# XiangLi2022/CM-TTS

Measured on AMD Instinct MI355X. Metric: mel-frames/s (text->mel hot path, consistency sampling T=4), higher is better.
Workload: dtype f32

## Files before the change

cm-tts_amd/csrc/cmtts_api.hip:

```cpp
#include <hip/hip_runtime.h>
#include <limits.h>
#include <math.h>
#include <stdio.h>
#include <stdlib.h>
#include <string.h>

#include <algorithm>
#include <map>
#include <string>
#include <vector>

#include "../../include/cmtts_hip.h"
#include "internal_hooks.h"
#include "conv_args.h"
#include "kernels.h"
#include "resblock_args.h"
#include "persist_args.h"
#include "cond_gemm.h"
#include "resblock_pair.h"
#include "inproj.h"
#include "attention.h"
#include "text_state.h"
#include "stream_windows.h"

namespace {

thread_local std::string g_err;
int fail(int code, const std::string& msg) {
    g_err = msg;
    return code;
}
#define HIPCHK(x)                                                                              \
    do {                                                                                       \
        hipError_t e_ = (x);                                                                   \
        if (e_ != hipSuccess) return fail(CMTTS_E_HIP, std::string(#x) + ": " + hipGetErrorString(e_)); \
    } while (0)
#define CHK(x)                 \
    do {                       \
        int r_ = (x);          \
        if (r_ != 0) return r_; \
    } while (0)

struct HostTensor {
    std::vector<int64_t> shape;
    std::vector<float> data;
    int64_t dim(int i) const { return i < (int)shape.size() ? shape[i] : 1; }
};

struct PackedConv {
    float* w = nullptr;
    float* bias = nullptr;
    int cout = 0, cin = 0, taps = 0, ld = 0;
    long tap_stride = 0, phase_stride = 0;
};

inline int round_up(int v, int m) { return (v + m - 1) / m * m; }

struct Allocs {
    std::vector<void*> ptrs;
    int upload(const std::vector<float>& h, float** out) {
        void* p = nullptr;
        HIPCHK(hipMalloc(&p, h.size() * sizeof(float) + 256));
        HIPCHK(hipMemcpy(p, h.data(), h.size() * sizeof(float), hipMemcpyHostToDevice));
        ptrs.push_back(p);
        *out = (float*)p;
        return 0;
    }
    int upload_bytes(const void* h, size_t nbytes, void** out) {
        void* p = nullptr;
        HIPCHK(hipMalloc(&p, nbytes + 256));
        HIPCHK(hipMemcpy(p, h, nbytes, hipMemcpyHostToDevice));
        ptrs.push_back(p);
        *out = p;
        return 0;
    }
    void release() {
        for (void* p : ptrs) (void)hipFree(p);
        ptrs.clear();
    }
};

int pack_conv(Allocs& al, const HostTensor& W, const HostTensor* bias, const std::vector<int>* perm, PackedConv* out,
              std::vector<float>* host_copy = nullptr) {
    const int Cout = (int)W.dim(0), Cin = (int)W.dim(1), K = (int)W.dim(2);
    const int ld = round_up(Cout, 4);
    std::vector<float> p((size_t)K * Cin * ld, 0.f);
    for (int k = 0; k < K; ++k)
        for (int ci = 0; ci < Cin; ++ci)
            for (int r = 0; r < Cout; ++r) {
                const int co = perm ? (*perm)[r] : r;
                p[((size_t)k * Cin + ci) * ld + r] = W.data[((size_t)co * Cin + ci) * K + k];
            }
    CHK(al.upload(p, &out->w));
    if (host_copy) *host_copy = p;
    out->bias = nullptr;
    if (bias) {
        std::vector<float> b(Cout);
        for (int r = 0; r < Cout; ++r) b[r] = bias->data[perm ? (*perm)[r] : r];
        CHK(al.upload(b, &out->bias));
    }
    out->cout = Cout; out->cin = Cin; out->taps = K; out->ld = ld;
    out->tap_stride = (long)Cin * ld;
    out->phase_stride = 0;
    return 0;
}

int pack_conv_transpose(Allocs& al, const HostTensor& W, const HostTensor& bias, int s, PackedConv* out,
                        std::vector<float>* two_tap = nullptr) {
    const int Cin = (int)W.dim(0), Cout = (int)W.dim(1), K = (int)W.dim(2);
    const int Q = K / s, ld = round_up(Cout, 4);
    if (two_tap && Q == 2) {
        two_tap->assign((size_t)2 * Cin * s * Cout, 0.f);
        for (int q = 0; q < 2; ++q)
            for (int ci = 0; ci < Cin; ++ci)
                for (int r = 0; r < s; ++r)
                    for (int co = 0; co < Cout; ++co)
                        (*two_tap)[((size_t)q * Cin + ci) * s * Cout + (size_t)r * Cout + co] = W.data[((size_t)ci * Cout + co) * K + (r + s * q)];
    }
    std::vector<float> p((size_t)s * Q * Cin * ld, 0.f);
    for (int r = 0; r < s; ++r)
        for (int q = 0; q < Q; ++q)
            for (int ci = 0; ci < Cin; ++ci)
                for (int co = 0; co < Cout; ++co)
                    p[(((size_t)r * Q + q) * Cin + ci) * ld + co] = W.data[((size_t)ci * Cout + co) * K + (r + s * q)];
    CHK(al.upload(p, &out->w));
    CHK(al.upload(bias.data, &out->bias));
    out->cout = Cout; out->cin = Cin; out->taps = Q; out->ld = ld;
    out->tap_stride = (long)Cin * ld;
    out->phase_stride = (long)Q * Cin * ld;
    return 0;
}

std::vector<float> to_fragment_order(const std::vector<float>& p, int taps, int K, int M) {
    std::vector<float> f((size_t)taps * K * M);
    const int G = K / 8, MTn = M / 32;
    for (int tap = 0; tap < taps; ++tap)
        for (int g = 0; g < G; ++g)
            for (int mt = 0; mt < MTn; ++mt)
                for (int lane = 0; lane < 64; ++lane)
                    for (int j = 0; j < 4; ++j)
                        f[((((size_t)tap * G + g) * MTn + mt) * 64 + lane) * 4 + j] =
                            p[((size_t)tap * K + 8 * g + 2 * j + (lane >> 5)) * M + 32 * mt + (lane & 31)];
    return f;
}

constexpr int WINO_PAD_HG = 4;
std::vector<float> to_wino_fragments(const std::vector<float>& p, int K, int M) {
    std::vector<float> f((size_t)4 * K * M + (size_t)WINO_PAD_HG * (M / 32) * 2 * 64 * 4, 0.0f);
    const int MTn = M / 32;
    for (int hg = 0; hg < K / 4; ++hg)
        for (int mt = 0; mt < MTn; ++mt)
            for (int ps = 0; ps < 2; ++ps)
                for (int lane = 0; lane < 64; ++lane)
                    for (int q = 0; q < 4; ++q) {
                        const int tr = 2 * ps + (q >> 1), k = 4 * hg + 2 * (q & 1) + (lane >> 5), mrow = 32 * mt + (lane & 31);
                        const double g0 = p[((size_t)0 * K + k) * M + mrow], g1 = p[((size_t)1 * K + k) * M + mrow], g2 = p[((size_t)2 * K + k) * M + mrow];
                        const double v = tr == 0 ? g0 : tr == 1 ? 0.5 * (g0 + g1 + g2) : tr == 2 ? 0.5 * (g0 - g1 + g2) : g2;
                        f[((((size_t)hg * MTn + mt) * 2 + ps) * 64 + lane) * 4 + q] = (float)v;
                    }
    return f;
}

constexpr int WINO43_PAD_KS = 4;
std::vector<float> to_wino43_fragments(const std::vector<float>& p, int K, int M) {
    const int NWV = M / 64;
    std::vector<float> f((size_t)(K / 4 + WINO43_PAD_KS) * NWV * 6 * 64 * 4, 0.0f);
    for (int ks = 0; ks < K / 4; ++ks)
        for (int w = 0; w < NWV; ++w)
            for (int tr = 0; tr < 6; ++tr)
                for (int lane = 0; lane < 64; ++lane)
                    for (int e = 0; e < 4; ++e) {
                        const int k = 4 * ks + (lane >> 4), mrow = 64 * w + 16 * e + (lane & 15);
// ... 816 lines not shown
            }
        if (H % 16 == 0 && (NL * C) % 32 == 0 && m->cond_all.ld == NL * C) {
            const std::vector<unsigned short> fs = to_fragment16_split(hp, 1, H, NL * C);
            CHK(al.upload_bytes(fs.data(), fs.size() * 2, &m->cond_all_f16[2]));
        }
    }
    CHK(al.upload(dproj, &m->dproj_wt));
    if (c.multi_speaker) CHK(al.upload(sproj, &m->sproj_wt));
    {
        GET(w, "net.skip_projection.conv.weight", C, C, 1); GET(b, "net.skip_projection.conv.bias", C);
        std::vector<float> hp;
        CHK(pack_conv(al, *w, b, nullptr, &m->skip_proj, &hp));
        if (C % 32 == 0 && m->skip_proj.ld == C) CHK(al.upload(to_fragment_order(hp, 1, C, C), &m->skip_f));
        GET(w2, "net.output_projection.conv.weight", c.n_mels, C, 1); GET(b2, "net.output_projection.conv.bias", c.n_mels);
        CHK(pack_conv(al, *w2, b2, nullptr, &m->out_proj, &hp));
        {
            const int ld = m->out_proj.ld, Mp = round_up(c.n_mels, 32);
            std::vector<float> padded((size_t)C * Mp, 0.f);
            for (int k = 0; k < C; ++k)
                for (int n = 0; n < c.n_mels; ++n) padded[(size_t)k * Mp + n] = hp[(size_t)k * ld + n];
            CHK(al.upload(to_fragment_order(padded, 1, C, Mp), &m->outp_f));
        }
    }
    if (m->cond_all_f && (NL * C) % 512 == 0) {
        GET(pe, va + "pitch_embed.weight", c.pitch_bins, H);
        float* peT = nullptr;
        void* p2 = nullptr;
        CHK(al.upload(transpose2d(pe->data.data(), c.pitch_bins, H), &peT));
        CHK(al.upload(std::vector<float>((size_t)NL * C, 0.f), &m->cond_zero_bias));
        HIPCHK(hipMalloc(&p2, (size_t)NL * C * c.pitch_bins * sizeof(float) + 256));
        al.ptrs.push_back(p2);
        CondGemmArgs ga;
        memset(&ga, 0, sizeof(ga));
        ga.X = peT; ga.Wf = m->cond_all_f; ga.bias = m->cond_all.bias; ga.Y = (float*)p2;
        ga.B = 1; ga.T = c.pitch_bins; ga.M = NL * C; ga.K = H; ga.force = 1; ga.row_split = NL * C / 512;
        if (cmtts_launch_cond_gemm(&ga, nullptr) == 0) {
            void* p2t = nullptr;
            HIPCHK(hipMalloc(&p2t, (size_t)NL * C * c.pitch_bins * sizeof(float) + 256));
            al.ptrs.push_back(p2t);
            k_transpose((const float*)p2, (float*)p2t, NL, C, c.pitch_bins, nullptr);
            HIPCHK(hipStreamSynchronize(nullptr));
            m->cond_p2 = (float*)p2;
            m->cond_p2t = (float*)p2t;
        }
    }
#undef GET
#undef UP
    m->host.clear();
    m->finalized = true;
    return 0;
}

constexpr int FFN2_SEG = 8;
struct TextWs {
    float *x, *h, *qk, *vt, *st, *o, *f, *part, *c1, *c2, *spk, *out1, *h128, *logd, *dround, *epred, *escaled, *pctl;
    int* cum;
    int64_t *eidx, *mlen;
    size_t bytes;
};
TextWs carve_text(const cmtts_config& c, int B, int L, void* base) {
    const int Lp = round_up(L, 4), H = c.hidden;
    Carver cv(base);
    TextWs w;
    const size_t n = (size_t)B * H * Lp;
    w.out1 = cv.take<float>(n);
    w.cum = cv.take<int>((size_t)B * L);
    w.spk = cv.take<float>((size_t)B * H);
    w.h128 = cv.take<float>((size_t)B * c.cwt_hidden * Lp);
    w.x = cv.take<float>(n);
    w.h = cv.take<float>(n);
    w.qk = cv.take<float>(3 * n);
    w.vt = w.qk + 2 * n;
    w.st = cv.take<float>((size_t)B * c.enc_heads * Lp * Lp);
    w.o = cv.take<float>(n);
    w.f = cv.take<float>(4 * n);
    w.part = cv.take<float>(FFN2_SEG * n);
    w.c1 = cv.take<float>(n);
    w.c2 = cv.take<float>(n);
    w.logd = cv.take<float>((size_t)B * L);
    w.dround = cv.take<float>((size_t)B * L);
    w.epred = cv.take<float>((size_t)B * L);
    w.eidx = cv.take<int64_t>((size_t)B * L);
    w.mlen = cv.take<int64_t>((size_t)B);
    w.escaled = cv.take<float>((size_t)B * L);
    w.pctl = cv.take<float>((size_t)B * L);
    w.bytes = cv.off + 256;
    return w;
}

struct FrameWs {
    float *xlr, *h128, *hp, *c1, *c2, *cwt, *r, *s1, *s2, *stats, *f0;
    int64_t* pidx;
    size_t bytes;
};
FrameWs carve_frame(const cmtts_config& c, int B, int T, void* base) {
    Carver cv(base);
    FrameWs w;
    const size_t n = (size_t)B * c.hidden * T;
    w.xlr = cv.take<float>(n);
    w.h128 = cv.take<float>((size_t)B * c.cwt_hidden * T);
    w.hp = cv.take<float>((size_t)B * c.cwt_hidden * T);
    w.c1 = cv.take<float>(n);
    w.c2 = cv.take<float>(n);
    w.cwt = cv.take<float>((size_t)B * T * 16);
    w.r = cv.take<float>((size_t)B * T);
    w.s1 = cv.take<float>((size_t)B * c.cwt_hidden);
    w.s2 = cv.take<float>((size_t)B * c.cwt_hidden);
    w.stats = cv.take<float>((size_t)B * 2);
    w.f0 = cv.take<float>((size_t)B * T);
    w.pidx = cv.take<int64_t>((size_t)B * T);
    w.bytes = cv.off + 256;
    return w;
}

struct DenWs {
    float *hin, *h, *u, *zb, *skip, *emb, *e1, *e2, *dproj, *sproj, *dp, *tbuf, *xcur, *cp;
    float* pst;
    unsigned long long* halo;
    size_t bytes;
};
DenWs carve_den(const cmtts_config& c, int B, int T, void* base) {
    Carver cv(base);
    DenWs w;
    const int C = c.res_channels, NL = c.res_layers;
    const size_t n = (size_t)B * C * T;
    w.hin = cv.take<float>((size_t)B * c.n_mels * T);
    w.h = cv.take<float>(n);
    w.u = cv.take<float>(n);
    w.zb = cv.take<float>(n);
    w.skip = cv.take<float>(n);
    w.emb = cv.take<float>((size_t)B * C);
    w.e1 = cv.take<float>((size_t)B * 4 * C);
    w.e2 = cv.take<float>((size_t)B * C);
    w.dproj = cv.take<float>((size_t)B * NL * C);
    w.sproj = cv.take<float>((size_t)B * NL * C);
    w.dp = cv.take<float>((size_t)B * NL * C);
    w.tbuf = cv.take<float>((size_t)B);
    w.xcur = cv.take<float>((size_t)B * T * c.n_mels);
    w.cp = cv.take<float>((size_t)NL * n);
    w.halo = cv.take<unsigned long long>(cmtts_persist_halo_bytes(B, T) / sizeof(unsigned long long));
    w.pst = cv.take<float>(cmtts_persist_state_floats(B, T));
    w.bytes = cv.off + 256;
    return w;
}

struct EnergyHead {
    const float* xin; const float* e_target; float e_control; const float* bins; int nbins; const float* E; float* out1; int64_t* e_idx; float* e_scaled;
    bool done;
    const float* e_table = nullptr;
};
int g_energy_head = 1;
int g_pred_wino = 1;
int g_pred_xres = 1;
int predictor(const Predictor& P, const float* in, int ld_in, int B, int T, int ld, const int64_t* ln_lens,
              const int64_t* out_lens, float* bufA, float* bufB, float* out, int O, hipStream_t s, int mode16 = 0, bool frame_level = false,
              EnergyHead* eh = nullptr) {
    const float* cur = in;
    int ldc = ld_in;
    auto other = [&](const float* p) { return p == bufA ? bufB : bufA; };
    int pend_ln = -1;
    for (size_t li = 0; li < P.convs.size(); ++li) {
        const PackedConv& w = P.convs[li];
        int rx = -2;
        float* dst = other(cur);
        if (frame_level && !mode16 && g_pred_wino && !ln_lens && li < P.convs_q.size() && P.convs_q[li] && w.taps == 5 && w.cout == 256 &&
            (pend_ln < 0 || w.cin == 256)) {
            ConvXlArgs xa;
            memset(&xa, 0, sizeof(xa));
            xa.x = cur; xa.y = dst; xa.wf = P.convs_q[li]; xa.bias = w.bias; xa.bstride = (long)w.cout * ld;
            xa.B = B; xa.C = 256; xa.T = T; xa.ld = ld; xa.k = w.taps; xa.dil = 1; xa.slope = 1.0f; xa.relu = 1;
            if (w.cin != 256) { xa.cin = w.cin; xa.xbstride = (long)w.cin * ldc; }
            if (pend_ln >= 0) { xa.ln_g = P.ln_g[pend_ln]; xa.ln_b = P.ln_b[pend_ln]; xa.ln_eps = 1e-12f; }
            if (ldc == ld || w.cin != 256) {
                rx = cmtts_launch_conv_k5q(&xa, (void*)s);
                if (rx == -3) return fail(CMTTS_E_HIP, "conv_k5q launch failed");
                if (rx == 0) pend_ln = -2;
            }
        }
        const bool small = (long)((T + 63) / 64) * B < 192;
        if (rx != 0 && !mode16 && g_pred_xres && small && P.convs_f[li] && w.cin == 256 && w.cout == 256 && ldc == ld) {
            ConvArgs a = conv_args(w, cur, T, ldc, (long)w.cin * ldc, dst, ld, (long)w.cout * ld, T);
            a.out[0].act = ACT_RELU;
            a.xres_nt = 1;
            if (pend_ln >= 0) { a.ln_g = P.ln_g[pend_ln]; a.ln_b = P.ln_b[pend_ln]; a.ln_eps = 1e-12f; a.ln_lens = ln_lens; a.ln_skip_tiles = 1; }
            rx = cmtts_launch_conv_xres(&a, P.convs_f[li], B, (void*)s);
            if (rx == -3) return fail(CMTTS_E_HIP, "conv_xres launch failed");
            if (rx == 0) pend_ln = -2;
        }
        if (pend_ln >= 0) {
            float* nd = other(cur);
            k_layernorm_ct(cur, nd, P.ln_g[pend_ln], P.ln_b[pend_ln], 1e-12f, ln_lens, B, T, ld, s);
            cur = nd;
            dst = other(cur);
        }
        pend_ln = -1;
        if (mode16 && li < P.convs_f16[mode16 - 1].size() && P.convs_f16[mode16 - 1][li]) {
            ConvArgs a = conv_args(w, cur, T, ldc, (long)w.cin * ldc, dst, ld, (long)w.cout * ld, T);
            a.out[0].act = ACT_RELU;
            a.text_epi = 1;
            rx = cmtts_launch_conv16(&a, P.convs_f16[mode16 - 1][li], mode16, B, (void*)s);
            if (rx == -3) return fail(CMTTS_E_HIP, "text16: predictor conv launch failed");
        }
        if (rx != 0 && g_pred_xl && P.convs_f[li] && ldc == ld && (long)((T + 63) / 64) * B >= 192) {
            ConvXlArgs xa;
            memset(&xa, 0, sizeof(xa));
            xa.x = cur; xa.y = dst; xa.wf = P.convs_f[li]; xa.bias = w.bias; xa.bstride = (long)w.cout * ld;
            xa.B = B; xa.C = 256; xa.T = T; xa.ld = ld; xa.k = w.taps; xa.dil = 1; xa.slope = 1.0f; xa.relu = 1;
            if (w.cin != 256) { xa.cin = w.cin; xa.xbstride = (long)w.cin * ldc; }
            rx = cmtts_launch_conv_xl(&xa, (void*)s);
            if (rx == -3) return fail(CMTTS_E_HIP, "conv_xl launch failed");
        }
        if (rx != 0) {
            ConvArgs a = conv_args(w, cur, T, ldc, (long)w.cin * ldc, dst, ld, (long)w.cout * ld, T);
            a.out[0].act = ACT_RELU;
            CHK(launch(a, EPI_PLAIN, B, s));
        }
        cur = dst;
        ldc = ld;
        if (g_pred_head && eh && g_energy_head && O == 1 && li + 1 == P.convs.size() && w.cout == 256) {
            k_ln_linear_energy(cur, P.ln_g[li], P.ln_b[li], 1e-12f, P.lin_w, P.lin_b, out, ln_lens, out_lens, B, T, ld, eh->xin, eh->e_target, eh->e_control,
                               eh->bins, eh->nbins, eh->E, eh->out1, eh->e_idx, eh->e_scaled, s, eh->e_table);
            eh->done = true;
            return 0;
        }
        if (g_pred_head && li + 1 == P.convs.size() && w.cout == 256 &&
            k_ln_linear(cur, P.ln_g[li], P.ln_b[li], 1e-12f, P.lin_w, P.lin_b, out, ln_lens, out_lens, B, T, ld, O, s))
            return 0;
        pend_ln = (int)li;
    }
    if (pend_ln >= 0) {
        float* nd = other(cur);
        k_layernorm_ct(cur, nd, P.ln_g[pend_ln], P.ln_b[pend_ln], 1e-12f, ln_lens, B, T, ld, s);
        cur = nd;
    }
    k_chan_linear(cur, P.lin_w, P.lin_b, out, out_lens, B, P.convs.back().cout, T, ld, O, s);
    return 0;
}

int cond_projections(cmtts_model* m, const DenWs& w, const float* cond_ct, int B, int T, hipStream_t s) {
    const cmtts_config& c = m->cfg;
    if (g_cond_gemm16 && m->precision >= 1 && m->precision <= 3 && m->cond_all_f16[m->precision - 1]) {
        CondGemmArgs g;
        g.X = cond_ct; g.Wf = nullptr; g.bias = m->cond_all.bias; g.Y = w.cp;
        g.row_split = 0;
        g.B = B; g.T = T; g.M = c.res_layers * c.res_channels; g.K = c.hidden; g.force = 1;
        const int r = cmtts_launch_cond_gemm16(&g, m->cond_all_f16[m->precision - 1], m->precision, (void*)s);
        if (r == 0) return 0;
        if (r != -2) return fail(CMTTS_E_HIP, "cond_gemm16 launch failed");
    }
    if (m->cond_all_f) {
        CondGemmArgs g;
        g.X = cond_ct; g.Wf = m->cond_all_f; g.bias = m->cond_all.bias; g.Y = w.cp;
        g.row_split = 0;
        g.B = B; g.T = T; g.M = c.res_layers * c.res_channels; g.K = c.hidden; g.force = g_cond_gemm == 2;
        const int r = g_cond_gemm ? cmtts_launch_cond_gemm(&g, (void*)s) : -2;
        if (r == 0) return 0;
        if (r != -2) return fail(CMTTS_E_HIP, "cond_gemm launch failed");
    }
    ConvArgs a = conv_args(m->cond_all, cond_ct, T, T, (long)c.hidden * T, w.cp, T, (long)c.res_layers * c.res_channels * T, T);
    return launch(a, EPI_PLAIN, B, s);
}

struct CondFactors {
    const float* p1 = nullptr;
    const float* p1t = nullptr;
    int ldp = 0, L = 0;
    const int64_t* mel2ph = nullptr;
    const int64_t* p_idx = nullptr;
    bool usable(const cmtts_model* m) const;
};
int g_cond_factored = 1;
int g_cond_inkernel = 1;
inline bool C_IS_256(const cmtts_config& c) { return c.res_channels == 256; }
bool CondFactors::usable(const cmtts_model* m) const {
    return g_cond_factored && p1 && mel2ph && p_idx && m->precision == 0 && m->cond_p2 && g_fused_resblock;
}
int cond_factored(cmtts_model* m, const DenWs& w, const CondFactors& f, int B, int T, hipStream_t s) {
    const cmtts_config& c = m->cfg;
    const int r = cmtts_launch_cond_expand(f.p1, f.ldp, f.L, m->cond_p2, c.pitch_bins, f.mel2ph, f.p_idx, w.cp, B, c.res_layers * c.res_channels, T, (void*)s);
    return r == 0 ? 0 : fail(CMTTS_E_HIP, "cond_expand launch failed");
}
int cond_phoneme_factor(cmtts_model* m, const float* out1, int B, int Lp, float* p1, hipStream_t s) {
    const cmtts_config& c = m->cfg;
    if (!m->cond_p2) return fail(CMTTS_E_UNSUPPORTED, "factored conditioner projections are not available for this model");
    CondGemmArgs g;
    memset(&g, 0, sizeof(g));
    g.X = out1; g.Wf = m->cond_all_f; g.bias = m->cond_zero_bias; g.Y = p1;
    g.B = B; g.T = Lp; g.M = c.res_layers * c.res_channels; g.K = c.hidden; g.force = 1;
    g.flat = 1;
    const long tiles = ((long)B * Lp + 63) / 64;
    const int npass = g.M / 512;
    int best = 1;
    double best_t = 1e30;
    for (int sp = 1; sp <= npass; ++sp) {
        const int ppg = (npass + sp - 1) / sp, groups = (npass + ppg - 1) / ppg;
        const long wg = tiles * groups, cap = persist_blocks();
        const double t = (double)((wg + cap - 1) / cap) * ppg;
        if (t < best_t - 1e-9) { best_t = t; best = sp; }
    }
    g.row_split = best;
    const int r = cmtts_launch_cond_gemm(&g, (void*)s);
    return r == 0 ? 0 : fail(r == -2 ? CMTTS_E_UNSUPPORTED : CMTTS_E_HIP, "cond_gemm (phoneme factor) launch failed");
}

int step_embedding(cmtts_model* m, const DenWs& w, const float* timesteps, const float* spk, int B, hipStream_t s,
                   float t_host = NAN) {
    const cmtts_config& c = m->cfg;
    const int C = c.res_channels, NL = c.res_layers;
    if (c.multi_speaker && !spk) return fail(CMTTS_E_INVALID, "speaker_emb is required for a multi-speaker model");
    const bool cacheable = g_step_cache && t_host == t_host;
    if (cacheable) {
        for (const cmtts_model::StepRow& e : m->step_rows)
            if (e.t == t_host && hipEventQuery(e.ready) == hipSuccess) {
                k_broadcast_row(e.row, w.dproj, B, NL * C, s);
                if (c.multi_speaker) {
                    k_dense_small(spk, c.hidden, 1, m->sproj_wt, nullptr, nullptr, w.sproj, B, c.hidden, NL * C, DENSE_NONE, s);
                    k_add_rows(w.dproj, w.sproj, w.dp, (long)B * NL * C, s);
                }
                return 0;
            }
    }
    k_diff_embed(timesteps, m->omega_res, w.emb, B, C, s);
    k_dense_small(w.emb, C, 1, m->mlp0_wt, nullptr, nullptr, w.e1, B, C, 4 * C, DENSE_MISH, s);
    k_dense_small(w.e1, 4 * C, 1, m->mlp2_wt, nullptr, nullptr, w.e2, B, 4 * C, C, DENSE_NONE, s);
    k_dense_small(w.e2, C, 1, m->dproj_wt, nullptr, nullptr, w.dproj, B, C, NL * C, DENSE_NONE, s);
    if (c.multi_speaker) {
        k_dense_small(spk, c.hidden, 1, m->sproj_wt, nullptr, nullptr, w.sproj, B, c.hidden, NL * C, DENSE_NONE, s);
        k_dense_small(w.e2, C, 1, m->dproj_wt, nullptr, w.sproj, w.dp, B, C, NL * C, DENSE_NONE, s);
    }
    if (cacheable && m->step_rows.size() < 16) {
        bool known = false;
        for (const cmtts_model::StepRow& e : m->step_rows) known = known || e.t == t_host;
        if (!known) {
            cmtts_model::StepRow e{t_host, nullptr, nullptr};
            void* p = nullptr;
            if (hipMalloc(&p, (size_t)NL * C * sizeof(float)) == hipSuccess && hipEventCreateWithFlags(&e.ready, hipEventDisableTiming) == hipSuccess) {
                e.row = (float*)p;
                m->al.ptrs.push_back(p);
                HIPCHK(hipMemcpyAsync(e.row, w.dproj, (size_t)NL * C * sizeof(float), hipMemcpyDeviceToDevice, s));
                HIPCHK(hipEventRecord(e.ready, s));
                m->step_rows.push_back(e);
            } else if (p) {
                (void)hipFree(p);
            }
        }
    }
    return 0;
}

struct MelPost {
    const float* xold;
    const float* noise;
    float c_out, c_skip, nstd;
    float* out;
};

int denoiser_prologue(cmtts_model* m, const DenWs& w, const float* x_src, float in_scale, const float* timesteps, const float* spk, int B,
                      int T, hipStream_t s, bool embed, float t_host, bool* halo_zeroed) {
    const cmtts_config& c = m->cfg;
    const int C = c.res_channels, NL = c.res_layers, M = c.n_mels;
    const long cs = (long)C * T;
    *halo_zeroed = false;
    int rin = -2;
    if (g_inproj_fused && m->in_proj_f) {
        InProjArgs ia;
        memset(&ia, 0, sizeof(ia));
        ia.x = x_src; ia.scale = in_scale; ia.wf = m->in_proj_f; ia.bias = m->in_proj.bias; ia.h = w.h;
        ia.B = B; ia.T = T; ia.M = M; ia.C = C;
        const bool persist_path = g_fused_resblock && g_persist && NL <= PERSIST_MAX_LAYERS;
        if (persist_path) { ia.zero = w.halo; ia.zero_f4 = (long)(cmtts_persist_halo_bytes(B, T) / 16); }
        rin = cmtts_launch_inproj(&ia, (void*)s);
        if (rin == -3) return fail(CMTTS_E_HIP, "inproj launch failed");
        *halo_zeroed = rin == 0 && persist_path && cmtts_persist_halo_bytes(B, T) % 16 == 0;
    }
    if (rin != 0) {
        k_mel_prep(x_src, nullptr, in_scale, w.hin, B, T, M, s);
        ConvArgs a = conv_args(m->in_proj, w.hin, T, T, (long)M * T, w.h, T, cs, T);
        a.out[0].act = ACT_RELU;
        CHK(launch(a, EPI_PLAIN, B, s));
    }
    if (embed) CHK(step_embedding(m, w, timesteps, spk, B, s, t_host));
    return 0;
}

int batch_invariant_form(const cmtts_model* m) {
    if (!m->batch_invariant || m->precision != 0 || !m->winograd || !g_persist_wino || !m->res[0].w3w) return 0;
    return m->winograd == 1 && g_persist_wino == 3 && m->res[0].w3w43 ? 1 : -1;
}
int check_batch_invariant(const cmtts_model* m) {
    if (batch_invariant_form(m) >= 0) return 0;
    return fail(CMTTS_E_UNSUPPORTED, "batch_invariant: the persistent denoiser stack runs the F(2,3) form (model option \"winograd\" = 2), "
                                     "which has no per-layer counterpart; set \"winograd\" to 1 or 0");
}

int denoiser_core(cmtts_model* m, const DenWs& w, const float* x_src, float in_scale, const float* timesteps,
                  const float* cond_ct, const float* spk, int B, int T, const MelPost& post, hipStream_t s, bool embed = true,
                  SideStream* pending = nullptr, float t_host = NAN,
                  const CondFactors* cfk = nullptr, bool* cp_ready = nullptr) {
    CHK(check_device_flag(true));
    const cmtts_config& c = m->cfg;
    const int C = c.res_channels, NL = c.res_layers, M = c.n_mels;
    const long cs = (long)C * T;
    bool halo_zeroed = false;
    CHK(denoiser_prologue(m, w, x_src, in_scale, timesteps, spk, B, T, s, embed, t_host, &halo_zeroed));
    if (pending) CHK(branch_join(pending));
    const float* dp = m->cfg.multi_speaker ? w.dp : w.dproj;
    const bool unfused = !g_fused_resblock;
    float* hcur = w.h;
    float* halt = w.u;
    bool layers_done = false;
    if (!unfused && g_persist && NL <= PERSIST_MAX_LAYERS) {
        PersistArgs pa;
        memset(&pa, 0, sizeof(pa));
        pa.x0 = w.h; pa.cp = w.cp; pa.cp_bstride = (long)NL * C * T;
        pa.dp = dp; pa.d = w.dproj; pa.vec_stride = (long)NL * C;
        pa.skip = w.skip; pa.halo = w.halo; pa.tmo = g_tmo_host;
        pa.B = B; pa.T = T; pa.NL = NL;
        pa.halo_zeroed = halo_zeroed;
        const int prec = m->precision;
        if (cfk && !(cp_ready && *cp_ready)) {
            pa.fact = 1; pa.p1 = cfk->p1; pa.p2 = m->cond_p2; pa.mel2ph = (const long long*)cfk->mel2ph; pa.pidx = (const long long*)cfk->p_idx;
            pa.ldp = cfk->ldp; pa.Lph = cfk->L; pa.ld2 = c.pitch_bins;
            pa.p1t = cfk->p1t; pa.p2t = m->cond_p2t;
        }
        if (g_persist_tail && m->skip_f && m->outp_f) {
            pa.tail = 1;
            pa.Wsf = m->skip_f; pa.bs = m->skip_proj.bias; pa.Wpf = m->outp_f; pa.bp = m->out_proj.bias;
            pa.skip_div = (float)sqrt((double)NL); pa.n_mels = M;
            pa.xold = post.xold; pa.noise = post.noise; pa.c_out = post.c_out; pa.c_skip = post.c_skip; pa.nstd = post.nstd;
            pa.out = post.out;
        }
        pa.wino = g_persist_wino && m->winograd && !prec && m->res[0].w3w && w.pst;
        if (pa.wino && g_persist_wino == 3 && m->winograd == 1 && m->res[0].w3w43) pa.wino = 3;
        pa.xst = w.pst;
        for (int l = 0; l < NL; ++l) {
            pa.W3f[l] = prec ? (const float*)m->res[l].w3f16[prec - 1] : (pa.wino == 3 ? m->res[l].w3w43 : pa.wino ? m->res[l].w3w : m->res[l].w3f);
            pa.Wof[l] = prec ? (const float*)m->res[l].wof16[prec - 1] : m->res[l].wof;
            pa.b3[l] = m->res[l].b3f; pa.bo[l] = m->res[l].outp.bias;
        }
        const bool prof = g_prof.on && g_prof.used + 2 <= g_prof.ev.size();
        const int need = cmtts_persist_plan(B, T, NL, persist_blocks(), g_persist == 2);
        if (need) CHK(persist_admit(s, need, persist_blocks()));
        if (prof) (void)hipEventRecord(g_prof.ev[g_prof.used], s);
        const int rc = prec ? cmtts_launch_denoiser_persist_lp(&pa, prec, persist_blocks(), g_persist == 2, (void*)s)
                            : cmtts_launch_denoiser_persist(&pa, persist_blocks(), g_persist == 2, (void*)s);
        if (rc == -3) return fail(CMTTS_E_HIP, "persistent denoiser launch failed");
        if (rc == 0) {
            CHK(persist_launched(s, need));
            if (prof) { (void)hipEventRecord(g_prof.ev[g_prof.used + 1], s); g_prof.used += 2; }
            layers_done = true;
            if (pa.tail) return 0;
        }
    }
    if (!layers_done && cfk && !(cp_ready && *cp_ready)) {
        CHK(cond_factored(m, w, *cfk, B, T, s));
        if (cp_ready) *cp_ready = true;
    }
    const bool w43 = batch_invariant_form(m) > 0;
    for (int l = 0; l < NL && !layers_done; ++l) {
        const ResLayer& R = m->res[l];
        const bool prof = g_prof.on && g_prof.used + 2 <= g_prof.ev.size() && (g_prof.seen++ % g_prof.stride) == 0;
        if (!unfused) {
            ResArgs ra;
            memset(&ra, 0, sizeof(ra));
            ra.x_in = hcur; ra.cp = w.cp + (long)l * C * T; ra.cp_bstride = (long)NL * C * T;
            ra.dp = dp + (long)l * C; ra.d = w.dproj + (long)l * C;
            ra.x_out = halt; ra.skip = w.skip;
            ra.W3f = R.w3f; ra.b3 = R.b3f; ra.Wof = R.wof; ra.bo = R.outp.bias;
            ra.vec_stride = (long)NL * C; ra.B = B; ra.T = T; ra.accum_skip = l > 0; ra.flag = g_tmo_host;
            if (prof) (void)hipEventRecord(g_prof.ev[g_prof.used], s);
            int lrc;
            if (m->precision == 0 || m->precision == 3) {
                const long tiles32 = (long)((T + 31) / 32) * B;
                ra.z = w.zb;
                if (w43) {
                    ra.W3f = R.w3w43;
                    lrc = cmtts_launch_resblock_w43(&ra, (void*)s);
                } else if (g_split_resblock == 2 || (g_split_resblock == 1 && tiles32 <= SPLIT_MAX_TILES)) lrc = cmtts_launch_resblock_split(&ra, (void*)s);
                else lrc = cmtts_launch_resblock(&ra, (void*)s);
            } else {
                ra.W3f = (const float*)R.w3f16[m->precision - 1];
                ra.Wof = (const float*)R.wof16[m->precision - 1];
                lrc = cmtts_launch_resblock_lp(&ra, m->precision, (void*)s);
            }
            if (lrc != 0) return fail(CMTTS_E_HIP, "fused residual block launch failed");
            if (prof) { (void)hipEventRecord(g_prof.ev[g_prof.used + 1], s); g_prof.used += 2; }
            float* t = hcur; hcur = halt; halt = t;
            continue;
        }
        {
            ConvArgs a = conv_args(R.cond, cond_ct, T, T, (long)c.hidden * T, halt, T, cs, T);
            a.out[0].bvec = dp + (long)l * C; a.out[0].bvec_zs = (long)NL * C;
            a.out[0].res = hcur; a.out[0].r_zs0 = cs; a.out[0].ldr = T;
            CHK(launch(a, EPI_PLAIN, B, s));
        }
        if (w43) {
            ResArgs ra;
            memset(&ra, 0, sizeof(ra));
            ra.u = halt; ra.x_in = hcur; ra.x_out = halt; ra.skip = w.skip; ra.z = w.zb;
            ra.d = w.dproj + (long)l * C; ra.dp = dp + (long)l * C; ra.cp = w.cp;
            ra.W3f = R.w3w43; ra.b3 = R.b3f; ra.Wof = R.wof; ra.bo = R.outp.bias;
            ra.vec_stride = (long)NL * C; ra.B = B; ra.T = T; ra.accum_skip = l > 0;
            if (cmtts_launch_resblock_w43(&ra, (void*)s) != 0) return fail(CMTTS_E_HIP, "F(4,3) residual block launch failed");
            float* t = hcur; hcur = halt; halt = t;
            continue;
        }
        {
            ConvArgs a = conv_args(R.conv3, halt, T, T, cs, w.zb, T, cs, T);
            if (prof) (void)hipEventRecord(g_prof.ev[g_prof.used], s);
            CHK(launch(a, EPI_GATED, B, s));
            if (prof) { (void)hipEventRecord(g_prof.ev[g_prof.used + 1], s); g_prof.used += 2; }
        }
        {
            ConvArgs a = conv_args(R.outp, w.zb, T, T, cs, hcur, T, cs, T);
            a.split = C;
            a.out[0].res = hcur; a.out[0].r_zs0 = cs; a.out[0].ldr = T;
            a.out[0].bvec = w.dproj + (long)l * C; a.out[0].bvec_zs = (long)NL * C;
            a.out[0].rmul = 0.70710678118654752440f;
            a.out[1].Y = w.skip; a.out[1].row_off = C; a.out[1].accum = l > 0;
            CHK(launch(a, EPI_PLAIN, B, s));
        }
    }
    {
        ConvArgs a = conv_args(m->skip_proj, w.skip, T, T, cs, halt, T, cs, T);
        a.pre_div = (float)sqrt((double)NL);
        a.out[0].act = ACT_RELU;
        CHK(launch(a, EPI_PLAIN, B, s));
        ConvArgs b = conv_args(m->out_proj, halt, T, T, cs, w.hin, T, (long)M * T, T);
        CHK(launch(b, EPI_PLAIN, B, s));
    }
    k_mel_post(w.hin, post.xold, post.noise, post.c_out, post.c_skip, post.nstd, post.out, B, T, M, g_tmo_host, s);
    return 0;
}

}

extern "C" {

const char* cmtts_last_error(void) { return g_err.c_str(); }
int cmtts_internal_fail(int code, const char* msg) { return fail(code, msg ? msg : "?"); }
const char* cmtts_version(void) { return "cmtts_hip 0.3 (gfx950)"; }
int cmtts_abi_version(void) { return CMTTS_ABI_VERSION; }

int cmtts_create(const cmtts_config* cfg, cmtts_model** out) {
    if (!cfg || !out) return fail(CMTTS_E_INVALID, "cmtts_create: null argument");
    cmtts_model* m = new cmtts_model();
    m->cfg = *cfg;
    *out = m;
    return 0;
}

int cmtts_set_tensor(cmtts_model* m, const char* name, const float* host_data, const int64_t* shape, int ndim) {
    if (!m || m->finalized) return fail(CMTTS_E_INVALID, "cmtts_set_tensor: model is null or already finalized");
    return set_tensor(m->host, name, host_data, shape, ndim);
}

int cmtts_finalize(cmtts_model* m) {
    if (!m || m->finalized) return fail(CMTTS_E_INVALID, "cmtts_finalize: model is null or already finalized");
    const int r = finalize_model(m);
    if (r != 0) m->al.release();
    if (r == 0 && !g_tmo_host) {
        if (hipHostMalloc((void**)&g_tmo_host, sizeof(unsigned), hipHostMallocMapped) != hipSuccess) g_tmo_host = nullptr;
        else *g_tmo_host = 0;
    }
    return r;
}

void cmtts_destroy(cmtts_model* m) {
    if (!m) return;
    for (cmtts_model::StepRow& e : m->step_rows) (void)hipEventDestroy(e.ready);
    m->al.release();
    delete m;
}

size_t cmtts_text_workspace_bytes(const cmtts_model* m, int B, int L) { return carve_text(m->cfg, B, L, nullptr).bytes; }
size_t cmtts_frame_workspace_bytes(const cmtts_model* m, int B, int T) { return carve_frame(m->cfg, B, T, nullptr).bytes; }
size_t cmtts_denoiser_workspace_bytes(const cmtts_model* m, int B, int T) { return carve_den(m->cfg, B, T, nullptr).bytes; }

int fft_stack(cmtts_model* m, const std::vector<EncLayer>& layers, const TextWs& w, const int64_t* src_lens, int B, int L,
              hipStream_t s, const int64_t* pad_lens = nullptr) {
    const cmtts_config& c = m->cfg;
    const int H = c.hidden, Lp = round_up(L, 4), NH = c.enc_heads, dh = H / NH;
    const long hs = (long)H * Lp;
    const int t96 = (L + 95) / 96, t64 = (L + 63) / 64;
    const bool cols96 = t96 * 96 <= t64 * 64;
    const bool xres_small = g_ffn_xres && g_xres_small && (long)t96 * B * 8 < 128;
    const bool xres_cols = g_ffn_xres && (cols96 || xres_small);
    for (size_t i = 0; i < layers.size(); ++i) {
        const EncLayer& E = layers[i];
        const bool fused_attn = g_attn_fused && dh == 128;
        const int pm = m->precision;
        const bool t16 = m->text16 && (pm == 1 || pm == 2) && E.ffn1_f16[pm - 1] && E.ffn2_f16[pm - 1] && E.qkv_f16[pm - 1] && E.wo_f16[pm - 1];
        const bool ln_qkv = !t16 && fused_attn && (g_text_xres & 1) && E.qkv_f && xres_cols && ((long)t96 * (3 * H / 128) * B >= 128 || xres_small);
        if (!ln_qkv) k_layernorm_ct(w.x, w.h, E.ln1_g, E.ln1_b, 1e-12f, nullptr, B, L, Lp, s);
        bool attn_done = false;
        if (fused_attn) {
            int rq = -2;
            if (ln_qkv) {
                ConvArgs a = conv_args(E.qkv, w.x, L, Lp, hs, w.qk, Lp, 3 * hs, L);
                a.ln_g = E.ln1_g; a.ln_b = E.ln1_b; a.ln_eps = 1e-12f;
                if (g_text_xres & 8) {
                    k_layernorm_ct(w.x, w.h, E.ln1_g, E.ln1_b, 1e-12f, nullptr, B, L, Lp, s);
                    a.X = w.h; a.ln_g = a.ln_b = nullptr;
                }
                a.xres_nt = g_qkv_nt ? g_qkv_nt : ((long)t96 * (3 * H / 128) * B > persist_blocks() ? 1 : 0);
                rq = cmtts_launch_conv_xres(&a, E.qkv_f, B, (void*)s);
// ... 62 lines not shown
            ConvOut& o = a.out[0];
            o.Y = w.o; o.y_zs0 = hs; o.y_zs1 = (long)dh * Lp; o.ldy = Lp; o.Tout = L; o.ostride = 1; o.alpha = 1.f; o.div = 1.f;
            CHK(launch(a, EPI_PLAIN, B * NH, s));
        }
        }
        {
            ConvArgs a = conv_args(E.wo, w.o, L, Lp, hs, w.x, Lp, hs, L);
            a.out[0].res = w.x; a.out[0].r_zs0 = hs; a.out[0].ldr = Lp; a.out[0].lens = src_lens;
            int rc = -2;
            if (t16) {
                a.text_epi = 1;
                rc = cmtts_launch_conv16(&a, E.wo_f16[pm - 1], pm, B, (void*)s);
                if (rc == -3) return fail(CMTTS_E_HIP, "text16: out-projection launch failed");
                a.text_epi = 0;
            } else if (E.wo_f && g_ffn_xres && (g_text_xres & 2)) {
                a.xres_nt = 1;
                rc = cmtts_launch_conv_xres(&a, E.wo_f, B, (void*)s);
                a.xres_nt = 0;
            }
            if (rc == -3) return fail(CMTTS_E_HIP, "conv_xres launch failed");
            if (rc != 0) CHK(launch(a, EPI_PLAIN, B, s));
        }
        if (t16) {
            k_layernorm_ct(w.x, w.h, E.ln2_g, E.ln2_b, 1e-12f, pad_lens, B, L, Lp, s);
            ConvArgs a = conv_args(E.ffn1, w.h, L, Lp, hs, w.f, Lp, 4 * hs, L);
            a.out[0].alpha = (float)pow((double)c.ffn_kernel, -0.5);
            a.out[0].act = ACT_GELU_ERF;
            a.text_epi = 1;
            int rc = cmtts_launch_conv16(&a, E.ffn1_f16[pm - 1], pm, B, (void*)s);
            if (rc == 0) {
                ConvArgs b = conv_args(E.ffn2, w.f, L, Lp, 4 * hs, w.x, Lp, hs, L);
                b.out[0].res = w.x; b.out[0].r_zs0 = hs; b.out[0].ldr = Lp; b.out[0].lens = src_lens;
                b.text_epi = 1;
                rc = cmtts_launch_conv16(&b, E.ffn2_f16[pm - 1], pm, B, (void*)s);
                if (rc != 0) return fail(CMTTS_E_HIP, "text16: FFN linear launch failed");
                continue;
            }
            if (rc != -2) return fail(CMTTS_E_HIP, "text16: FFN conv launch failed");
        }
        const bool ffn2_seg = m->ffn2_split && E.ffn2.cin % FFN2_SEG == 0 && E.ffn2.taps == 1;
        bool ffn_fused = false;
        {
            const float* wqf = g_ffn_wino == 2 ? E.ffn1_q : E.ffn1_p;
            const bool wq = g_ffn_wino && g_ffn_xres && g_ffn_fused && (g_text_xres & 4) && wqf && E.ffn2_f && m->ffn2_split && E.ffn2.cin % FFN2_SEG == 0 &&
                            E.ffn2.taps == 1 && E.ffn1.cout == FFN2_SEG * 128 && H == 256;
            const bool xr = wq || (xres_cols && E.ffn1_f && ((long)t96 * ((E.ffn1.cout + 127) / 128) * B >= 128 || xres_small));
            const bool ln_ffn = xr && (g_text_xres & 4);
            if (!ln_ffn) k_layernorm_ct(w.x, w.h, E.ln2_g, E.ln2_b, 1e-12f, pad_lens, B, L, Lp, s);
            ConvArgs a = conv_args(E.ffn1, ln_ffn ? w.x : w.h, L, Lp, hs, w.f, Lp, 4 * hs, L);
            a.out[0].alpha = (float)pow((double)c.ffn_kernel, -0.5);
            a.out[0].act = ACT_GELU_ERF;
            if (ln_ffn) { a.ln_g = E.ln2_g; a.ln_b = E.ln2_b; a.ln_eps = 1e-12f; a.ln_lens = pad_lens; a.ln_skip_tiles = pad_lens != nullptr; }
            int rc = -2;
            if (xr && g_ffn_fused && ffn2_seg && E.ffn2_f && E.ffn1.cout == FFN2_SEG * 128) {
                a.w2frag = E.ffn2_f; a.part = w.part; a.part_zs0 = (long)FFN2_SEG * hs; a.part_zs1 = hs; a.part_ld = Lp; a.M2 = H;
                rc = wq ? cmtts_launch_conv_xresq(&a, wqf, B, (void*)s, g_ffn_wino == 2 ? 1 : 2) : -2;
                if (rc == -2) rc = cmtts_launch_conv_xres(&a, E.ffn1_f, B, (void*)s);
                if (rc == 0) ffn_fused = true;
                else { a.w2frag = nullptr; a.part = nullptr; }
            }
            if (xr && !ffn_fused) rc = cmtts_launch_conv_xres(&a, E.ffn1_f, B, (void*)s);
            if (rc == -3) return fail(CMTTS_E_HIP, "conv_xres launch failed");
            if (rc != 0) {
                if (ln_ffn) {
                    k_layernorm_ct(w.x, w.h, E.ln2_g, E.ln2_b, 1e-12f, pad_lens, B, L, Lp, s);
                    a.X = w.h; a.ln_g = a.ln_b = nullptr; a.ln_lens = nullptr;
                }
                CHK(launch(a, EPI_PLAIN, B, s));
            }
        }
        if (ffn_fused) {
            k_reduce_partials(w.part, FFN2_SEG, E.ffn2.bias, w.x, src_lens, w.x, B, H, L, Lp, s);
        } else if (ffn2_seg) {
            const int kseg = E.ffn2.cin / FFN2_SEG;
            ConvArgs a = conv_args(E.ffn2, w.f, L, Lp, 4 * hs, w.part, Lp, (long)FFN2_SEG * hs, L);
            a.K = kseg;
            a.zdiv = FFN2_SEG; a.a_zs0 = 0; a.a_zs1 = (long)kseg * a.a_ld; a.x_zs1 = (long)kseg * Lp;
            a.out[0].y_zs1 = hs; a.out[0].bias = nullptr;
            CHK(launch(a, EPI_PLAIN, B * FFN2_SEG, s));
            k_reduce_partials(w.part, FFN2_SEG, E.ffn2.bias, w.x, src_lens, w.x, B, H, L, Lp, s);
        } else {
            ConvArgs a = conv_args(E.ffn2, w.f, L, Lp, 4 * hs, w.x, Lp, hs, L);
            a.out[0].res = w.x; a.out[0].r_zs0 = hs; a.out[0].ldr = Lp; a.out[0].lens = src_lens;
            CHK(launch(a, EPI_PLAIN, B, s));
        }
    }
    return 0;
}

int cmtts_text_forward(cmtts_model* m, const int64_t* texts, const int64_t* src_lens, const float* spker_embeds,
                       const int64_t* speakers, int B, int L, float d_control, float* log_d, float* d_rounded, int64_t* mel_len,
                       float* e_pred, int64_t* e_idx, float* enc_out_ct, float* speaker_emb,
                       void* text_ws, size_t text_ws_bytes, void* stream) {
    return cmtts_text_forward_ragged(m, texts, src_lens, nullptr, spker_embeds, speakers, B, L, d_control, log_d, d_rounded, mel_len, e_pred,
                                     e_idx, enc_out_ct, speaker_emb, text_ws, text_ws_bytes, stream);
}

int cmtts_text_forward_ragged(cmtts_model* m, const int64_t* texts, const int64_t* src_lens, const int64_t* pad_lens, const float* spker_embeds,
                              const int64_t* speakers, int B, int L, float d_control, float* log_d, float* d_rounded, int64_t* mel_len,
                              float* e_pred, int64_t* e_idx, float* enc_out_ct, float* speaker_emb,
                              void* text_ws, size_t text_ws_bytes, void* stream) {
    if (!m || !m->finalized) return fail(CMTTS_E_INVALID, "model not finalized");
    if (!texts || !src_lens || !text_ws || B <= 0 || L <= 0) return fail(CMTTS_E_INVALID, "cmtts_text_forward: bad argument");
    const cmtts_config& c = m->cfg;
    if (c.multi_speaker && c.n_speaker > 0 && !speakers) return fail(CMTTS_E_INVALID, "speakers (ids into the speaker_emb table) are required (model/cmtts.py:78)");
    if (c.multi_speaker && c.n_speaker <= 0 && !spker_embeds) return fail(CMTTS_E_INVALID, "Speaker embedding should not be None (model/cmtts.py:80)");
    const cmtts_control_tables& ct = m->ct;
    if ((ct.d || ct.e || ct.p) && ct.ld != L)
        return fail(CMTTS_E_INVALID, "cmtts_text_forward: the control tables' row pitch ld must equal L (cmtts_set_control_tables)");
    if (ct.d && d_control != 1.0f)
        return fail(CMTTS_E_INVALID, "cmtts_text_forward: a duration table replaces d_control, which must then be 1");
    if (ct.e && m->vc.e_control != 1.0f)
        return fail(CMTTS_E_INVALID, "cmtts_text_forward: an energy table replaces e_control, which must then be 1");
    TextWs w = carve_text(c, B, L, text_ws);
    if (text_ws_bytes < w.bytes) return fail(CMTTS_E_WORKSPACE, "text workspace too small");
    hipStream_t s = (hipStream_t)stream;
    const int H = c.hidden, Lp = round_up(L, 4);
    if (!log_d) log_d = w.logd;
    if (!d_rounded) d_rounded = w.dround;
    if (!mel_len) mel_len = w.mlen;
    if (!e_pred) e_pred = w.epred;
    if (!e_idx) e_idx = w.eidx;

    k_embed_tokens(texts, src_lens, m->embed, m->omega_h, m->pe_h, PE_ROWS, w.x, B, L, Lp, H, (float)sqrt((double)H), s);
    CHK(fft_stack(m, m->enc, w, src_lens, B, L, s, pad_lens));
    k_layernorm_ct(w.x, w.x, m->encln_g, m->encln_b, 1e-5f, src_lens, B, L, Lp, s);
    if (enc_out_ct && c.multi_speaker)
        k_copy_rows(enc_out_ct, L, w.x, Lp, L, (long)B * H, s);
    if (c.multi_speaker) {
        if (c.n_speaker > 0) k_gather_rows(m->spk_table, speakers, w.spk, B, H, c.n_speaker, s);
        else k_dense_small(spker_embeds, c.external_speaker_dim, 1, m->spk_wt, m->spk_b, nullptr, w.spk, B,
                      c.external_speaker_dim, H, DENSE_NONE, s);
        k_add_rowvec(w.x, w.spk, B, H, L, Lp, s, pad_lens);
        if (speaker_emb) HIPCHK(hipMemcpyAsync(speaker_emb, w.spk, (size_t)B * H * 4, hipMemcpyDeviceToDevice, s));
    }
    SideStream* ss = side_for(s);
    hipStream_t se = ss ? ss->side : s;
    float* ec1 = ss ? w.qk : w.c1;
    float* ec2 = ss ? w.qk + (size_t)B * H * Lp : w.c2;
    if (ss) CHK(branch_fork(ss));
    const int t16mode = (m->text16 && (m->precision == 1 || m->precision == 2)) ? m->precision : 0;
    CHK(predictor(m->dur, w.x, Lp, B, L, Lp, src_lens, src_lens, w.c1, w.c2, log_d, 1, s, t16mode));
    if (m->vc.d_target) {
        HIPCHK(hipMemcpyAsync(d_rounded, m->vc.d_target, (size_t)B * L * 4, hipMemcpyDeviceToDevice, s));
        k_cumsum_durations(m->vc.d_target, w.cum, mel_len, B, L, s);
    } else if (ct.d) {
        k_durations_table(log_d, ct.d, d_rounded, w.cum, mel_len, B, L, s);
    } else {
        k_durations(log_d, d_control, d_rounded, w.cum, mel_len, B, L, s);
    }
    if (ct.p) HIPCHK(hipMemcpyAsync(w.pctl, ct.p, (size_t)B * L * 4, hipMemcpyDeviceToDevice, s));
    if (enc_out_ct && !c.multi_speaker)
        k_copy_rows(enc_out_ct, L, w.x, Lp, L, (long)B * H, s);
    k_pos_embed_add(w.x, w.h, m->energy.alpha, m->omega_h, m->pe_h, PE_ROWS, B, H, L, Lp, se);
    EnergyHead eh{w.x, m->vc.e_target, m->vc.e_control, m->energy_bins, c.energy_bins - 1, m->energy_emb, w.out1, e_idx, w.escaled, false, ct.e};
    CHK(predictor(m->energy, w.h, Lp, B, L, Lp, pad_lens, pad_lens, ec1, ec2, e_pred, 1, se, t16mode, false, H == 256 ? &eh : nullptr));
    if (ss) CHK(branch_join(ss));
    if (!eh.done)
        k_energy_embed(w.x, e_pred, w.escaled, m->vc.e_target, m->vc.e_control, m->energy_bins, c.energy_bins - 1, m->energy_emb,
                       w.out1, e_idx, B, H, L, Lp, s, ct.e);
    {
        ConvArgs a = conv_args(m->cwt_in, w.out1, L, Lp, (long)H * Lp, w.h128, Lp, (long)c.cwt_hidden * Lp, L);
        int rc = -2;
        if (g_ffn_xres && g_pred_xres && m->cwt_in_f) {
            a.xres_nt = 1;
            rc = cmtts_launch_conv_xres(&a, m->cwt_in_f, B, (void*)s);
            if (rc == -3) return fail(CMTTS_E_HIP, "conv_xres launch failed");
            a.xres_nt = 0;
        }
        if (rc != 0) CHK(launch(a, EPI_PLAIN, B, s));
    }
    if (!m->vc.e_target && (ct.e || m->vc.e_control != 1.0f))
        HIPCHK(hipMemcpyAsync(e_pred, w.escaled, (size_t)B * L * 4, hipMemcpyDeviceToDevice, s));
    HIPCHK(hipGetLastError());
    return 0;
}

int cmtts_frame_forward(cmtts_model* m, const void* text_ws, int B, int L, int T, float* cond_ct, int64_t* mel2ph,
                        float* cwt_out, float* f0_denorm, int64_t* p_idx, float* f0_stats, void* frame_ws,
                        size_t frame_ws_bytes, void* stream) {
    return cmtts_frame_forward_sub(m, text_ws, B, L, 0, B, T, cond_ct, mel2ph, cwt_out, f0_denorm, p_idx, f0_stats, nullptr, frame_ws, frame_ws_bytes, stream);
}

int cmtts_frame_forward_sub(cmtts_model* m, const void* text_ws, int B_all, int L_all, int b0, int B, int T, float* cond_ct, int64_t* mel2ph,
                            float* cwt_out, float* f0_denorm, int64_t* p_idx, float* f0_stats, float* cond_p1, void* frame_ws,
                            size_t frame_ws_bytes, void* stream) {
    return cmtts_frame_forward_sub_t(m, text_ws, B_all, L_all, b0, B, T, cond_ct, mel2ph, cwt_out, f0_denorm, p_idx, f0_stats, cond_p1, nullptr, frame_ws,
                                     frame_ws_bytes, stream);
}

int cmtts_frame_forward_sub_t(cmtts_model* m, const void* text_ws, int B_all, int L_all, int b0, int B, int T, float* cond_ct, int64_t* mel2ph,
                              float* cwt_out, float* f0_denorm, int64_t* p_idx, float* f0_stats, float* cond_p1, float* cond_p1t, void* frame_ws,
                              size_t frame_ws_bytes, void* stream) {
    if (!m || !m->finalized) return fail(CMTTS_E_INVALID, "model not finalized");
    if (!text_ws || !frame_ws || !cond_ct || !mel2ph || B <= 0 || L_all <= 0 || T <= 0 || b0 < 0 || b0 + B > B_all)
        return fail(CMTTS_E_INVALID, "cmtts_frame_forward: bad argument");
    const cmtts_config& c = m->cfg;
    const int L = L_all;
    TextWs tw = carve_text(c, B_all, L_all, const_cast<void*>(text_ws));
    tw.out1 += (size_t)b0 * c.hidden * round_up(L_all, 4);
    tw.h128 += (size_t)b0 * c.cwt_hidden * round_up(L_all, 4);
    tw.cum += (size_t)b0 * L_all;
    tw.pctl += (size_t)b0 * L_all;
    if (m->ct.p && m->ct.ld != L_all)
        return fail(CMTTS_E_INVALID, "cmtts_frame_forward: the control tables' row pitch ld must equal L_all (cmtts_set_control_tables)");
    if (m->ct.p && m->vc.p_control != 1.0f)
        return fail(CMTTS_E_INVALID, "cmtts_frame_forward: a pitch table replaces p_control, which must then be 1");
    FrameWs w = carve_frame(c, B, T, frame_ws);
    if (frame_ws_bytes < w.bytes) return fail(CMTTS_E_WORKSPACE, "frame workspace too small");
    hipStream_t s = (hipStream_t)stream;
    const int H = c.hidden, Lp = round_up(L, 4), O = c.use_uv ? 11 : 10, CH = c.cwt_hidden;
    if (!cwt_out) cwt_out = w.cwt;
    if (!f0_denorm) f0_denorm = w.f0;
    if (!p_idx) p_idx = w.pidx;
    if (!f0_stats) f0_stats = w.stats;

    SideStream* ss = side_for(s);
    hipStream_t sst = ss ? ss->side : s;
    if (ss) CHK(branch_fork(ss));
    if (cond_p1t && !cond_p1) return fail(CMTTS_E_INVALID, "cmtts_frame_forward_sub_t: cond_p1t needs cond_p1");
    if (cond_p1 && m->cond_p2) {
        CHK(cond_phoneme_factor(m, tw.out1, B, Lp, cond_p1, sst));
        if (cond_p1t) k_transpose(cond_p1, cond_p1t, B * c.res_layers, c.res_channels, Lp, sst);
    }
    if (!(g_stats_mlp && k_stats_mlp(tw.out1, (long)H * Lp, Lp, m->st0_wt, m->st0_b, m->st2_wt, m->st2_b, m->st4_wt, m->st4_b, f0_stats, B, H, CH, CH, 2, sst))) {
        k_dense_small(tw.out1, (long)H * Lp, Lp, m->st0_wt, m->st0_b, nullptr, w.s1, B, H, CH, DENSE_RELU, sst);
        k_dense_small(w.s1, CH, 1, m->st2_wt, m->st2_b, nullptr, w.s2, B, CH, CH, DENSE_RELU, sst);
        k_dense_small(w.s2, CH, 1, m->st4_wt, m->st4_b, nullptr, f0_stats, B, CH, 2, DENSE_NONE, sst);
    }
    k_mel2ph(tw.cum, mel2ph, B, L, T, s);
    if (!g_cwt_in_phoneme) k_length_regulate(tw.out1, mel2ph, w.xlr, B, H, Lp, T, s);
    bool hp_done = false;
    if (g_cwt_in_phoneme) {
        k_pos_embed_add_lr(tw.h128, Lp, mel2ph, m->cwt_in.bias, w.hp, m->cwt.alpha, m->omega_cwt, m->pe_cwt, PE_ROWS, B, CH, T, s);
        hp_done = true;
    } else {
        ConvArgs a = conv_args(m->cwt_in, w.xlr, T, T, (long)H * T, w.h128, T, (long)CH * T, T);
        CHK(launch(a, EPI_PLAIN, B, s));
    }
    if (!hp_done) k_pos_embed_add(w.h128, w.hp, m->cwt.alpha, m->omega_cwt, m->pe_cwt, PE_ROWS, B, CH, T, T, s);
    CHK(predictor(m->cwt, w.hp, T, B, T, T, nullptr, nullptr, w.c1, w.c2, cwt_out, O, s, (m->text16 && (m->precision == 1 || m->precision == 2)) ? m->precision : 0, true));
    if (ss) CHK(branch_join(ss));
    if (m->ct.p) k_pitch_table_scale(cwt_out, mel2ph, tw.cum, tw.pctl, B, O, L, T, s);
    else if (m->vc.p_control != 1.0f) k_scale(cwt_out, cwt_out, (long)B * T * O, m->vc.p_control, s);
    if (m->vc.cwt_spec) {
        k_pitch_index(m->vc.cwt_spec, 10, m->vc.f0_mean, m->vc.f0_std, 1, 1.0f, nullptr, 0, c.use_uv ? m->vc.uv : nullptr,
                      c.pitch_norm_eps, w.r, p_idx, f0_denorm, B, T, s);
    } else {
        k_pitch_index(cwt_out, O, f0_stats, f0_stats + 1, 2, c.cwt_std_scale, c.use_uv ? cwt_out + (O - 1) : nullptr, O, nullptr,
                      c.pitch_norm_eps, w.r, p_idx, f0_denorm, B, T, s);
    }
    if (g_cwt_in_phoneme) k_lr_gather_add(tw.out1, mel2ph, Lp, p_idx, m->pitch_emb, cond_ct, B, H, T, s);
    else k_gather_add(w.xlr, p_idx, m->pitch_emb, cond_ct, B, H, T, s);
    HIPCHK(hipGetLastError());
    return 0;
}

namespace {
struct TextStateLayout {
    long off[TEXT_STATE_MAX_REGIONS], bytes[TEXT_STATE_MAX_REGIONS], stride[TEXT_STATE_MAX_REGIONS];
    long rec_bytes;
    int n_regions;
};
TextStateLayout text_state_layout(const cmtts_config& c, int L, bool with_p) {
    const int Lp = round_up(L, 4);
    TextStateLayout t;
    t.bytes[0] = (long)c.hidden * Lp * 4;
    t.bytes[1] = (long)c.cwt_hidden * Lp * 4;
    t.bytes[2] = (long)c.hidden * 4;
    t.bytes[3] = (long)L * 4;
    t.bytes[4] = (long)L * 4;
    t.n_regions = with_p ? 5 : 4;
    long off = TEXT_STATE_HEADER_BYTES;
    for (int g = 0; g < t.n_regions; ++g) {
        t.stride[g] = t.bytes[g];
        t.off[g] = off;
        off += (t.bytes[g] + 15) / 16 * 16;
    }
    t.rec_bytes = off;
    return t;
}
TextStateCopy text_state_args(const cmtts_config& c, void* ws, int B_all, int L, void* records, int n, int unpack, bool with_p) {
    const TextStateLayout t = text_state_layout(c, L, with_p);
    TextWs tw = carve_text(c, B_all, L, ws);
    char* base[TEXT_STATE_MAX_REGIONS] = {(char*)tw.out1, (char*)tw.h128, (char*)tw.spk, (char*)tw.cum, (char*)tw.pctl};
    TextStateCopy a;
    memset(&a, 0, sizeof(a));
    int chunks = 0;
    for (int g = 0; g < t.n_regions; ++g) {
        TextStateRegion& R = a.reg[g];
        R.ws = base[g]; R.ws_stride = t.stride[g]; R.rec_off = t.off[g]; R.bytes = t.bytes[g];
        R.vec16 = ((uintptr_t)R.ws % 16 == 0 && R.ws_stride % 16 == 0 && R.bytes % 16 == 0 && (uintptr_t)records % 16 == 0) ? 1 : 0;
        R.chunk0 = chunks;
        chunks += (int)((R.bytes + TEXT_STATE_CHUNK - 1) / TEXT_STATE_CHUNK);
    }
    a.n_regions = t.n_regions; a.n_chunks = chunks; a.unpack = unpack;
    a.layout = with_p ? TEXT_STATE_LAYOUT_P : TEXT_STATE_LAYOUT;
    a.n = n; a.B_all = B_all; a.L_all = L; a.hidden = c.hidden; a.cwt_hidden = c.cwt_hidden;
    a.rec = (char*)records; a.rec_bytes = t.rec_bytes;
    a.cum = tw.cum;
    return a;
}
}

size_t cmtts_text_state_record_bytes(const cmtts_model* m, int L_all) {
    if (!m || L_all <= 0) return 0;
    return (size_t)text_state_layout(m->cfg, L_all, m->ct.p != nullptr).rec_bytes;
}

int cmtts_text_state_pack(cmtts_model* m, const void* text_ws, int B_all, int L_all, const int32_t* rows, int n, const int64_t* global_idx,
                          const int64_t* src_lens, void* records, void* stream) {
    if (!m || !m->finalized) return fail(CMTTS_E_INVALID, "model not finalized");
    if (!text_ws || !records || (n > 0 && !rows) || B_all <= 0 || L_all <= 0 || n < 0)
        return fail(CMTTS_E_INVALID, "cmtts_text_state_pack: bad argument");
    if ((uintptr_t)records % 16) return fail(CMTTS_E_INVALID, "cmtts_text_state_pack: records must be 16-byte aligned");
    if (m->ct.p && m->ct.ld != L_all)
        return fail(CMTTS_E_INVALID, "cmtts_text_state_pack: the control tables' row pitch ld must equal L_all (cmtts_set_control_tables)");
    TextStateCopy a = text_state_args(m->cfg, const_cast<void*>(text_ws), B_all, L_all, records, n, 0, m->ct.p != nullptr);
    a.rows = rows; a.index = global_idx; a.src_lens = src_lens;
    if (cmtts_launch_text_state_copy(&a, stream) != 0) return fail(CMTTS_E_HIP, "text-state pack launch failed");
    return 0;
}

int cmtts_text_state_unpack(cmtts_model* m, const void* records, int n, int L_all, void* text_ws, size_t text_ws_bytes, void* stream) {
    if (!m || !m->finalized) return fail(CMTTS_E_INVALID, "model not finalized");
    if (!text_ws || !records || n <= 0 || L_all <= 0) return fail(CMTTS_E_INVALID, "cmtts_text_state_unpack: bad argument");
    if ((uintptr_t)records % 16) return fail(CMTTS_E_INVALID, "cmtts_text_state_unpack: records must be 16-byte aligned");
    if (text_ws_bytes < carve_text(m->cfg, n, L_all, nullptr).bytes) return fail(CMTTS_E_WORKSPACE, "text workspace too small");
    if (m->ct.p && m->ct.ld != L_all)
        return fail(CMTTS_E_INVALID, "cmtts_text_state_unpack: the control tables' row pitch ld must equal L_all (cmtts_set_control_tables)");
    TextStateCopy a = text_state_args(m->cfg, text_ws, n, L_all, const_cast<void*>(records), n, 1, m->ct.p != nullptr);
    if (cmtts_launch_text_state_copy(&a, stream) != 0) return fail(CMTTS_E_HIP, "text-state unpack launch failed");
    return 0;
}

int cmtts_length_regulate(const float* x_ct, const float* durations, int B, int C, int L, int T, float* out_ct,
                          int64_t* mel2ph, int64_t* mel_len, int32_t* scratch_cum, void* stream) {
    if (!x_ct || !durations || !out_ct || !mel2ph || !mel_len || !scratch_cum || B <= 0 || L <= 0 || T <= 0)
        return fail(CMTTS_E_INVALID, "cmtts_length_regulate: bad argument");
    hipStream_t s = (hipStream_t)stream;
    k_cumsum_durations(durations, scratch_cum, mel_len, B, L, s);
    k_mel2ph(scratch_cum, mel2ph, B, L, T, s);
    k_length_regulate(x_ct, mel2ph, out_ct, B, C, L, T, s);
    HIPCHK(hipGetLastError());
    return 0;
}

int cmtts_denoiser_forward(cmtts_model* m, const float* x, const float* timesteps, const float* cond_ct,
                           const float* speaker_emb, int B, int T, float* out, void* ws, size_t ws_bytes, void* stream) {
    if (!m || !m->finalized) return fail(CMTTS_E_INVALID, "model not finalized");
    if (!x || !timesteps || !cond_ct || !out || !ws || B <= 0 || T <= 0)
        return fail(CMTTS_E_INVALID, "cmtts_denoiser_forward: bad argument");
    CHK(check_batch_invariant(m));
    DenWs w = carve_den(m->cfg, B, T, ws);
    if (ws_bytes < w.bytes) return fail(CMTTS_E_WORKSPACE, "denoiser workspace too small");
    hipStream_t s = (hipStream_t)stream;
    SideStream* ss = g_fused_resblock ? side_for(s) : nullptr;
    if (ss) CHK(branch_fork(ss));
    if (g_fused_resblock) CHK(cond_projections(m, w, cond_ct, B, T, ss ? ss->side : s));
    const MelPost post = {nullptr, nullptr, 1.0f, 0.0f, 0.0f, out};
    CHK(denoiser_core(m, w, x, 1.0f, timesteps, cond_ct, speaker_emb, B, T, post, s, true, ss));
    HIPCHK(hipGetLastError());
    return 0;
}

int cmtts_schedule(const cmtts_model* m, int n_steps, float* sigmas, float* renoise_std) {
    if (!m || !sigmas || !renoise_std || n_steps < 1) return fail(CMTTS_E_INVALID, "cmtts_schedule: bad argument");
    const cmtts_config& c = m->cfg;
    if (n_steps == 1) {
        sigmas[0] = c.sigma_max;
        renoise_std[0] = -1.0f;
        return 0;
    }
    const double rho = c.rho, tmax = pow((double)c.sigma_max, 1.0 / rho), tmin = pow((double)c.sigma_min, 1.0 / rho);
    for (int i = 0; i < n_steps; ++i) {
        const double tsi = 0.0, tsn = (i + 1 == n_steps) ? 1.0 : 0.0;
        const double t = pow(tmax + tsi / 1.0 * (tmin - tmax), rho);
        double nt = pow(tmax + tsn / 1.0 * (tmin - tmax), rho);
        nt = nt < c.sigma_min ? (double)c.sigma_min : (nt > c.sigma_max ? (double)c.sigma_max : nt);
        sigmas[i] = (float)t;
        renoise_std[i] = (float)sqrt(nt * nt - (double)c.sigma_min * (double)c.sigma_min);
    }
    return 0;
}

}
namespace {
int sample_core(cmtts_model* m, const DenWs& w, const float* noise, long noise_stride, const float* cond_ct, const float* speaker_emb, int B,
                int T, int n_steps, const float* sigmas, const float* renoise_std, float* mel, hipStream_t s, const CondFactors* cf = nullptr) {
    const cmtts_config& c = m->cfg;
    const long nel = (long)B * T * c.n_mels;
    SideStream* ss = g_fused_resblock ? side_for(s) : nullptr;
    if (ss) CHK(branch_fork(ss));
    const CondFactors* cfk = nullptr;
    CondFactors cf_local;
    bool cp_ready = false;
    if (g_fused_resblock) {
        if (cf && cf->usable(m)) {
            const bool inkernel = g_cond_inkernel && g_persist && g_persist_tail && m->skip_f && m->outp_f && c.res_layers <= PERSIST_MAX_LAYERS &&
                                  cmtts_persist_plan(B, T, c.res_layers, persist_blocks(), g_persist == 2) > 0;
            if (inkernel && cf->ldp <= T && m->cond_p2t && C_IS_256(c)) {
                cf_local = *cf;
                if (!cf_local.p1t) {
                    k_transpose(cf->p1, w.cp, B * c.res_layers, c.res_channels, cf->ldp, ss ? ss->side : s);
                    cf_local.p1t = w.cp;
                }
                cfk = &cf_local;
            } else CHK(cond_factored(m, w, *cf, B, T, ss ? ss->side : s));
        } else CHK(cond_projections(m, w, cond_ct, B, T, ss ? ss->side : s));
    }
    k_scale(noise, w.xcur, nel, c.sigma_max, s);
    const float smin = c.sigma_min, sd2 = c.sigma_data * c.sigma_data;
    for (int i = 0; i < n_steps; ++i) {
        const float sg = sigmas[i];
        const float dm = sg - smin;
        const float c_skip = sd2 / (dm * dm + sd2);
        const float rt = sqrtf(sg * sg + sd2);
        const float c_out = dm * c.sigma_data / rt;
        const float c_in = 1.0f / rt;
        const float t_resc = 250.0f * logf(sg + 1e-44f);
        const bool new_sigma = i == 0 || sigmas[i] != sigmas[i - 1];
        const bool embed_side = i == 0 && ss != nullptr;
        if (new_sigma) k_fill_float(w.tbuf, t_resc, B, embed_side ? ss->side : s);
        if (embed_side) CHK(step_embedding(m, w, w.tbuf, speaker_emb, B, ss->side, t_resc));
        const bool last = i + 1 == n_steps;
        const bool renoise = renoise_std[i] >= 0.0f;
        const MelPost post = {w.xcur, renoise ? noise + (long)(1 + i) * noise_stride : nullptr, c_out, c_skip,
                              renoise ? renoise_std[i] : 0.0f, last ? mel : w.xcur};
        CHK(denoiser_core(m, w, w.xcur, c_in, w.tbuf, cond_ct, speaker_emb, B, T, post, s, new_sigma && !embed_side, i == 0 ? ss : nullptr, t_resc, cfk, &cp_ready));
    }
    HIPCHK(hipGetLastError());
    return 0;
}

DenWs den_slice(const cmtts_config& c, const DenWs& w, int b0, int T) {
    const long C = c.res_channels, NL = c.res_layers, M = c.n_mels;
    DenWs v = w;
    v.hin += (long)b0 * M * T; v.h += b0 * C * T; v.u += b0 * C * T; v.zb += b0 * C * T; v.skip += b0 * C * T;
    v.emb += b0 * C; v.e1 += b0 * 4 * C; v.e2 += b0 * C; v.dproj += b0 * NL * C; v.sproj += b0 * NL * C; v.dp += b0 * NL * C;
    v.tbuf += b0; v.xcur += (long)b0 * T * M; v.cp += (long)b0 * NL * C * T;
    return v;
}
}
extern "C" {

int cmtts_sample(cmtts_model* m, const float* noise, const float* cond_ct, const float* speaker_emb, int B, int T,
                 int n_steps, const float* sigmas, const float* renoise_std, float* mel, void* ws, size_t ws_bytes,
                 void* stream) {
    if (!m || !m->finalized) return fail(CMTTS_E_INVALID, "model not finalized");
    if (!noise || !cond_ct || !mel || !ws || !sigmas || !renoise_std || B <= 0 || T <= 0 || n_steps < 1)
        return fail(CMTTS_E_INVALID, "cmtts_sample: bad argument");
    CHK(check_batch_invariant(m));
    const cmtts_config& c = m->cfg;
    DenWs w = carve_den(c, B, T, ws);
    if (ws_bytes < w.bytes) return fail(CMTTS_E_WORKSPACE, "denoiser workspace too small");
    return sample_core(m, w, noise, (long)B * T * c.n_mels, cond_ct, speaker_emb, B, T, n_steps, sigmas, renoise_std, mel, (hipStream_t)stream);
}

int cmtts_sample_factored(cmtts_model* m, const float* noise, const float* cond_ct, const float* speaker_emb, int B, int T,
                          int n_steps, const float* sigmas, const float* renoise_std, float* mel, void* ws, size_t ws_bytes,
                          void* stream, const float* cond_p1, int p1_ld, int L, const int64_t* mel2ph, const int64_t* p_idx) {
    return cmtts_sample_factored_t(m, noise, cond_ct, speaker_emb, B, T, n_steps, sigmas, renoise_std, mel, ws, ws_bytes, stream, cond_p1, nullptr, p1_ld, L,
                                   mel2ph, p_idx);
}

int cmtts_sample_factored_t(cmtts_model* m, const float* noise, const float* cond_ct, const float* speaker_emb, int B, int T,
                            int n_steps, const float* sigmas, const float* renoise_std, float* mel, void* ws, size_t ws_bytes,
                            void* stream, const float* cond_p1, const float* cond_p1t, int p1_ld, int L, const int64_t* mel2ph, const int64_t* p_idx) {
    if (!m || !m->finalized) return fail(CMTTS_E_INVALID, "model not finalized");
    if (!noise || !cond_ct || !mel || !ws || !sigmas || !renoise_std || B <= 0 || T <= 0 || n_steps < 1)
        return fail(CMTTS_E_INVALID, "cmtts_sample_factored: bad argument");
    if (cond_p1 && (!mel2ph || !p_idx || L <= 0 || p1_ld < L)) return fail(CMTTS_E_INVALID, "cmtts_sample_factored: incomplete factors");
    CHK(check_batch_invariant(m));
    const cmtts_config& c = m->cfg;
    DenWs w = carve_den(c, B, T, ws);
    if (ws_bytes < w.bytes) return fail(CMTTS_E_WORKSPACE, "denoiser workspace too small");
    CondFactors cf;
    cf.p1 = cond_p1; cf.ldp = p1_ld; cf.L = L; cf.mel2ph = mel2ph; cf.p_idx = p_idx;
    cf.p1t = cond_p1 ? cond_p1t : nullptr;
    return sample_core(m, w, noise, (long)B * T * c.n_mels, cond_ct, speaker_emb, B, T, n_steps, sigmas, renoise_std, mel, (hipStream_t)stream,
                       cond_p1 ? &cf : nullptr);
}

int cmtts_sample_ragged(cmtts_model* m, const cmtts_sample_group* groups, int n_groups, int n_steps, const float* sigmas,
                        const float* renoise_std, int tail_frames, void* stream) {
    if (!m || !m->finalized) return fail(CMTTS_E_INVALID, "model not finalized");
    if (!groups || n_groups < 1 || n_steps < 1 || !sigmas || !renoise_std || tail_frames < 0)
        return fail(CMTTS_E_INVALID, "cmtts_sample_ragged: bad argument");
    CHK(check_batch_invariant(m));
    const cmtts_config& c = m->cfg;
    const int C = c.res_channels, NL = c.res_layers, M = c.n_mels;
    hipStream_t s = (hipStream_t)stream;
    long padded_tiles = 0;
    for (int g = 0; g < n_groups; ++g) {
        const cmtts_sample_group& G = groups[g];
        if (!G.noise || !G.cond_ct || !G.mel || !G.ws || G.B <= 0 || G.T <= 0) return fail(CMTTS_E_INVALID, "cmtts_sample_ragged: bad group");
        if (c.multi_speaker && !G.speaker_emb) return fail(CMTTS_E_INVALID, "speaker_emb is required for a multi-speaker model");
        if (G.ws_bytes < carve_den(c, G.B, G.T, nullptr).bytes) return fail(CMTTS_E_WORKSPACE, "denoiser workspace too small");
        padded_tiles += (long)G.B * ((G.T + 63) / 64);
    }
    bool one_launch = m->precision == 0 && g_fused_resblock && g_persist && g_persist_tail && g_inproj_fused && m->skip_f && m->outp_f &&
                      m->in_proj_f && NL <= PERSIST_MAX_LAYERS && n_groups <= PERSIST_MAX_GROUPS && padded_tiles * 2 > persist_blocks();
    for (int g = 0; g < n_groups && one_launch; ++g)
        if ((groups[g].T + 63) / 64 > 127 || (groups[g].T + 63) / 64 > std::min(persist_blocks(), PERSIST_MAX_WG) || groups[g].B > 1023 || (long)C * groups[g].T >= (1L << 30) ||
            cmtts_persist_halo_bytes(groups[g].B, groups[g].T) % 16 != 0)
            one_launch = false;
    if (!one_launch) {
        for (int g = 0; g < n_groups; ++g) {
            const cmtts_sample_group& G = groups[g];
            const int rc = cmtts_sample_factored(m, G.noise, G.cond_ct, G.speaker_emb, G.B, G.T, n_steps, sigmas, renoise_std, G.mel, G.ws, G.ws_bytes,
                                                 stream, G.cond_p1, G.p1_ld, G.L, G.mel2ph, G.p_idx);
            if (rc != 0) return rc;
        }
        return 0;
    }
    CHK(check_device_flag(true));
    const int cap_all = std::min(persist_blocks(), PERSIST_MAX_WG);
    auto utt_tiles = [&](const cmtts_sample_group& G, int b, int eval) {
        const int tiles = (G.T + 63) / 64;
        if (!G.active_frames) return (long)tiles;
        const long need = (long)G.active_frames[b] + tail_frames + (long)NL * (n_steps - eval);
        return std::min<long>(tiles, std::max<long>(1, (need + 63) / 64));
    };
    std::vector<int> keep(n_groups);
    {
        long total = 0;
        for (int g = 0; g < n_groups; ++g) {
            keep[g] = groups[g].B;
            for (int b = 0; b < groups[g].B; ++b) total += utt_tiles(groups[g], b, 0);
        }
        if (total > cap_all) {
            std::vector<int> order(n_groups), k2 = keep;
            for (int g = 0; g < n_groups; ++g) order[g] = g;
            std::sort(order.begin(), order.end(), [&](int x, int y) { return groups[x].T < groups[y].T; });
            long out = 0, rest = total;
            for (int g : order) {
                while (rest > cap_all && k2[g] > 0) {
                    const long t = utt_tiles(groups[g], k2[g] - 1, 0);
                    out += t; rest -= t; --k2[g];
                }
                if (rest <= cap_all) break;
            }
            if (rest <= cap_all && rest > 0 && out <= 64) keep = k2;
        }
    }
    bool fact_all = g_cond_inkernel != 0;
    for (int g = 0; g < n_groups && fact_all; ++g) {
        if (keep[g] == 0) continue;
        CondFactors cf;
        cf.p1 = groups[g].cond_p1; cf.ldp = groups[g].p1_ld; cf.L = groups[g].L; cf.mel2ph = groups[g].mel2ph; cf.p_idx = groups[g].p_idx;
        if (!cf.usable(m) || groups[g].p1_ld > groups[g].T || !m->cond_p2t) fact_all = false;
    }
    std::vector<DenWs> ws(n_groups);
    SideStream* ss = side_for(s);
    struct JoinGuard {
        SideStream* ss; bool armed;
        ~JoinGuard() { if (armed && ss) (void)branch_join(ss); }
    } guard{ss, false};
    if (ss) { CHK(branch_fork(ss)); guard.armed = true; }
    bool any_aside = false;
    for (int g = 0; g < n_groups; ++g) {
        const cmtts_sample_group& G = groups[g];
        ws[g] = carve_den(c, G.B, G.T, G.ws);
        if (keep[g] < G.B) any_aside = true;
        if (keep[g] == 0) continue;
        CondFactors cf;
        cf.p1 = G.cond_p1; cf.ldp = G.p1_ld; cf.L = G.L; cf.mel2ph = G.mel2ph; cf.p_idx = G.p_idx;
        if (fact_all) {
            k_transpose(G.cond_p1, ws[g].cp, keep[g] * NL, C, G.p1_ld, s);
        }
        else if (cf.usable(m)) CHK(cond_factored(m, ws[g], cf, keep[g], G.T, ss ? ss->side : s));
        else CHK(cond_projections(m, ws[g], G.cond_ct, keep[g], G.T, ss ? ss->side : s));
        k_scale(G.noise, ws[g].xcur, (long)keep[g] * G.T * M, c.sigma_max, s);
        if (G.active_frames) HIPCHK(hipMemsetAsync(G.mel, 0, (size_t)keep[g] * G.T * M * sizeof(float), s));
    }
    if (ss) { guard.armed = false; CHK(branch_join(ss)); }
    if (any_aside) {
        hipStream_t q = ss ? ss->side : s;
        if (ss) { CHK(branch_fork(ss)); guard.armed = true; }
        const int prev_persist = g_persist;
        g_persist = 0;
        int rc = 0;
// ... 472 lines not shown
    if (!(max_wav_value > 0.f && max_wav_value <= 32768.f)) return fail(CMTTS_E_INVALID, "cmtts_vocoder_forward_windows: max_wav_value outside (0, 32768]");
    if (ws_bytes < cmtts_vocoder_windows_workspace_bytes(v, N, Tw)) return fail(CMTTS_E_WORKSPACE, "cmtts_vocoder_forward_windows: workspace too small");
    hipStream_t s = (hipStream_t)stream;
    std::vector<StreamWindow> tab(N);
    hipPointerAttribute_t at{};
    const bool known = hipPointerGetAttributes(&at, windows) == hipSuccess;
    if (!known) (void)hipGetLastError();
    const bool on_host = known && at.type == hipMemoryTypeHost;
    const bool on_dev = known && (at.type == hipMemoryTypeDevice || at.type == hipMemoryTypeManaged || at.type == hipMemoryTypeUnified);
    if (!on_host && !on_dev) return fail(CMTTS_E_INVALID, "cmtts_vocoder_forward_windows: the window table must be device or page-locked host memory");
    if (on_host) {
        memcpy(tab.data(), windows, (size_t)N * sizeof(StreamWindow));
    } else {
        HIPCHK(hipMemcpyAsync(tab.data(), windows, (size_t)N * sizeof(StreamWindow), hipMemcpyDeviceToHost, s));
        HIPCHK(hipStreamSynchronize(s));
    }
    for (int n = 0; n < N; ++n) {
        const StreamWindow& w = tab[n];
        char msg[200];
        const char* bad = w.b < 0 || w.b >= B                                   ? "utterance outside [0, B)"
                          : w.start < 0 || (long)w.start + Tw > T              ? "window outside [0, T)"
                          : w.core_len <= 0 || w.core_len > core               ? "core_len outside [1, core]"
                          : w.core_off < 0 || (long)w.core_off + w.core_len > Tw ? "core_off + core_len > Tw"
                                                                                  : nullptr;
        if (bad) {
            snprintf(msg, sizeof msg, "cmtts_vocoder_forward_windows: window %d (%d, %d, %d, %d): %s", n, w.b, w.start, w.core_off, w.core_len, bad);
            return fail(CMTTS_E_INVALID, msg);
        }
    }
    Carver cv(ws);
    float* mel_w = cv.take<float>((size_t)N * 80 * Tw);
    StreamWindow* win = cv.take<StreamWindow>(N);
    void* gws = cv.base + ((cv.off + 255) & ~(size_t)255);
    if (on_host) HIPCHK(hipMemcpyAsync(win, windows, (size_t)N * sizeof(StreamWindow), hipMemcpyHostToDevice, s));
    else HIPCHK(hipMemcpyAsync(win, windows, (size_t)N * sizeof(StreamWindow), hipMemcpyDeviceToDevice, s));
    if (cmtts_launch_mel_window_gather(mel_ct, 80, T, win, N, Tw, mel_w, (void*)s) != 0) return fail(CMTTS_E_HIP, "mel window gather launch failed");
    const float* x = nullptr;
    int ch = 0, Ti = 0, ld = 0;
    if (const int rc = vocoder_generator(v, mel_w, N, Tw, gws, s, &x, &ch, &Ti, &ld)) return rc;
    long hop = 1;
    for (int i = 0; i < 4; ++i) hop *= v->up_rate[i];
    const int rc = cmtts_launch_conv_post_windows(x, v->post_w, v->post_b, 3.0f, 0.01f, win, N, ch, Ti, ld, v->post_k, (int)hop, core,
                                                  max_wav_value, pcm, (void*)s);
    if (rc == -2) return fail(CMTTS_E_UNSUPPORTED, "cmtts_vocoder_forward_windows: conv_post kernel wider than 7");
    if (rc != 0) return fail(CMTTS_E_HIP, "conv_post windows launch failed");
    return 0;
}
int cmtts_internal_mel_window_gather(const float* mel_ct, int B, int T, const int32_t* windows, int N, int Tw, float* out, void* stream) {
    (void)B;
    if (!mel_ct || !windows || !out || N <= 0 || Tw <= 0 || Tw > T) return fail(CMTTS_E_INVALID, "cmtts_internal_mel_window_gather: bad argument");
    return cmtts_launch_mel_window_gather(mel_ct, 80, T, (const StreamWindow*)windows, N, Tw, out, stream) == 0 ? 0
                                                                                                              : fail(CMTTS_E_HIP, "gather launch failed");
}

struct Knob { const char* name; int* var; int lo, hi; };
static int knob_set(const Knob* tab, size_t n, const char* name, int value, bool* found) {
    for (size_t i = 0; i < n; ++i)
        if (!strcmp(name, tab[i].name)) {
            *found = true;
            const int prev = *tab[i].var;
            if (value >= tab[i].lo && value <= tab[i].hi) *tab[i].var = value;
            return prev;
        }
    *found = false;
    return 0;
}

int cmtts_set_option(const char* name, int value) {
    if (!name) return fail(CMTTS_E_INVALID, "cmtts_set_option: null name");
    if (!strcmp(name, "cooperative_launch")) {
        const int prev = cmtts_persist_set_cooperative(value == 2 ? -1 : (value == 0 || value == 1) ? value : -2);
        return prev < 0 ? 2 : prev;
    }
    if (!strcmp(name, "process_group")) {
        return cmtts_persist_note_process_group(value);
    }
    static const Knob tab[] = {
        {"branch_streams", &g_branch_streams, 0, 1},
        {"resblock_split", &g_split_resblock, 0, 2},
        {"step_cache", &g_step_cache, 0, 1},
    };
    bool found;
    const int prev = knob_set(tab, sizeof(tab) / sizeof(tab[0]), name, value, &found);
    if (found) return prev;
    return fail(CMTTS_E_INVALID, "cmtts_set_option: unknown option");
}

int cmtts_model_set_option(cmtts_model* m, const char* name, int value) {
    if (!m || !name) return fail(CMTTS_E_INVALID, "cmtts_model_set_option: null argument");
    const Knob tab[] = {
        {"ffn2_split", &m->ffn2_split, 0, 1},
        {"text16", &m->text16, 0, 1},
        {"winograd", &m->winograd, 0, 2},
        {"batch_invariant", &m->batch_invariant, 0, 1},
    };
    bool found;
    const int prev = knob_set(tab, sizeof(tab) / sizeof(tab[0]), name, value, &found);
    if (found) return prev;
    return fail(CMTTS_E_INVALID, "cmtts_model_set_option: unknown option");
}

int cmtts_vocoder_set_option(cmtts_vocoder* v, const char* name, int value) {
    if (!v || !name) return fail(CMTTS_E_INVALID, "cmtts_vocoder_set_option: null argument");
    const Knob tab[] = {
        {"ups16", &v->ups16, 0, 1},
        {"winograd", &v->winograd, 0, 1},
        {"batch_invariant", &v->batch_invariant, 0, 1},
    };
    bool found;
    const int prev = knob_set(tab, sizeof(tab) / sizeof(tab[0]), name, value, &found);
    if (found) return prev;
    return fail(CMTTS_E_INVALID, "cmtts_vocoder_set_option: unknown option");
}

int cmtts_internal_set(const char* name, int value) {
    if (!name) return fail(CMTTS_E_INVALID, "cmtts_internal_set: null name");
    static const Knob tab[] = {
        {"qkv_nt", &g_qkv_nt, 0, 3},
        {"cwt_in_phoneme", &g_cwt_in_phoneme, 0, 1},
        {"pred_xres", &g_pred_xres, 0, 1},
        {"xres_small", &g_xres_small, 0, 1},
        {"cond_inkernel", &g_cond_inkernel, 0, 1},
        {"cond_factored", &g_cond_factored, 0, 1},
        {"cond_gemm16", &g_cond_gemm16, 0, 1},
        {"cond_gemm", &g_cond_gemm, 0, 2},
        {"persist_tail", &g_persist_tail, 0, 1},
        {"persist_wino", &g_persist_wino, 0, 3},
        {"inproj_fused", &g_inproj_fused, 0, 1},
        {"ffn_xres", &g_ffn_xres, 0, 1},
        {"ffn_wino", &g_ffn_wino, 0, 2},
        {"ffn_fused", &g_ffn_fused, 0, 1},
        {"text_xres", &g_text_xres, 0, 15},
        {"attn_fused", &g_attn_fused, 0, 1},
        {"pred_xl", &g_pred_xl, 0, 1},
        {"pred_head", &g_pred_head, 0, 1},
        {"voc_pair", &g_voc_pair, 0, 2},
        {"voc_pair3", &g_voc_pair3, 0, 1},
        {"voc_pairw", &g_voc_pairw, 0, 1},
        {"voc_pair128", &g_voc_pair128, 0, 1},
        {"voc_rb16", &g_voc_rb16, 0, 2},
        {"voc_xl", &g_voc_xl, 0, 1},
        {"voc_wino64_k", &g_voc_wino64_k, 3, 99},
        {"voc_wino43", &g_voc_wino43, 0, 3},
        {"voc_qpair", &g_voc_qpair, 0, 2},
        {"voc_wino64", &g_voc_wino64, 0, 1},
        {"voc_wino", &g_voc_wino, 0, 2},
        {"voc_xl16", &g_voc_xl16, 0, 1},
        {"voc_upsT", &g_voc_upsT, 0, 1},
        {"post_v4", &g_post_v4, 0, 1},
        {"pred_wino", &g_pred_wino, 0, 1},
        {"energy_head", &g_energy_head, 0, 1},
        {"stats_mlp", &g_stats_mlp, 0, 1},
        {"text_xt16", &g_conv_xt16, 0, 1},
    };
    if (!strcmp(name, "voc_xl_split")) return cmtts_xl_set_split(value);
    if (!strcmp(name, "attn_qb")) return cmtts_attention_set_qb(value);
    if (!strcmp(name, "xres_nt")) return cmtts_xres_set_nt(value);
    bool found;
    const int prev = knob_set(tab, sizeof(tab) / sizeof(tab[0]), name, value, &found);
    if (found) return prev;
    return fail(CMTTS_E_INVALID, "cmtts_internal_set: unknown switch");
}

int cmtts_internal_cond_projections(cmtts_model* m, const float* cond_ct, int B, int T, float* cp, void* stream) {
    if (!m || !cond_ct || !cp || B <= 0 || T <= 0) return fail(CMTTS_E_INVALID, "cmtts_internal_cond_projections: bad argument");
    DenWs w;
    memset(&w, 0, sizeof(w));
    w.cp = cp;
    return cond_projections(m, w, cond_ct, B, T, (hipStream_t)stream);
}

int cmtts_internal_cond_factored(cmtts_model* m, const float* p1, int p1_ld, int L, const int64_t* mel2ph, const int64_t* p_idx, int B, int T,
                                 float* cp, void* stream) {
    if (!m || !m->finalized || !p1 || !mel2ph || !p_idx || !cp) return fail(CMTTS_E_INVALID, "cmtts_internal_cond_factored: bad argument");
    if (!m->cond_p2) return fail(CMTTS_E_UNSUPPORTED, "no pitch-table factor for this model");
    DenWs w;
    memset(&w, 0, sizeof(w));
    w.cp = cp;
    CondFactors cf;
    cf.p1 = p1; cf.ldp = p1_ld; cf.L = L; cf.mel2ph = mel2ph; cf.p_idx = p_idx;
    return cond_factored(m, w, cf, B, T, (hipStream_t)stream);
}

int cmtts_poll_error(void) { return check_device_flag(); }

int cmtts_set_persistent_denoiser(int mode) {
    const int prev = g_persist;
    if (mode >= 0 && mode <= 2) g_persist = mode;
    return prev;
}

int cmtts_set_fused_resblock(int on) {
    const int prev = g_fused_resblock ? 1 : 0;
    g_fused_resblock = on != 0;
    return prev;
}

int cmtts_set_precision(cmtts_model* m, int mode) {
    if (!m || mode < 0 || mode > 3) return fail(CMTTS_E_INVALID, "cmtts_set_precision: mode 0 (fp32), 1 (bf16), 2 (fp16) or 3 (fp16x3)");
    m->precision = mode;
    return 0;
}

int cmtts_set_variance_controls(cmtts_model* m, const cmtts_variance_controls* vc) {
    if (!m) return fail(CMTTS_E_INVALID, "cmtts_set_variance_controls: null model");
    const cmtts_variance_controls off = {1.f, 1.f, nullptr, nullptr, nullptr, nullptr, nullptr, nullptr};
    if (!vc) { m->vc = off; return 0; }
    if (!(vc->p_control > 0.f) || !(vc->e_control == vc->e_control))
        return fail(CMTTS_E_INVALID, "cmtts_set_variance_controls: p_control must be > 0 (it also scales the uv logit)");
    if (vc->cwt_spec && (!vc->f0_mean || !vc->f0_std || (m->cfg.use_uv && !vc->uv)))
        return fail(CMTTS_E_INVALID, "cmtts_set_variance_controls: a pitch target needs cwt_spec, f0_mean, f0_std (and uv)");
    m->vc = *vc;
    return 0;
}

int cmtts_set_control_tables(cmtts_model* m, const cmtts_control_tables* t) {
    if (!m) return fail(CMTTS_E_INVALID, "cmtts_set_control_tables: null model");
    const cmtts_control_tables off = {nullptr, nullptr, nullptr, 0};
    if (!t) t = &off;
    if ((t->d || t->e || t->p) && t->ld <= 0)
        return fail(CMTTS_E_INVALID, "cmtts_set_control_tables: ld (the row pitch = L of the next text-side call) must be > 0");
    m->ct = *t;
    return 0;
}

int cmtts_vocoder_set_precision(cmtts_vocoder* v, int mode) {
    if (!v || mode < 0 || mode > 3) return fail(CMTTS_E_INVALID, "cmtts_vocoder_set_precision: mode 0 (fp32), 1 (bf16), 2 (fp16) or 3 (fp16x3)");
    v->precision = mode;
    return 0;
}

int cmtts_set_resblock_tile(int frames) {
    if (frames != 0 && frames != 32 && frames != 64) return fail(CMTTS_E_INVALID, "cmtts_set_resblock_tile: 0, 32 or 64");
    cmtts_resblock_set_tile(frames);
    return 0;
}

int cmtts_set_debug_stamps(void* dev_buf) {
    cmtts_resblock_set_debug((long long*)dev_buf);
    cmtts_persist_set_debug((long long*)dev_buf);
    cmtts_pair_set_debug((long long*)dev_buf);
    cmtts_xres_set_debug((long long*)dev_buf);
    {
        int M = 0, K = 0;
        const char* mk = getenv("CMTTS_CONV_DBG_MK");
        if (mk && sscanf(mk, "%d,%d", &M, &K) == 2) cmtts_conv_set_debug(dev_buf ? (long long*)dev_buf : nullptr, M, K);
        else cmtts_conv_set_debug(nullptr, 0, 0);
    }
    return 0;
}

int cmtts_profile_begin(int max_launches, int stride) {
    if (max_launches <= 0 || stride <= 0) return fail(CMTTS_E_INVALID, "cmtts_profile_begin: bad argument");
    g_prof.stride = stride;
    g_prof.seen = 0;
    for (hipEvent_t e : g_prof.ev) (void)hipEventDestroy(e);
    g_prof.ev.assign((size_t)max_launches * 2, nullptr);
    for (auto& e : g_prof.ev) HIPCHK(hipEventCreate(&e));
    g_prof.used = 0;
    g_prof.on = true;
    return 0;
}
int cmtts_profile_end(double* total_ms, int* n_launches) {
    if (!total_ms || !n_launches) return fail(CMTTS_E_INVALID, "cmtts_profile_end: bad argument");
    g_prof.on = false;
    double tot = 0.0;
    for (size_t i = 0; i + 1 < g_prof.used; i += 2) {
        HIPCHK(hipEventSynchronize(g_prof.ev[i + 1]));
        float ms = 0.f;
        HIPCHK(hipEventElapsedTime(&ms, g_prof.ev[i], g_prof.ev[i + 1]));
        tot += ms;
    }
    *total_ms = tot;
    *n_launches = (int)(g_prof.used / 2);
    for (hipEvent_t e : g_prof.ev) (void)hipEventDestroy(e);
    g_prof.ev.clear();
    g_prof.used = 0;
    return 0;
}

int cmtts_wav_to_int16(const float* wav, int16_t* pcm, int64_t n, float max_wav_value, void* stream) {
    if (!wav || !pcm || n < 0) return fail(CMTTS_E_INVALID, "cmtts_wav_to_int16: bad argument");
    if (n) k_wav_to_int16(wav, pcm, (long)n, max_wav_value, (hipStream_t)stream);
    HIPCHK(hipGetLastError());
    return 0;
}

size_t cmtts_decoder_workspace_bytes(const cmtts_model* m, int B, int T) { return carve_text(m->cfg, B, T, nullptr).bytes; }

int cmtts_decoder_forward(cmtts_model* m, const float* x_ct, const int64_t* lens, int B, int T, float* out_ct, void* ws,
                          size_t ws_bytes, void* stream) {
    if (!m || !m->finalized) return fail(CMTTS_E_INVALID, "model not finalized");
    if (m->dec.empty()) return fail(CMTTS_E_INVALID, "cmtts_decoder_forward: the state dict held no decoder.* tensors");
    if (!x_ct || !lens || !out_ct || !ws || B <= 0 || T <= 0) return fail(CMTTS_E_INVALID, "cmtts_decoder_forward: bad argument");
    if (T + 1 >= PE_ROWS) return fail(CMTTS_E_UNSUPPORTED, "cmtts_decoder_forward: T exceeds the position table");
    const cmtts_config& c = m->cfg;
    TextWs w = carve_text(c, B, T, ws);
    if (ws_bytes < w.bytes) return fail(CMTTS_E_WORKSPACE, "decoder workspace too small");
    hipStream_t s = (hipStream_t)stream;
    const int H = c.hidden, Tp = round_up(T, 4);
    k_copy_rows(w.f, Tp, x_ct, T, T, (long)B * H, s);
    k_pos_embed_add(w.f, w.x, m->dec_alpha, m->omega_h, m->pe_h, PE_ROWS, B, H, T, Tp, s, lens);
    CHK(fft_stack(m, m->dec, w, lens, B, T, s));
    k_layernorm_ct(w.x, w.x, m->decln_g, m->decln_b, 1e-5f, lens, B, T, Tp, s);
    k_copy_rows(out_ct, T, w.x, Tp, T, (long)B * H, s);
    HIPCHK(hipGetLastError());
    return 0;
}

int cmtts_length_mask(const int64_t* lens, uint8_t* mask, int B, int W, void* stream) {
    if (!lens || !mask || B <= 0 || W < 0) return fail(CMTTS_E_INVALID, "cmtts_length_mask: bad argument");
    if (W == 0) return 0;
    k_length_mask(lens, mask, B, W, (hipStream_t)stream);
    HIPCHK(hipGetLastError());
    return 0;
}

int cmtts_transpose(const float* in, float* out, int B, int R, int C, void* stream) {
    if (!in || !out || B <= 0 || R <= 0 || C <= 0) return fail(CMTTS_E_INVALID, "cmtts_transpose: bad argument");
    k_transpose(in, out, B, R, C, (hipStream_t)stream);
    HIPCHK(hipGetLastError());
    return 0;
}

int cmtts_pack_conv_weight(const float* host_w, int Cout, int Cin, int K, float** dev_packed, int* ld) {
    if (!host_w || !dev_packed || !ld || Cout <= 0 || Cin <= 0 || K <= 0) return fail(CMTTS_E_INVALID, "cmtts_pack_conv_weight: bad argument");
    HostTensor W;
    W.shape = {Cout, Cin, K};
    W.data.assign(host_w, host_w + (size_t)Cout * Cin * K);
    Allocs al;
    PackedConv p;
    CHK(pack_conv(al, W, nullptr, nullptr, &p));
    *dev_packed = p.w;
    *ld = p.ld;
// ... 23 lines not shown
```

cm-tts_amd/csrc/cond_gemm.h:

```cpp
#pragma once

struct CondGemmArgs {
    const float* X;
    const float* Wf;
    const float* bias;
    float* Y;
    int B, T, M, K;
    int force;
    int flat;
    int row_split;
};

#ifdef __cplusplus
extern "C" {
#endif
int cmtts_launch_cond_gemm(const CondGemmArgs* a, void* stream);
int cmtts_launch_cond_expand(const float* p1, int ldp, int L, const float* p2, int ld2, const int64_t* mel2ph, const int64_t* pidx,
                             float* cp, int B, int M, int T, void* stream);
int cmtts_launch_cond_gemm16(const CondGemmArgs* a, const void* wf16, int mode, void* stream);
#ifdef __cplusplus
}
#endif
```

cm-tts_amd/csrc/cond_gemm.hip:

```cpp
#include <hip/hip_runtime.h>
#include "cond_gemm.h"

typedef float f32x16 __attribute__((ext_vector_type(16)));
typedef float f32x4 __attribute__((ext_vector_type(4)));

namespace {

constexpr int K = 256;
constexpr int NW = 8;
constexpr int MT = 2;
constexpr int FN = 64;
constexpr int NT = FN / 32;
constexpr int X_LD = FN + 4;
constexpr int RING = 4;
constexpr int NG = K / 8;

__device__ __forceinline__ float ldg(const float* base, unsigned idx) {
    return *reinterpret_cast<const float*>(reinterpret_cast<const char*>(base) + (size_t)(idx * 4u));
}
__device__ __forceinline__ int acc_row(int r, int lane) { return (r & 3) + 8 * (r >> 2) + 4 * (lane >> 5); }

__global__ __launch_bounds__(64 * NW, 2) void cond_gemm_kernel(const CondGemmArgs a) {
    extern __shared__ __attribute__((aligned(16))) float xs[];
    const int tid = threadIdx.x, lane = tid & 63, w = tid >> 6;
    const int t0 = blockIdx.x * FN;
    const int l31 = lane & 31, khalf = lane >> 5;
    const int T = a.T;
    const long ncol = a.flat ? (long)a.B * T : T;
    auto col_x = [&](long c) -> long { return a.flat ? (c / T) * (long)K * T + (c % T) : (long)blockIdx.y * K * T + c; };
    auto col_y = [&](long c) -> long { return a.flat ? (c / T) * (long)a.M * T + (c % T) : (long)blockIdx.y * a.M * T + c; };
    const float* xin = a.X;
    float* yb = a.Y;

    {
        const long t = t0 + lane;
        const long xo = col_x(t < ncol ? t : ncol - 1);
#pragma unroll 1
        for (int i = 0; i < K / NW; i += 8) {
            float xv[8];
#pragma unroll
            for (int q = 0; q < 8; ++q) xv[q] = xin[xo + (long)(w * (K / NW) + i + q) * T];
#pragma unroll
            for (int q = 0; q < 8; ++q) xs[(w * (K / NW) + i + q) * X_LD + lane] = t < ncol ? xv[q] : 0.f;
        }
    }
    const int MTn = a.M / 32;
    auto load_a = [&](f32x4 (&dst)[MT], int mt0, int g) {
#pragma unroll
        for (int i = 0; i < MT; ++i)
            dst[i] = *reinterpret_cast<const f32x4*>(a.Wf + (((long)g * MTn + mt0 + i) * 64 + lane) * 4);
    };
    auto load_b = [&](float (&dst)[4][NT], int g) {
        const float* bs = xs + (g * 8 + khalf) * X_LD + l31;
#pragma unroll
        for (int kk = 0; kk < 4; ++kk)
#pragma unroll
            for (int j = 0; j < NT; ++j) dst[kk][j] = bs[2 * kk * X_LD + j * 32];
    };
    const int npass_all = a.M / (32 * MT * NW);
    const int ppg = (npass_all + (int)gridDim.z - 1) / (int)gridDim.z;
    const int p_first = (int)blockIdx.z * ppg;
    const int npass = min(npass_all, p_first + ppg);
    if (p_first >= npass) return;
    f32x4 A[RING][MT];
#pragma unroll
    for (int s = 0; s < RING - 1; ++s) load_a(A[s], (p_first * NW + w) * MT, s);
    __syncthreads();

    for (int p = p_first; p < npass; ++p) {
        const int mt0 = (p * NW + w) * MT;
        f32x16 acc[MT][NT];
#pragma unroll
        for (int i = 0; i < MT; ++i)
#pragma unroll
            for (int j = 0; j < NT; ++j)
#pragma unroll
                for (int r = 0; r < 16; ++r) acc[i][j][r] = 0.f;
        float Bv[2][4][NT];
        load_b(Bv[0], 0);
        const int mt_next = (min(p + 1, npass - 1) * NW + w) * MT;
#pragma unroll 1
        for (int it = 0; it < NG; it += RING) {
#pragma unroll
            for (int s = 0; s < RING; ++s) {
                const int nx = it + s + RING - 1;
                if (nx < NG) load_a(A[(s + RING - 1) % RING], mt0, nx);
                else load_a(A[(s + RING - 1) % RING], mt_next, nx - NG);
                load_b(Bv[(s + 1) & 1], min(it + s + 1, NG - 1));
                __builtin_amdgcn_sched_barrier(0);
#pragma unroll
                for (int kk = 0; kk < 4; ++kk)
#pragma unroll
                    for (int i = 0; i < MT; ++i)
#pragma unroll
                        for (int j = 0; j < NT; ++j)
                            acc[i][j] = __builtin_amdgcn_mfma_f32_32x32x2f32(A[s][i][kk], Bv[s & 1][kk][j], acc[i][j], 0, 0, 0);
                __builtin_amdgcn_sched_barrier(0);
            }
        }
#pragma unroll
        for (int i = 0; i < MT; ++i) {
            const int m0 = (mt0 + i) * 32;
            float bi[16];
#pragma unroll
            for (int r = 0; r < 16; ++r) bi[r] = ldg(a.bias, (unsigned)(m0 + acc_row(r, lane)));
#pragma unroll
            for (int j = 0; j < NT; ++j) {
                const long t = t0 + j * 32 + l31;
                const long yo = col_y(t < ncol ? t : ncol - 1);
#pragma unroll
                for (int r = 0; r < 16; ++r)
                    if (t < ncol) yb[yo + (long)(m0 + acc_row(r, lane)) * T] = acc[i][j][r] + bi[r];
            }
        }
    }
}

}

extern "C" int cmtts_launch_cond_gemm(const CondGemmArgs* ap, void* stream_) {
    const CondGemmArgs& a = *ap;
    if (a.K != K || a.M % (32 * MT * NW) != 0 || (long)a.M * a.T >= (1L << 30) || a.B <= 0 || a.T <= 0) return -2;
    if (a.flat && (long)a.B * a.T >= (1L << 30)) return -2;
    if (!a.force && (long)((a.T + FN - 1) / FN) * a.B < 128) return -2;
    static bool attr_set = false;
    const size_t lds = (size_t)K * X_LD * sizeof(float);
    if (!attr_set) {
        if (hipFuncSetAttribute(reinterpret_cast<const void*>(cond_gemm_kernel), hipFuncAttributeMaxDynamicSharedMemorySize,
                                (int)lds) != hipSuccess)
            return -3;
        attr_set = true;
    }
    const int zsplit = a.row_split > 1 ? a.row_split : 1;
    const dim3 grid = a.flat ? dim3((unsigned)(((long)a.B * a.T + FN - 1) / FN), 1, zsplit) : dim3((a.T + FN - 1) / FN, a.B, zsplit);
    hipLaunchKernelGGL(cond_gemm_kernel, grid, dim3(64 * NW), lds, (hipStream_t)stream_, a);
    return hipGetLastError() == hipSuccess ? 0 : -3;
}

namespace {
constexpr int CEX_ROWS = 64;
template <int V>
__global__ __launch_bounds__(256) void cond_expand_kernel(const float* __restrict__ p1, int ldp, int L, const float* __restrict__ p2, int ld2,
                                                          const int64_t* __restrict__ mel2ph, const int64_t* __restrict__ pidx,
                                                          float* __restrict__ cp, int M, int T) {
    const int t = (blockIdx.x * 64 + (threadIdx.x & 63)) * V;
    const int r0 = blockIdx.y * CEX_ROWS + (threadIdx.x >> 6) * (CEX_ROWS / 4), b = blockIdx.z;
    if (t >= T) return;
    int ph[V], ix[V];
#pragma unroll
    for (int e = 0; e < V; ++e) {
        const int64_t p64 = mel2ph[(long)b * T + t + e];
        ph[e] = (int)(p64 > L ? L : p64);
        const int i = (int)pidx[(long)b * T + t + e];
        ix[e] = i < 0 ? 0 : (i >= ld2 ? ld2 - 1 : i);
    }
    const float* a = p1 + ((long)b * M + r0) * ldp;
    const float* q = p2 + (long)r0 * ld2;
    float* o = cp + ((long)b * M + r0) * T + t;
#pragma unroll 1
    for (int r = 0; r < CEX_ROWS / 4; r += 4) {
        float av[4][V], qv[4][V];
#pragma unroll
        for (int j = 0; j < 4; ++j)
#pragma unroll
            for (int e = 0; e < V; ++e) {
                av[j][e] = a[(long)(r + j) * ldp + (ph[e] > 0 ? ph[e] - 1 : 0)];
                qv[j][e] = q[(long)(r + j) * ld2 + ix[e]];
            }
#pragma unroll
        for (int j = 0; j < 4; ++j) {
            if (V == 4) {
                f32x4 v;
#pragma unroll
                for (int e = 0; e < 4; ++e) v[e] = (ph[e] > 0 ? av[j][e] : 0.f) + qv[j][e];
                *reinterpret_cast<f32x4*>(o + (long)(r + j) * T) = v;
            } else {
                o[(long)(r + j) * T] = (ph[0] > 0 ? av[j][0] : 0.f) + qv[j][0];
            }
        }
    }
}
}

extern "C" int cmtts_launch_cond_expand(const float* p1, int ldp, int L, const float* p2, int ld2, const int64_t* mel2ph, const int64_t* pidx,
                                        float* cp, int B, int M, int T, void* stream_) {
    if (M % CEX_ROWS != 0 || B <= 0 || T <= 0 || L <= 0) return -2;
    if ((T & 3) == 0 && ((uintptr_t)cp & 15) == 0)
        hipLaunchKernelGGL(cond_expand_kernel<4>, dim3((T / 4 + 63) / 64, M / CEX_ROWS, B), dim3(256), 0, (hipStream_t)stream_, p1, ldp, L, p2, ld2,
                           mel2ph, pidx, cp, M, T);
    else
        hipLaunchKernelGGL(cond_expand_kernel<1>, dim3((T + 63) / 64, M / CEX_ROWS, B), dim3(256), 0, (hipStream_t)stream_, p1, ldp, L, p2, ld2,
                           mel2ph, pidx, cp, M, T);
    return hipGetLastError() == hipSuccess ? 0 : -3;
}
```

cm-tts_amd/csrc/conv_k5q.hip:

```cpp
#include <hip/hip_runtime.h>
#include <stdint.h>
#include "resblock_pair.h"
#include "xcd_map.h"
#ifndef XCD_MAP
#define XCD_MAP 1
#endif

namespace {

typedef float f32x4 __attribute__((ext_vector_type(4)));
typedef float f32x2 __attribute__((ext_vector_type(2)));

constexpr int CO = 256;
constexpr int KT = 5, PAD = 2;
constexpr int BN = 64;
constexpr int XIN = BN + KT;
constexpr int XW = 72;
constexpr int NPT = 12;
constexpr int NV = XW / 4;
constexpr int R = 4;
constexpr int U = 2;

template <int CIN, bool LN>
__global__ __launch_bounds__(256, 2) void conv_k5q_kernel(const ConvXlArgs a) {
    constexpr int NKS = CIN / 4;
    static_assert(NKS % U == 0, "k-steps per round");
    extern __shared__ __attribute__((aligned(16))) float Xs[];
    const int tid = threadIdx.x, lane = tid & 63, nthr = blockDim.x;
    const int wl = __builtin_amdgcn_readfirstlane(tid >> 6), nwv = nthr >> 6;
    const int w = blockIdx.z * nwv + wl;
    int bx_ = blockIdx.x, by_ = blockIdx.y;
    if (XCD_MAP) xcd_tile(bx_, by_);
    const int b = by_;
    const int t0 = bx_ * BN;
    const int T = a.T;
    const float* xb = a.x + (long)b * (a.cin ? a.xbstride : a.bstride);
    float* gs = Xs + CIN * XW;
    if (LN) {
        for (int i = tid; i < 256; i += nthr) { gs[i] = a.ln_g[i]; gs[256 + i] = a.ln_b[i]; }
    }
    {
        const int tbase = t0 - PAD;
        constexpr int total = CIN * NV;
#pragma unroll 1
        for (int base = tid; base < total; base += nthr * NV) {
            f32x4 v[NV];
#pragma unroll
            for (int u = 0; u < NV; ++u) {
                const int idx = min(base + u * nthr, total - 1), r = idx / NV, q = idx - r * NV;
                const int t = tbase + 4 * q;
                const float* src = xb + (long)r * a.ld;
                if (t >= 0 && t + 3 < T) v[u] = *reinterpret_cast<const f32x4*>(src + t);
                else {
#pragma unroll
                    for (int c = 0; c < 4; ++c) v[u][c] = src[min(max(t + c, 0), T - 1)];
                }
            }
#pragma unroll
            for (int u = 0; u < NV; ++u) {
                const int idx = base + u * nthr;
                if (idx < total) {
                    const int r = idx / NV, q = idx - r * NV;
                    const int t = tbase + 4 * q;
                    f32x4 o;
#pragma unroll
                    for (int c = 0; c < 4; ++c) o[c] = (4 * q + c < XIN && t + c >= 0 && t + c < T) ? v[u][c] : 0.f;
                    *reinterpret_cast<f32x4*>(Xs + r * XW + 4 * q) = o;
                }
            }
        }
    }
    __syncthreads();
    if constexpr (LN) {
        static_assert(!LN || CIN == 256, "LayerNorm prologue: 256 channels");
        const int l31 = lane & 31, khalf = lane >> 5;
        for (int cb = 32 * wl; cb < XW; cb += 32 * nwv) {
            const int c = cb + l31;
            const int t = t0 - PAD + c;
            const bool live = c < XIN && t >= 0 && t < T;
            const float* cr = Xs + min(c, XW - 1) + 4 * khalf * XW;
            float p[4] = {0.f, 0.f, 0.f, 0.f}, q[4];
#pragma unroll 8
            for (int i2 = 0; i2 < 32; ++i2)
#pragma unroll
                for (int y = 0; y < 4; ++y) p[y] += cr[(y + 8 * i2) * XW];
#pragma unroll
            for (int y = 0; y < 4; ++y) q[y] = __shfl_xor(p[y], 32);
            float tot = 0.f;
#pragma unroll
            for (int y = 0; y < 4; ++y) tot += khalf ? q[y] : p[y];
#pragma unroll
            for (int y = 0; y < 4; ++y) tot += khalf ? p[y] : q[y];
            const float mean = tot / 256.0f;
#pragma unroll
            for (int y = 0; y < 4; ++y) p[y] = 0.f;
#pragma unroll 8
            for (int i2 = 0; i2 < 32; ++i2)
#pragma unroll
                for (int y = 0; y < 4; ++y) { const float d = cr[(y + 8 * i2) * XW] - mean; p[y] = __fmaf_rn(d, d, p[y]); }
#pragma unroll
            for (int y = 0; y < 4; ++y) q[y] = __shfl_xor(p[y], 32);
            float var = 0.f;
#pragma unroll
            for (int y = 0; y < 4; ++y) var += khalf ? q[y] : p[y];
#pragma unroll
            for (int y = 0; y < 4; ++y) var += khalf ? p[y] : q[y];
            var = var / 256.0f;
            const float rstd = 1.0f / sqrtf(var + a.ln_eps);
            if (live) {
                float* wc = Xs + c + 4 * khalf * XW;
                const float* g = gs + 4 * khalf;
                const float* be = gs + 256 + 4 * khalf;
#pragma unroll 1
                for (int i0 = 0; i0 < 32; i0 += 4) {
                    float xv[16], gv[16], bv[16];
#pragma unroll
                    for (int e = 0; e < 16; ++e) {
                        const int k = (e & 3) + 8 * (i0 + (e >> 2));
                        xv[e] = wc[k * XW]; gv[e] = g[k]; bv[e] = be[k];
                    }
#pragma unroll
                    for (int e = 0; e < 16; ++e) {
                        const int k = (e & 3) + 8 * (i0 + (e >> 2));
                        wc[k * XW] = __fmaf_rn((xv[e] - mean) * rstd, gv[e], bv[e]);
                    }
                }
            }
        }
        __syncthreads();
    }

    f32x4 M[4][6];
#pragma unroll
    for (int i = 0; i < 4; ++i)
#pragma unroll
        for (int p = 0; p < 6; ++p) M[i][p] = f32x4{0.f, 0.f, 0.f, 0.f};
    {
        constexpr int NWVT = CO / 64;
        const __amdgpu_buffer_rsrc_t rs = __builtin_amdgcn_make_buffer_rsrc(const_cast<float*>(a.wf), 0, NKS * NWVT * NPT * 1024, 0x00020000);
        const int voff = lane * 16;
        f32x4 A[R][6];
        auto load_a = [&](f32x4 (&dst)[6], int ks0, int n) {
            const int soff = ((min(ks0 + n / 2, NKS - 1) * NWVT + w) * NPT + 6 * (n % 2)) * 1024;
#pragma unroll
            for (int p = 0; p < 6; ++p) dst[p] = __builtin_bit_cast(f32x4, __builtin_amdgcn_raw_buffer_load_b128(rs, voff + p * 1024, soff, 0));
        };
        const float* xl = Xs + (lane >> 4) * XW + 4 * (lane & 15);
        float D[2][6];
        auto load_d = [&](float (&d)[6], int ks0, int n) {
            const float* r = xl + min(ks0 + n / 2, NKS - 1) * (4 * XW);
            if (n % 2 == 0) {
                const f32x4 p = *reinterpret_cast<const f32x4*>(r);
                const f32x2 q = *reinterpret_cast<const f32x2*>(r + 4);
                d[0] = p[0]; d[1] = p[1]; d[2] = p[2]; d[3] = p[3]; d[4] = q.x; d[5] = q.y;
            } else {
                const f32x4 p = *reinterpret_cast<const f32x4*>(r + 4);
                d[0] = r[3]; d[1] = p[0]; d[2] = p[1]; d[3] = p[2]; d[4] = p[3]; d[5] = r[8];
            }
        };
#pragma unroll
        for (int s = 0; s < R - 1; ++s) load_a(A[s], 0, s);
        load_d(D[0], 0, 0);
#pragma unroll 1
        for (int ks0 = 0; ks0 < NKS; ks0 += U) {
#pragma unroll
            for (int n = 0; n < U * 2; ++n) {
                const int slot = n % R;
                float V[6];
                {
                    const float (&d)[6] = D[n & 1];
                    const f32x2 P01 = {d[0], d[1]}, P23 = {d[2], d[3]}, P45 = {d[4], d[5]};
                    const f32x2 c4 = {4.f, 4.f}, cm5 = {-5.f, -5.f}, c2 = {2.f, -2.f};
                    const f32x2 V05 = __builtin_elementwise_fma(c4, P01, __builtin_elementwise_fma(cm5, P23, P45));
                    const float u0 = __builtin_fmaf(-4.f, d[2], d[4]), u1 = __builtin_fmaf(-4.f, d[1], d[3]);
                    const float u2 = d[4] - d[2], u3 = d[3] - d[1];
                    const f32x2 a0 = {u0, u0}, a1 = {u1, -u1}, b0 = {u2, u2}, b1 = {u3, u3};
                    const f32x2 V12 = a0 + a1;
                    const f32x2 V34 = __builtin_elementwise_fma(c2, b1, b0);
                    V[0] = V05.x; V[1] = V12.x; V[2] = V12.y; V[3] = V34.x; V[4] = V34.y; V[5] = V05.y;
                }
                __builtin_amdgcn_sched_barrier(0);
                load_a(A[(slot + R - 1) % R], ks0, n + R - 1);
                load_d(D[(n + 1) & 1], ks0, n + 1);
#pragma unroll
                for (int p = 0; p < 6; ++p)
#pragma unroll
                    for (int i = 0; i < 4; ++i) M[i][p] = __builtin_amdgcn_mfma_f32_16x16x4f32(A[slot][p][i], V[p], M[i][p], 0, 0, 0);
                __builtin_amdgcn_sched_barrier(0);
            }
        }
    }

    float* yb = a.y + (long)b * a.bstride;
    const int q4 = lane & 15, rq = lane >> 4;
    const int tq = t0 + 4 * q4;
    const bool vec = ((a.ld & 3) == 0) && ((reinterpret_cast<size_t>(yb) & 15) == 0) && tq + 3 < T;
#pragma unroll
    for (int i = 0; i < 4; ++i) {
        float bi[4];
#pragma unroll
        for (int r = 0; r < 4; ++r) bi[r] = a.bias[w * 64 + 16 * i + 4 * rq + r];
#pragma unroll
        for (int r = 0; r < 4; ++r) {
            const int row = w * 64 + 16 * i + 4 * rq + r;
            const float m0 = M[i][0][r], m1 = M[i][1][r], m2 = M[i][2][r], m3 = M[i][3][r], m4 = M[i][4][r], m5 = M[i][5][r];
            const float s12 = m1 + m2, d12 = m1 - m2, s34 = m3 + m4, d34 = m3 - m4;
            f32x4 y;
            y[0] = ((m0 + s12) + s34) + bi[r];
            y[1] = __builtin_fmaf(2.f, d34, d12) + bi[r];
            y[2] = __builtin_fmaf(4.f, s34, s12) + bi[r];
            y[3] = (__builtin_fmaf(8.f, d34, d12) + m5) + bi[r];
            if (a.relu) {
#pragma unroll
                for (int c = 0; c < 4; ++c) y[c] = y[c] > 0.f ? y[c] : 0.f;
            }
            const long o = (long)row * a.ld + tq;
            if (vec) *reinterpret_cast<f32x4*>(yb + o) = y;
            else {
#pragma unroll
                for (int c = 0; c < 4; ++c)
                    if (tq + c < T) yb[o + c] = y[c];
            }
        }
    }
}

template <int CIN, bool LN>
int launch_k5q(const ConvXlArgs& a, hipStream_t stream) {
    const size_t lds = ((size_t)CIN * XW + (LN ? 512 : 0)) * sizeof(float);
    static bool attr_set = false;
    if (!attr_set) {
        if (hipFuncSetAttribute(reinterpret_cast<const void*>(conv_k5q_kernel<CIN, LN>), hipFuncAttributeMaxDynamicSharedMemorySize, (int)lds) != hipSuccess) return -3;
        attr_set = true;
    }
    const long tiles = (long)((a.T + BN - 1) / BN) * a.B;
    const int split = a.row_split == 1 || a.row_split == 2 || a.row_split == 4 ? a.row_split : (tiles >= 128 ? 1 : tiles >= 64 ? 2 : 4);
    dim3 grid((a.T + BN - 1) / BN, a.B, split);
    hipLaunchKernelGGL((conv_k5q_kernel<CIN, LN>), grid, dim3(256 / split), lds, stream, a);
    return hipGetLastError() == hipSuccess ? 0 : -3;
}

}

extern "C" int cmtts_launch_conv_k5q(const ConvXlArgs* a, void* stream_) {
    hipStream_t s = (hipStream_t)stream_;
    if (a->C != CO || a->k != KT || a->dil != 1 || a->T < 1 || a->B < 1 || a->res || a->accum || a->slope != 1.0f || !a->wf || !a->bias) return -2;
    const int cin = a->cin ? a->cin : a->C;
    if (a->ln_g && (!a->ln_b || cin != 256)) return -2;
    if (cin == 256) return a->ln_g ? launch_k5q<256, true>(*a, s) : launch_k5q<256, false>(*a, s);
    if (cin == 128 && !a->ln_g) return launch_k5q<128, false>(*a, s);
    return -2;
}
```

cm-tts_amd/csrc/conv_xres.hip:

```cpp
#include <hip/hip_runtime.h>
#include <stdlib.h>
#include "conv_args.h"
#include "conv_epilogue.h"

typedef float f32x4 __attribute__((ext_vector_type(4)));
typedef float f32x2 __attribute__((ext_vector_type(2)));

namespace {

#ifndef XRES_OCC1
#define XRES_OCC1 2
#endif
constexpr int KMAX = 256;
constexpr int HALO = 8;
constexpr int RING = 4;

template <bool LN, int NT, int WQ = 0>
__global__ __launch_bounds__(256, NT == 1 ? XRES_OCC1 : 1) void conv_xres_kernel(const ConvArgs a, const float* __restrict__ wfrag, long long* dbg) {
    constexpr int BN = 32 * NT;
    constexpr int X_LD = BN + HALO;
    extern __shared__ __attribute__((aligned(16))) float xs[];
    const int tid = threadIdx.x, lane = tid & 63, w = tid >> 6;
    auto stamp = [&](int slot) {
        if (dbg && lane == 0)
            dbg[((((long)blockIdx.z * gridDim.y + blockIdx.y) * gridDim.x + blockIdx.x) * 4 + w) * 8 + slot] =
                (long long)__builtin_readcyclecounter();
    };
    stamp(0);
    int by = blockIdx.y, bz = blockIdx.z;
    if (gridDim.x == 1 && (gridDim.z & 7) == 0) {
        const int lin = blockIdx.y + gridDim.y * blockIdx.z;
        const int slot = lin >> 3;
        by = slot % gridDim.y;
        bz = (lin & 7) + 8 * (slot / gridDim.y);
    }
    const int n0 = blockIdx.x * BN;
    const int mt = by * 4 + w;
    const int z = bz;
    if (LN && a.ln_skip_tiles && a.ln_lens && n0 > 0 && (int64_t)n0 >= a.ln_lens[z]) return;
    const int l31 = lane & 31, khalf = lane >> 5;
    const float* Xb = a.X + z * a.x_zs0;
    const int MTn = (a.M + 31) / 32;
    const int total = (a.K / 16) * a.taps * 2;

    const int mtc = min(mt, MTn - 1);
    const float* wl = wfrag + ((long)mtc * 64 + lane) * 4;
    auto load_a = [&](f32x4& dst, int it) {
        dst = *reinterpret_cast<const f32x4*>(wl + (long)min(it, total - 1) * MTn * 256);
    };
    f32x4 A[RING];
    if constexpr (WQ == 0) {
#pragma unroll
        for (int s = 0; s < RING - 1; ++s) load_a(A[s], s);
    }

    const int xw = BN + (a.taps - 1) * a.dil;
    float* gs = xs + a.K * X_LD;
    if (LN) { gs[tid] = a.ln_g[tid]; gs[256 + tid] = a.ln_b[tid]; }
    if (((n0 - a.pad) & 3) == 0 && (a.ldx & 3) == 0 && ((uintptr_t)Xb & 15) == 0) {
        constexpr int V = X_LD / 4, U = NT == 3 ? 26 : 10;
        const int nvec = a.K * V;
        const int t00 = n0 - a.pad;
#pragma unroll 1
        for (int base = tid; base < nvec; base += 256 * U) {
            f32x4 v[U];
#pragma unroll
            for (int u = 0; u < U; ++u) {
                const int idx = min(base + 256 * u, nvec - 1);
                const int row = idx / V, c4 = idx - row * V;
                const int t4 = min(max(t00 + 4 * c4, 0), a.ldx - 4);
                v[u] = *reinterpret_cast<const f32x4*>(Xb + (long)row * a.ldx + t4);
            }
#pragma unroll
            for (int u = 0; u < U; ++u) {
                const int idx = base + 256 * u;
                if (idx < nvec) {
                    const int row = idx / V, c4 = idx - row * V;
                    const int c = 4 * c4, t = t00 + c;
                    f32x4 o;
#pragma unroll
                    for (int e = 0; e < 4; ++e) o[e] = (c + e < xw && t + e >= 0 && t + e < a.Tin) ? v[u][e] : 0.f;
                    *reinterpret_cast<f32x4*>(xs + row * X_LD + c) = o;
                }
            }
        }
    } else {
        const int rows = a.K / 4;
#pragma unroll
        for (int cp = 0; cp < 2; ++cp) {
            const int c = lane + 64 * cp;
            const int t = n0 - a.pad + c;
            const bool ok = c < xw && t >= 0 && t < a.Tin;
            const int tc = min(max(t, 0), a.Tin - 1);
            if (c < X_LD) {
#pragma unroll 1
                for (int k0 = w * rows; k0 < (w + 1) * rows; k0 += 32) {
                    float v[32];
#pragma unroll
                    for (int q = 0; q < 32; ++q) v[q] = Xb[(long)min(k0 + q, a.K - 1) * a.ldx + tc];
#pragma unroll
                    for (int q = 0; q < 32; ++q)
                        if (k0 + q < (w + 1) * rows) xs[(k0 + q) * X_LD + c] = ok ? v[q] : 0.f;
                }
            }
        }
    }
    stamp(1);
    __syncthreads();
    if (LN) {
        const int c = 32 * w + l31;
        const int t = n0 - a.pad + c;
        const bool live = c < xw && t >= 0 && t < a.Tin;
        const bool on = live && !(a.ln_lens && (int64_t)t >= a.ln_lens[z]);
        const float* col = xs + min(c, X_LD - 1);
        float p[4] = {0.f, 0.f, 0.f, 0.f}, q[4];
        const float* cr = col + 4 * khalf * X_LD;
#pragma unroll 8
        for (int i2 = 0; i2 < 32; ++i2)
#pragma unroll
            for (int y = 0; y < 4; ++y) p[y] += cr[(y + 8 * i2) * X_LD];
#pragma unroll
        for (int y = 0; y < 4; ++y) q[y] = __shfl_xor(p[y], 32);
        float tot = 0.f;
#pragma unroll
        for (int y = 0; y < 4; ++y) tot += khalf ? q[y] : p[y];
#pragma unroll
        for (int y = 0; y < 4; ++y) tot += khalf ? p[y] : q[y];
        const float mean = tot / 256.0f;
#pragma unroll
        for (int y = 0; y < 4; ++y) p[y] = 0.f;
#pragma unroll 8
        for (int i2 = 0; i2 < 32; ++i2)
#pragma unroll
            for (int y = 0; y < 4; ++y) { const float d = cr[(y + 8 * i2) * X_LD] - mean; p[y] = __fmaf_rn(d, d, p[y]); }
#pragma unroll
        for (int y = 0; y < 4; ++y) q[y] = __shfl_xor(p[y], 32);
        float var = 0.f;
#pragma unroll
        for (int y = 0; y < 4; ++y) var += khalf ? q[y] : p[y];
#pragma unroll
        for (int y = 0; y < 4; ++y) var += khalf ? p[y] : q[y];
        var = var / 256.0f;
        const float rstd = 1.0f / sqrtf(var + a.ln_eps);
        if (on) {
            float* wc = xs + c + 4 * khalf * X_LD;
            const float* g = gs + 4 * khalf;
            const float* be = gs + 256 + 4 * khalf;
#pragma unroll 1
            for (int i0 = 0; i0 < 32; i0 += 4) {
                float xv[16], gv[16], bv[16];
#pragma unroll
                for (int e = 0; e < 16; ++e) {
                    const int k = (e & 3) + 8 * (i0 + (e >> 2));
                    xv[e] = wc[k * X_LD]; gv[e] = g[k]; bv[e] = be[k];
                }
#pragma unroll
                for (int e = 0; e < 16; ++e) {
                    const int k = (e & 3) + 8 * (i0 + (e >> 2));
                    wc[k * X_LD] = __fmaf_rn((xv[e] - mean) * rstd, gv[e], bv[e]);
                }
            }
        } else if (live) {
            float* wc = xs + c + 4 * khalf * X_LD;
#pragma unroll 8
            for (int i2 = 0; i2 < 32; ++i2)
#pragma unroll
                for (int y = 0; y < 4; ++y) wc[(y + 8 * i2) * X_LD] = 0.f;
        }
        __syncthreads();
    }
    stamp(2);

    constexpr int NTQ = NT == 3 ? 2 : 1;
    f32x4 Mq[WQ == 1 ? 2 : 1][WQ == 1 ? NTQ : 1][6];
    f32x4 Mp[WQ == 2 ? 2 : 1][WQ == 2 ? NT : 1][4];
    f32x16 acc[NT];
#pragma unroll
    for (int j = 0; j < NT; ++j)
#pragma unroll
        for (int r = 0; r < 16; ++r) acc[j][r] = 0.f;
    const float* bl = xs + khalf * X_LD + l31;
    if constexpr (WQ == 2) {
#pragma unroll
        for (int i = 0; i < 2; ++i)
#pragma unroll
            for (int nt = 0; nt < NT; ++nt)
#pragma unroll
                for (int p = 0; p < 4; ++p) Mp[i][nt][p] = f32x4{0.f, 0.f, 0.f, 0.f};
        constexpr int R = 3, U = 2;
        const int NKS = a.K / 4;
        const __amdgpu_buffer_rsrc_t rs = __builtin_amdgcn_make_buffer_rsrc(const_cast<float*>(wfrag), 0, NKS * MTn * 6 * 1024, 0x00020000);
        const int voff = lane * 16;
        const int mtu = __builtin_amdgcn_readfirstlane(mtc);
        f32x4 Ap[R][2];
        auto load_ap = [&](f32x4 (&dst)[2], int ks0, int n) {
            const int soff = ((min(ks0 + n / 3, NKS - 1) * MTn + mtu) * 3 + (n % 3)) * 2048;
#pragma unroll
            for (int j = 0; j < 2; ++j) dst[j] = __builtin_bit_cast(f32x4, __builtin_amdgcn_raw_buffer_load_b128(rs, voff + j * 1024, soff, 0));
        };
        const float* xl = xs + (lane >> 4) * X_LD + 2 * (lane & 15);
        float D[2][NT][4];
        auto load_dp = [&](float (&d)[NT][4], int ks0, int n) {
            const int g = n % 3;
#pragma unroll
            for (int nt = 0; nt < NT; ++nt) {
                const float* r = xl + min(ks0 + n / 3, NKS - 1) * (4 * X_LD) + nt * 32;
                if (g == 1) {
                    const f32x2 q = *reinterpret_cast<const f32x2*>(r + 4);
                    d[nt][0] = r[3]; d[nt][1] = q.x; d[nt][2] = q.y; d[nt][3] = r[6];
                } else {
                    const f32x2 p = *reinterpret_cast<const f32x2*>(r + 3 * g), q = *reinterpret_cast<const f32x2*>(r + 3 * g + 2);
// ... 167 lines not shown
#pragma unroll
                    for (int nt = 0; nt < NT; ++nt) {
                        const float m0 = Mp[i][nt][0][r], m1 = Mp[i][nt][1][r], m2 = Mp[i][nt][2][r], m3 = Mp[i][nt][3][r];
                        f32x2 y;
                        y.x = (m0 + m1) + m2;
                        y.y = (m1 - m2) - m3;
#pragma unroll
                        for (int c = 0; c < 2; ++c) {
                            float v = y[c];
                            if (o.bias) v += bq;
                            v *= o.alpha;
                            y[c] = act_apply(v, ACT_GELU_ERF);
                        }
                        *reinterpret_cast<f32x2*>(xs + rowl * X_LD + 2 * (p16 + 16 * nt)) = y;
                    }
                }
        } else if constexpr (WQ == 1) {
            const int q4 = lane & 15, rq = lane >> 4;
#pragma unroll
            for (int i = 0; i < 2; ++i)
#pragma unroll
                for (int r = 0; r < 4; ++r) {
                    const int rowl = w * 32 + 16 * i + 4 * rq + r;
                    const float bq = o.bias ? o.bias[(unsigned)(mt * 32 + 16 * i + 4 * rq + r)] : 0.f;
#pragma unroll
                    for (int nt = 0; nt < NTQ; ++nt) {
                        const float m0 = Mq[i][nt][0][r], m1 = Mq[i][nt][1][r], m2 = Mq[i][nt][2][r], m3 = Mq[i][nt][3][r], m4 = Mq[i][nt][4][r], m5 = Mq[i][nt][5][r];
                        const float s12 = m1 + m2, d12 = m1 - m2, s34 = m3 + m4, d34 = m3 - m4;
                        f32x4 y;
                        y[0] = (m0 + s12) + s34;
                        y[1] = __builtin_fmaf(2.f, d34, d12);
                        y[2] = __builtin_fmaf(4.f, s34, s12);
                        y[3] = __builtin_fmaf(8.f, d34, d12) + m5;
#pragma unroll
                        for (int c = 0; c < 4; ++c) {
                            float v = y[c];
                            if (o.bias) v += bq;
                            v *= o.alpha;
                            y[c] = act_apply(v, ACT_GELU_ERF);
                        }
                        const int col = 4 * (q4 + 16 * nt);
                        if (col < BN) *reinterpret_cast<f32x4*>(xs + rowl * X_LD + col) = y;
                    }
                }
        } else {
#pragma unroll
        for (int j = 0; j < NT; ++j)
#pragma unroll
            for (int r = 0; r < 16; ++r) {
                float v = acc[j][r];
                if (o.bias) v += bi[r];
                v *= o.alpha;
                v = act_apply(v, ACT_GELU_ERF);
                xs[(w * 32 + (r & 3) + 8 * (r >> 2) + 4 * khalf) * X_LD + j * 32 + l31] = v;
            }
        }
        __syncthreads();
        f32x16 acc2[2][NT];
#pragma unroll
        for (int i = 0; i < 2; ++i)
#pragma unroll
            for (int j = 0; j < NT; ++j)
#pragma unroll
                for (int r = 0; r < 16; ++r) acc2[i][j][r] = 0.f;
#pragma unroll
        for (int it = 0; it < 16; ++it)
#pragma unroll
            for (int kk = 0; kk < 4; ++kk) {
                float b2[NT];
#pragma unroll
                for (int j = 0; j < NT; ++j) b2[j] = bl[(it * 8 + 2 * kk) * X_LD + j * 32];
#pragma unroll
                for (int i = 0; i < 2; ++i)
#pragma unroll
                    for (int j = 0; j < NT; ++j)
                        acc2[i][j] = __builtin_amdgcn_mfma_f32_32x32x2f32(A2[it][i][kk], b2[j], acc2[i][j], 0, 0, 0);
            }
        float* pb = a.part + z * a.part_zs0 + by * a.part_zs1;
#pragma unroll
        for (int i = 0; i < 2; ++i)
#pragma unroll
            for (int j = 0; j < NT; ++j) {
                const int n = n0 + j * 32 + l31;
                if (n < a.N && n < o.Tout) {
#pragma unroll
                    for (int r = 0; r < 16; ++r)
                        pb[(unsigned)((2 * w + i) * 32 + (r & 3) + 8 * (r >> 2) + 4 * khalf) * (unsigned)a.part_ld + (unsigned)n] = acc2[i][j][r] * 1.0f;
                }
            }
        stamp(4);
        return;
    }
    if (mt >= MTn) return;
    if (epi_simple(o) && o.act == ACT_GELU_ERF) {
#pragma unroll
        for (int j = 0; j < NT; ++j) epi_tile_simple<ACT_GELU_ERF>(o, acc[j], mt * 32, 4 * khalf, n0 + j * 32 + l31, a.M, a.N, z);
    } else if (epi_simple(o) && o.act == ACT_RELU) {
#pragma unroll
        for (int j = 0; j < NT; ++j) epi_tile_simple<ACT_RELU>(o, acc[j], mt * 32, 4 * khalf, n0 + j * 32 + l31, a.M, a.N, z);
    } else if (epi_simple(o) && o.act == ACT_NONE) {
#pragma unroll
        for (int j = 0; j < NT; ++j) epi_tile_simple<ACT_NONE>(o, acc[j], mt * 32, 4 * khalf, n0 + j * 32 + l31, a.M, a.N, z);
    } else {
#pragma unroll
        for (int j = 0; j < NT; ++j) epi_tile(o, acc[j], mt * 32, 4 * khalf, n0 + j * 32 + l31, a.M, a.N, z, 0);
    }
    stamp(4);
}

long long* g_xres_dbg = nullptr;
int g_xres_nt = 0;

}

extern "C" void cmtts_xres_set_debug(long long* dbg) { g_xres_dbg = dbg; }
extern "C" int cmtts_xres_set_nt(int nt) { const int p = g_xres_nt; if (nt == 0 || nt == 1 || nt == 3) g_xres_nt = nt; return p; }

extern "C" int cmtts_launch_conv_xres(const ConvArgs* ap, const float* wfrag, int nbatch, void* stream_) {
    const ConvArgs& a = *ap;
    if (a.M <= 0 || a.N <= 0 || nbatch <= 0) return 0;
    if (!wfrag || a.zdiv != 1 || a.split != INT_MAX || a.dil <= 0 || a.K % 32 != 0 || a.K > KMAX || (a.taps - 1) * a.dil > HALO ||
        a.pre_div != 1.0f || a.pre_slope != 1.0f)
        return -2;
    if (a.ln_g && (!a.ln_b || a.K != 256)) return -2;
    if (a.w2frag) {
        const ConvOut& o = a.out[0];
        if (!a.part || a.M2 != 256 || a.M % 128 != 0 || a.K < 128 || o.ostride != 1 || o.ooff_base || o.ooff_mul || o.row_off || o.div != 1.0f || o.accum || o.bvec || o.act != ACT_GELU_ERF || o.res || o.lens) return -2;
    }
    const int mblocks = ((a.M + 31) / 32 + 3) / 4;
    const long wg96 = (long)((a.N + 95) / 96) * mblocks * nbatch;
    const int nt = a.xres_nt == 1 || a.xres_nt == 3 ? a.xres_nt : (g_xres_nt == 1 || g_xres_nt == 3 ? g_xres_nt : (wg96 >= 128 ? 3 : 1));
    const int bn = 32 * nt, x_ld = bn + HALO;
    static bool attr_set = false;
    const size_t lds = (size_t)a.K * x_ld * sizeof(float) + (a.ln_g ? 2 * 256 * sizeof(float) : 0);
    if (!attr_set) {
        const int mx = (int)((size_t)KMAX * (96 + HALO) * sizeof(float) + 2 * 256 * sizeof(float));
        if (hipFuncSetAttribute(reinterpret_cast<const void*>(conv_xres_kernel<false, 3>), hipFuncAttributeMaxDynamicSharedMemorySize, mx) != hipSuccess ||
            hipFuncSetAttribute(reinterpret_cast<const void*>(conv_xres_kernel<true, 3>), hipFuncAttributeMaxDynamicSharedMemorySize, mx) != hipSuccess ||
            hipFuncSetAttribute(reinterpret_cast<const void*>(conv_xres_kernel<false, 1>), hipFuncAttributeMaxDynamicSharedMemorySize, mx) != hipSuccess ||
            hipFuncSetAttribute(reinterpret_cast<const void*>(conv_xres_kernel<true, 1>), hipFuncAttributeMaxDynamicSharedMemorySize, mx) != hipSuccess)
            return -3;
        attr_set = true;
    }
    dim3 grid((a.N + bn - 1) / bn, mblocks, nbatch);
    long long* dbg = g_xres_dbg;
    if (dbg) {
        static const char* want = getenv("CMTTS_XRES_DBG_M");
        if (want && atoi(want) != a.M) dbg = nullptr;
    }
    hipStream_t st = (hipStream_t)stream_;
    if (dbg) {
        static const char* twice = getenv("CMTTS_XRES_DBG_TWICE");
        if (twice && atoi(twice) == 1 && a.out[0].res != a.out[0].Y && !a.w2frag) {
            if (nt == 3) { if (a.ln_g) hipLaunchKernelGGL((conv_xres_kernel<true, 3>), grid, dim3(256), lds, st, a, wfrag, nullptr); else hipLaunchKernelGGL((conv_xres_kernel<false, 3>), grid, dim3(256), lds, st, a, wfrag, nullptr); }
            else { if (a.ln_g) hipLaunchKernelGGL((conv_xres_kernel<true, 1>), grid, dim3(256), lds, st, a, wfrag, nullptr); else hipLaunchKernelGGL((conv_xres_kernel<false, 1>), grid, dim3(256), lds, st, a, wfrag, nullptr); }
        }
    }
    if (nt == 3) {
        if (a.ln_g) hipLaunchKernelGGL((conv_xres_kernel<true, 3>), grid, dim3(256), lds, st, a, wfrag, dbg);
        else hipLaunchKernelGGL((conv_xres_kernel<false, 3>), grid, dim3(256), lds, st, a, wfrag, dbg);
    } else {
        if (a.ln_g) hipLaunchKernelGGL((conv_xres_kernel<true, 1>), grid, dim3(256), lds, st, a, wfrag, dbg);
        else hipLaunchKernelGGL((conv_xres_kernel<false, 1>), grid, dim3(256), lds, st, a, wfrag, dbg);
    }
    return hipGetLastError() == hipSuccess ? 0 : -3;
}

extern "C" int cmtts_launch_conv_xresq(const ConvArgs* ap, const float* wfrag, int nbatch, void* stream_, int form) {
    const ConvArgs& a = *ap;
    if (a.M <= 0 || a.N <= 0 || nbatch <= 0) return 0;
    if (!wfrag || a.zdiv != 1 || a.split != INT_MAX || a.dil <= 0 || a.K % 32 != 0 || a.K > KMAX || (a.taps - 1) * a.dil > HALO ||
        a.pre_div != 1.0f || a.pre_slope != 1.0f)
        return -2;
    if (a.ln_g && (!a.ln_b || a.K != 256)) return -2;
    if (!a.w2frag || a.taps != 9 || a.dil != 1 || a.pad != 4 || a.K != 256) return -2;
    if (a.w2frag) {
        const ConvOut& o = a.out[0];
        if (!a.part || a.M2 != 256 || a.M % 128 != 0 || a.K < 128 || o.ostride != 1 || o.ooff_base || o.ooff_mul || o.row_off || o.div != 1.0f || o.accum || o.bvec || o.act != ACT_GELU_ERF || o.res || o.lens) return -2;
    }
    const int mblocks = ((a.M + 31) / 32 + 3) / 4;
    const long wg96 = (long)((a.N + 95) / 96) * mblocks * nbatch;
    const int nt = a.xres_nt == 1 || a.xres_nt == 3 ? a.xres_nt : (g_xres_nt == 1 || g_xres_nt == 3 ? g_xres_nt : (wg96 >= 128 ? 3 : 1));
    const int bn = 32 * nt, x_ld = bn + HALO;
    static bool attr_set = false;
    const size_t lds = (size_t)a.K * x_ld * sizeof(float) + (a.ln_g ? 2 * 256 * sizeof(float) : 0);
    if (!attr_set) {
        const int mx = (int)((size_t)KMAX * (96 + HALO) * sizeof(float) + 2 * 256 * sizeof(float));
        if (hipFuncSetAttribute(reinterpret_cast<const void*>(conv_xres_kernel<false, 3, 1>), hipFuncAttributeMaxDynamicSharedMemorySize, mx) != hipSuccess ||
            hipFuncSetAttribute(reinterpret_cast<const void*>(conv_xres_kernel<true, 3, 1>), hipFuncAttributeMaxDynamicSharedMemorySize, mx) != hipSuccess ||
            hipFuncSetAttribute(reinterpret_cast<const void*>(conv_xres_kernel<false, 1, 1>), hipFuncAttributeMaxDynamicSharedMemorySize, mx) != hipSuccess ||
            hipFuncSetAttribute(reinterpret_cast<const void*>(conv_xres_kernel<true, 1, 1>), hipFuncAttributeMaxDynamicSharedMemorySize, mx) != hipSuccess ||
            hipFuncSetAttribute(reinterpret_cast<const void*>(conv_xres_kernel<false, 3, 2>), hipFuncAttributeMaxDynamicSharedMemorySize, mx) != hipSuccess ||
            hipFuncSetAttribute(reinterpret_cast<const void*>(conv_xres_kernel<true, 3, 2>), hipFuncAttributeMaxDynamicSharedMemorySize, mx) != hipSuccess ||
            hipFuncSetAttribute(reinterpret_cast<const void*>(conv_xres_kernel<false, 1, 2>), hipFuncAttributeMaxDynamicSharedMemorySize, mx) != hipSuccess ||
            hipFuncSetAttribute(reinterpret_cast<const void*>(conv_xres_kernel<true, 1, 2>), hipFuncAttributeMaxDynamicSharedMemorySize, mx) != hipSuccess)
            return -3;
        attr_set = true;
    }
    dim3 grid((a.N + bn - 1) / bn, mblocks, nbatch);
    long long* dbg = g_xres_dbg;
    if (dbg) {
        static const char* want = getenv("CMTTS_XRES_DBG_M");
        if (want && atoi(want) != a.M) dbg = nullptr;
    }
    hipStream_t st = (hipStream_t)stream_;
    if (form == 2) {
        if (nt == 3) {
            if (a.ln_g) hipLaunchKernelGGL((conv_xres_kernel<true, 3, 2>), grid, dim3(256), lds, st, a, wfrag, dbg);
            else hipLaunchKernelGGL((conv_xres_kernel<false, 3, 2>), grid, dim3(256), lds, st, a, wfrag, dbg);
        } else {
            if (a.ln_g) hipLaunchKernelGGL((conv_xres_kernel<true, 1, 2>), grid, dim3(256), lds, st, a, wfrag, dbg);
            else hipLaunchKernelGGL((conv_xres_kernel<false, 1, 2>), grid, dim3(256), lds, st, a, wfrag, dbg);
        }
    } else if (nt == 3) {
        if (a.ln_g) hipLaunchKernelGGL((conv_xres_kernel<true, 3, 1>), grid, dim3(256), lds, st, a, wfrag, dbg);
        else hipLaunchKernelGGL((conv_xres_kernel<false, 3, 1>), grid, dim3(256), lds, st, a, wfrag, dbg);
    } else {
        if (a.ln_g) hipLaunchKernelGGL((conv_xres_kernel<true, 1, 1>), grid, dim3(256), lds, st, a, wfrag, dbg);
        else hipLaunchKernelGGL((conv_xres_kernel<false, 1, 1>), grid, dim3(256), lds, st, a, wfrag, dbg);
    }
    return hipGetLastError() == hipSuccess ? 0 : -3;
}
```

cm-tts_amd/csrc/internal_hooks.h:

```cpp
#pragma once
#ifdef __cplusplus
extern "C" {
#endif
int cmtts_internal_set(const char* name, int value);
struct cmtts_model;
int cmtts_internal_cond_projections(struct cmtts_model* m, const float* cond_ct, int B, int T, float* cp, void* stream);
int cmtts_internal_cond_factored(struct cmtts_model* m, const float* p1, int p1_ld, int L, const int64_t* mel2ph, const int64_t* p_idx, int B, int T,
                                 float* cp, void* stream);
int cmtts_internal_mel_window_gather(const float* mel_ct, int B, int T, const int32_t* windows, int N, int Tw, float* out, void* stream);
#ifdef __cplusplus
}
#endif
```

cm-tts_amd/csrc/kernels.hip:

```cpp
#include <hip/hip_runtime.h>
#include <math.h>
#include <stdint.h>
#include "kernels.h"

namespace {

__device__ __forceinline__ float sin_exact(float a) { return (float)sin((double)a); }
__device__ __forceinline__ float cos_exact(float a) { return (float)cos((double)a); }

__device__ __forceinline__ float pos_embed(int p, int c, int C, const float* omega, const float* tab, int tab_rows) {
    if (p == 0) return 0.f;
    if (p < tab_rows) return tab[(long)p * C + c];
    const int half = C >> 1;
    const int j = c < half ? c : c - half;
    const float arg = (float)p * omega[j];
    return c < half ? sin_exact(arg) : cos_exact(arg);
}

template <typename FlagFn>
__device__ void block_positions(FlagFn flag, int T, int* pos, int* counts) {
    const int tid = threadIdx.x;
    const int seg = (T + 255) / 256;
    const int start = tid * seg;
    const int end = min(T, start + seg);
    int cnt = 0;
    for (int t = start; t < end; ++t) cnt += flag(t) ? 1 : 0;
    counts[tid] = cnt;
    __syncthreads();
    if (tid == 0) {
        int run = 0;
        for (int i = 0; i < 256; ++i) { const int c = counts[i]; counts[i] = run; run += c; }
    }
    __syncthreads();
    int run = counts[tid];
    for (int t = start; t < end; ++t) {
        const bool f = flag(t);
        run += f ? 1 : 0;
        pos[t] = f ? run : 0;
    }
    __syncthreads();
}

constexpr int EMB_CG = 32;
__global__ __launch_bounds__(256) void embed_tokens_kernel(const int64_t* texts, const int64_t* lens,
                                                           const float* E, const float* omega, const float* tab,
                                                           int tab_rows, float* x, int L, int ld, int C, float scale) {
    extern __shared__ int sh[];
    int* counts = sh;
    int* pos = sh + 256;
    const int b = blockIdx.x;
    const int64_t* tok = texts + (long)b * L;
    block_positions([&](int t) { return tok[t] != 0; }, L, pos, counts);
    const int len = (int)lens[b];
    const int c0 = blockIdx.y * EMB_CG;
    for (int idx = threadIdx.x; idx < EMB_CG * L; idx += 256) {
        const int cl = idx / L, l = idx - cl * L, c = c0 + cl;
        if (c >= C) break;
        float v = 0.f;
        if (l < len) v = scale * E[tok[l] * C + c] + pos_embed(pos[l], c, C, omega, tab, tab_rows);
        x[((long)b * C + c) * ld + l] = v;
    }
}

__global__ __launch_bounds__(256) void layernorm_ct_kernel(const float* in, float* out, const float* gamma,
                                                           const float* beta, float eps, const int64_t* lens,
                                                           int T, int ld) {
    constexpr int C = 256;
    const int lane = threadIdx.x & 63, w = threadIdx.x >> 6;
    const int tx = lane & 7, ty = lane >> 3;
    const int t = blockIdx.x * 32 + w * 8 + tx;
    const int b = blockIdx.y;
    const bool ok = t < T;
    float v[32];
    float sum = 0.f;
#pragma unroll
    for (int i = 0; i < 32; ++i) {
        const int c = ty + 8 * i;
        v[i] = ok ? in[((long)b * C + c) * ld + t] : 0.f;
        sum += v[i];
    }
    float tot = 0.f;
#pragma unroll
    for (int y = 0; y < 8; ++y) tot += __shfl(sum, y * 8 + tx);
    const float mean = tot / (float)C;
    float sq = 0.f;
#pragma unroll
    for (int i = 0; i < 32; ++i) { const float d = v[i] - mean; sq = __fmaf_rn(d, d, sq); }
    float var = 0.f;
#pragma unroll
    for (int y = 0; y < 8; ++y) var += __shfl(sq, y * 8 + tx);
    var = var / (float)C;
    const float rstd = 1.0f / sqrtf(var + eps);
    const bool keep = !(lens && (int64_t)t >= lens[b]);
    if (ok) {
#pragma unroll
        for (int i = 0; i < 32; ++i) {
            const int c = ty + 8 * i;
            const float y = __fmaf_rn((v[i] - mean) * rstd, gamma[c], beta[c]);
            out[((long)b * C + c) * ld + t] = keep ? y : 0.f;
        }
    }
}

__global__ __launch_bounds__(256) void softmax_cols_kernel(float* st, const int64_t* lens, int H, int L, int ld, long zs) {
    __shared__ float red[4][64];
    const int il = threadIdx.x & 63, sl = threadIdx.x >> 6;
    const int i = blockIdx.x * 64 + il;
    const int z = blockIdx.y;
    const int len = min((int)lens[z / H], L);
    float* col = st + (long)z * zs + min(i, L - 1);
    float mx = -INFINITY;
    for (int j = sl; j < len; j += 4) mx = fmaxf(mx, col[(long)j * ld]);
    red[sl][il] = mx;
    __syncthreads();
    mx = fmaxf(fmaxf(red[0][il], red[1][il]), fmaxf(red[2][il], red[3][il]));
    __syncthreads();
    float sum = 0.f;
    for (int j = sl; j < len; j += 4) sum += expf(col[(long)j * ld] - mx);
    red[sl][il] = sum;
    __syncthreads();
    sum = (red[0][il] + red[1][il]) + (red[2][il] + red[3][il]);
    if (i >= L) return;
    for (int j = sl; j < len; j += 4) col[(long)j * ld] = expf(col[(long)j * ld] - mx) / sum;
    for (int j = len + sl; j < L; j += 4) col[(long)j * ld] = 0.f;
}

__global__ void add_rowvec_kernel(float* x, const float* vec, int C, int L, int ld, const int64_t* lens) {
    const int l = blockIdx.x * blockDim.x + threadIdx.x;
    const int c = blockIdx.y, b = blockIdx.z;
    if (l < L && !(lens && (int64_t)l >= lens[b])) x[((long)b * C + c) * ld + l] += vec[(long)b * C + c];
}

constexpr int POS_CG = 8;
__global__ __launch_bounds__(256) void pos_embed_add_kernel(const float* x, float* out, const float* alpha,
                                                            const float* omega, const float* tab, int tab_rows,
                                                            int C, int T, int ld, const int64_t* lens) {
    extern __shared__ int sh[];
    int* counts = sh;
    int* pos = sh + 256;
    const int b = blockIdx.x;
    const float* x0 = x + (long)b * C * ld;
    block_positions([&](int t) { return x0[t] != 0.f; }, T, pos, counts);
    const float al = alpha[0];
    const int c0 = blockIdx.y * POS_CG;
    const int valid = lens ? (int)min((int64_t)T, lens[b]) : T;
    for (int cl = 0; cl < POS_CG && c0 + cl < C; ++cl) {
        const int c = c0 + cl;
        for (int t = threadIdx.x; t < T; t += 256) {
            const long off = ((long)b * C + c) * ld + t;
            const float v = x[off] + al * pos_embed(pos[t], c, C, omega, tab, tab_rows);
            out[off] = t < valid ? v : 0.f;
        }
    }
}

__global__ __launch_bounds__(256) void pos_embed_add_lr_kernel(const float* src, int ldl, const int64_t* mel2ph, const float* padv, float* out,
                                                               const float* alpha, const float* omega, const float* tab, int tab_rows,
                                                               int C, int T) {
    extern __shared__ int sh[];
    int* counts = sh;
    int* pos = sh + 256;
    const int b = blockIdx.x;
    const int64_t* mp = mel2ph + (long)b * T;
    const float* s0 = src + (long)b * C * ldl;
    const float pad0 = padv[0];
    block_positions([&](int t) { const int64_t ph = mp[t]; return (ph > 0 ? s0[ph - 1] : pad0) != 0.f; }, T, pos, counts);
    const float al = alpha[0];
    const int c0 = blockIdx.y * POS_CG;
    for (int cl = 0; cl < POS_CG && c0 + cl < C; ++cl) {
        const int c = c0 + cl;
        const float* sc = s0 + (long)c * ldl;
        const float pc = padv[c];
        for (int t = threadIdx.x; t < T; t += 256) {
            const int64_t ph = mp[t];
            const float xv = ph > 0 ? sc[ph - 1] : pc;
            out[((long)b * C + c) * T + t] = xv + al * pos_embed(pos[t], c, C, omega, tab, tab_rows);
        }
    }
}

__global__ __launch_bounds__(256) void chan_linear_kernel(const float* x, const float* W, const float* bias,
                                                          float* out, const int64_t* lens, int C, int T, int ld, int O) {
    extern __shared__ float wsh[];
    float* part = wsh + O * C;
    for (int i = threadIdx.x; i < O * C; i += 256) wsh[i] = W[i];
    __syncthreads();
    const int tl = threadIdx.x & 63, cs = threadIdx.x >> 6;
    const int t = blockIdx.x * 64 + tl;
    const int b = blockIdx.y;
    const int tc = min(t, T - 1);
    const int cq = C / 4, c0 = cs * cq;
    float acc[16];
#pragma unroll
    for (int o = 0; o < 16; ++o) acc[o] = 0.f;
    const float* xb = x + (long)b * C * ld + tc;
#pragma unroll 8
    for (int c = c0; c < c0 + cq; ++c) {
        const float xv = xb[(long)c * ld];
#pragma unroll
        for (int o = 0; o < 16; ++o)
            if (o < O) acc[o] = fmaf(xv, wsh[o * C + c], acc[o]);
    }
    if (cs > 0) {
#pragma unroll
        for (int o = 0; o < 16; ++o)
            if (o < O) part[((cs - 1) * 16 + o) * 64 + tl] = acc[o];
    }
    __syncthreads();
    if (cs == 0 && t < T) {
        const bool keep = !(lens && (int64_t)t >= lens[b]);
#pragma unroll
        for (int o = 0; o < 16; ++o)
            if (o < O) {
                const float v = ((acc[o] + part[(0 * 16 + o) * 64 + tl]) + part[(1 * 16 + o) * 64 + tl]) + part[(2 * 16 + o) * 64 + tl];
                out[((long)b * T + t) * O + o] = keep ? v + bias[o] : 0.f;
            }
    }
}

constexpr int LNL_PAD = 65;
struct EnergyEpi {
    const float* xin;
    const float* e_target;
    float e_control;
    const float* bins;
    int nbins;
    const float* E;
    float* out1;
    int64_t* e_idx;
    float* e_scaled;
    const float* e_table;
};
template <int O, int EE = 0>
__global__ __launch_bounds__(256) void ln_linear_kernel(const float* __restrict__ x, const float* __restrict__ gamma,
                                                        const float* __restrict__ beta, float eps, const float* __restrict__ W,
                                                        const float* __restrict__ bias, float* __restrict__ out,
                                                        const int64_t* ln_lens, const int64_t* out_lens, int T, int ld, const EnergyEpi ee = EnergyEpi{}) {
    constexpr int C = 256, CQ = 64;
    constexpr int NV = (O + 2) * C / 4;
    constexpr int PER = (NV + 255) / 256;
    __shared__ float lsm[(O + 2) * 4 * LNL_PAD];
    {
        float4 wv[PER];
#pragma unroll
        for (int u = 0; u < PER; ++u) {
            const int i4 = min((int)threadIdx.x + 256 * u, NV - 1);
            const int r = i4 >> 6, c4 = i4 & 63;
            const float* src = r < O ? W + (long)r * C : (r == O ? gamma : beta);
            wv[u] = *reinterpret_cast<const float4*>(src + 4 * c4);
        }
#pragma unroll
        for (int u = 0; u < PER; ++u) {
            const int i4 = threadIdx.x + 256 * u;
            if (i4 < NV) {
                const int r = i4 >> 6, c = 4 * (i4 & 63);
                float* d = lsm + (r * 4 + (c >> 6)) * LNL_PAD + (c & 63);
                d[0] = wv[u].x; d[1] = wv[u].y; d[2] = wv[u].z; d[3] = wv[u].w;
            }
        }
    }
    const int lane = threadIdx.x & 63, w = threadIdx.x >> 6;
    const int col = lane & 15, q = lane >> 4;
    const int t = blockIdx.x * 64 + w * 16 + col;
    const int b = blockIdx.y;
    const int tc = min(t, T - 1);
    const float* xb = x + ((long)b * C + q * CQ) * ld + tc;
    float v[CQ];
#pragma unroll
    for (int i = 0; i < CQ; ++i) v[i] = xb[(long)i * ld];
    __syncthreads();
    float s = 0.f;
#pragma unroll
    for (int i = 0; i < CQ; ++i) s += v[i];
    s += __shfl_xor(s, 16);
    s += __shfl_xor(s, 32);
    const float mean = s / (float)C;
    float sq = 0.f;
#pragma unroll
    for (int i = 0; i < CQ; ++i) { const float d = v[i] - mean; sq = __fmaf_rn(d, d, sq); }
    sq += __shfl_xor(sq, 16);
    sq += __shfl_xor(sq, 32);
    const float rstd = 1.0f / sqrtf(sq / (float)C + eps);
    const bool ln_keep = !(ln_lens && (int64_t)t >= ln_lens[b]);
    float acc[O];
#pragma unroll
    for (int o = 0; o < O; ++o) acc[o] = 0.f;
    const float* wq = lsm + q * LNL_PAD;
#pragma unroll
    for (int i = 0; i < CQ; ++i) {
        float y = __fmaf_rn((v[i] - mean) * rstd, wq[(O * 4) * LNL_PAD + i], wq[((O + 1) * 4) * LNL_PAD + i]);
        if (!ln_keep) y = 0.f;
#pragma unroll
        for (int o = 0; o < O; ++o) acc[o] = __fmaf_rn(y, wq[(o * 4) * LNL_PAD + i], acc[o]);
    }
#pragma unroll
    for (int o = 0; o < O; ++o) {
        acc[o] += __shfl_xor(acc[o], 16);
        acc[o] += __shfl_xor(acc[o], 32);
    }
    const bool keep = !(out_lens && (int64_t)t >= out_lens[b]);
    if (q == 0 && t < T) {
#pragma unroll
        for (int o = 0; o < O; ++o) out[((long)b * T + t) * O + o] = keep ? acc[o] + bias[o] : 0.f;
    }
    if constexpr (EE) {
        static_assert(EE == 0 || O == 1, "energy head");
        if (t < T) {
            const float pred = keep ? acc[0] + bias[0] : 0.f;
            float v;
            if (ee.e_target) v = ee.e_target[(long)b * T + t];
            else if constexpr (EE == 2) { v = pred * ee.e_table[(long)b * T + t]; if (q == 0) ee.e_scaled[(long)b * T + t] = v; }
            else { v = pred * ee.e_control; if (q == 0 && ee.e_control != 1.0f) ee.e_scaled[(long)b * T + t] = v; }
            int lo = 0, hi = ee.nbins;
            while (lo < hi) { const int mid = (lo + hi) >> 1; if (ee.bins[mid] >= v) hi = mid; else lo = mid + 1; }
            if (v != v) lo = ee.nbins;
            if (q == 0) ee.e_idx[(long)b * T + t] = lo;
            const float* e = ee.E + (long)lo * C + q * CQ;
            const float* xi = ee.xin + ((long)b * C + q * CQ) * ld + t;
            float* o1 = ee.out1 + ((long)b * C + q * CQ) * ld + t;
            float xv[CQ], ev[CQ];
#pragma unroll
            for (int i = 0; i < CQ; ++i) { xv[i] = xi[(long)i * ld]; ev[i] = e[i]; }
#pragma unroll
            for (int i = 0; i < CQ; ++i) o1[(long)i * ld] = xv[i] + ev[i];
        }
        else if (t < ld) {
            float* o1 = ee.out1 + ((long)b * C + q * CQ) * ld + t;
#pragma unroll
            for (int i = 0; i < CQ; ++i) o1[(long)i * ld] = 0.f;
// ... 687 lines not shown
```

Measured before the change: 1.963 million.

## Fuse positional embedding into predictor first convs and skip redundant step embeddings

Folds the length-regulated gather plus positional-embedding add into the first pitch-predictor conv (k5q gather variant), and folds the energy-predictor positional embedding into the xres conv. Has the conditioner GEMM write the transposed phoneme factor directly instead of running a separate transpose. Reuses cached per-sigma step-embedding rows, which skips the step-embedding computation and the side-stream fork when a row is ready. Each piece removes a kernel launch or an intermediate round trip through memory, at the cost of more kernel variants and more complex dispatch conditions.

New measurement: 1.963 million. No clear change (-0.0%).

```diff
diff --git a/cm-tts_amd/csrc/cmtts_api.hip b/cm-tts_amd/csrc/cmtts_api.hip
--- a/cm-tts_amd/csrc/cmtts_api.hip
+++ b/cm-tts_amd/csrc/cmtts_api.hip
@@ -18,6 +18,8 @@
 #include "persist_args.h"
 #include "cond_gemm.h"
 #include "resblock_pair.h"
+#include "conv_k5q.h"
+#include "conv_xres_pe.h"
 #include "inproj.h"
 #include "attention.h"
 #include "text_state.h"
@@ -1140,9 +1142,16 @@
 int g_energy_head = 1;
 int g_pred_wino = 1;
 int g_pred_xres = 1;
+struct LrInput {
+    const float* src; int ldl; const int64_t* mel2ph; const float* pad; float* hp; const float* alpha; const float* omega; const float* tab; int C;
+    int kind = 1;
+};
+int g_xres_pe = 1;
+int g_k5q_gather = 1;
 int predictor(const Predictor& P, const float* in, int ld_in, int B, int T, int ld, const int64_t* ln_lens,
               const int64_t* out_lens, float* bufA, float* bufB, float* out, int O, hipStream_t s, int mode16 = 0, bool frame_level = false,
-              EnergyHead* eh = nullptr) {
+              EnergyHead* eh = nullptr,
+              const LrInput* lri = nullptr) {
     const float* cur = in;
     int ldc = ld_in;
     auto other = [&](const float* p) { return p == bufA ? bufB : bufA; };
@@ -1159,21 +1168,33 @@
             xa.B = B; xa.C = 256; xa.T = T; xa.ld = ld; xa.k = w.taps; xa.dil = 1; xa.slope = 1.0f; xa.relu = 1;
             if (w.cin != 256) { xa.cin = w.cin; xa.xbstride = (long)w.cin * ldc; }
             if (pend_ln >= 0) { xa.ln_g = P.ln_g[pend_ln]; xa.ln_b = P.ln_b[pend_ln]; xa.ln_eps = 1e-12f; }
-            if (ldc == ld || w.cin != 256) {
+            if (li == 0 && lri && lri->kind == 1 && w.cin == 128 && lri->C == 128) {
+                const K5qGather kg{lri->mel2ph, lri->src, lri->pad, lri->ldl, lri->alpha, lri->omega, lri->tab, PE_ROWS};
+                rx = cmtts_launch_conv_k5q_lr(&xa, &kg, (void*)s);
+            } else if (!(li == 0 && lri && lri->kind == 1) && (ldc == ld || w.cin != 256)) {
                 rx = cmtts_launch_conv_k5q(&xa, (void*)s);
-                if (rx == -3) return fail(CMTTS_E_HIP, "conv_k5q launch failed");
-                if (rx == 0) pend_ln = -2;
             }
-        }
+            if (rx == -3) return fail(CMTTS_E_HIP, "conv_k5q launch failed");
+            if (rx == 0) pend_ln = -2;
+        }
+        if (li == 0 && lri && lri->kind == 1 && rx != 0)
+            k_pos_embed_add_lr(lri->src, lri->ldl, lri->mel2ph, lri->pad, lri->hp, lri->alpha, lri->omega, lri->tab, PE_ROWS, B, lri->C, T, s);
         const bool small = (long)((T + 63) / 64) * B < 192;
         if (rx != 0 && !mode16 && g_pred_xres && small && P.convs_f[li] && w.cin == 256 && w.cout == 256 && ldc == ld) {
             ConvArgs a = conv_args(w, cur, T, ldc, (long)w.cin * ldc, dst, ld, (long)w.cout * ld, T);
             a.out[0].act = ACT_RELU;
             a.xres_nt = 1;
             if (pend_ln >= 0) { a.ln_g = P.ln_g[pend_ln]; a.ln_b = P.ln_b[pend_ln]; a.ln_eps = 1e-12f; a.ln_lens = ln_lens; a.ln_skip_tiles = 1; }
-            rx = cmtts_launch_conv_xres(&a, P.convs_f[li], B, (void*)s);
+            if (li == 0 && lri && lri->kind == 2) {
+                const XresPe pe{lri->alpha, lri->omega, lri->tab, PE_ROWS};
+                rx = cmtts_launch_conv_xres_pe(&a, P.convs_f[li], B, (void*)s, &pe);
+            } else rx = cmtts_launch_conv_xres(&a, P.convs_f[li], B, (void*)s);
             if (rx == -3) return fail(CMTTS_E_HIP, "conv_xres launch failed");
             if (rx == 0) pend_ln = -2;
+        }
+        if (li == 0 && lri && lri->kind == 2 && rx != 0) {
+            k_pos_embed_add(lri->src, lri->hp, lri->alpha, lri->omega, lri->tab, PE_ROWS, B, lri->C, T, lri->ldl, s);
+            cur = lri->hp;
         }
         if (pend_ln >= 0) {
             float* nd = other(cur);
@@ -1268,12 +1289,13 @@
     const int r = cmtts_launch_cond_expand(f.p1, f.ldp, f.L, m->cond_p2, c.pitch_bins, f.mel2ph, f.p_idx, w.cp, B, c.res_layers * c.res_channels, T, (void*)s);
     return r == 0 ? 0 : fail(CMTTS_E_HIP, "cond_expand launch failed");
 }
-int cond_phoneme_factor(cmtts_model* m, const float* out1, int B, int Lp, float* p1, hipStream_t s) {
+int g_cond_gemm_t = 1;
+int cond_phoneme_factor(cmtts_model* m, const float* out1, int B, int Lp, float* p1, float* p1t, hipStream_t s) {
     const cmtts_config& c = m->cfg;
     if (!m->cond_p2) return fail(CMTTS_E_UNSUPPORTED, "factored conditioner projections are not available for this model");
     CondGemmArgs g;
     memset(&g, 0, sizeof(g));
-    g.X = out1; g.Wf = m->cond_all_f; g.bias = m->cond_zero_bias; g.Y = p1;
+    g.X = out1; g.Wf = m->cond_all_f; g.bias = m->cond_zero_bias; g.Y = p1; g.Yt = p1t;
     g.B = B; g.T = Lp; g.M = c.res_layers * c.res_channels; g.K = c.hidden; g.force = 1;
     g.flat = 1;
     const long tiles = ((long)B * Lp + 63) / 64;
@@ -1291,6 +1313,13 @@
     return r == 0 ? 0 : fail(r == -2 ? CMTTS_E_UNSUPPORTED : CMTTS_E_HIP, "cond_gemm (phoneme factor) launch failed");
 }
 
+int g_step_row_direct = 1;
+const float* step_row_lookup(const cmtts_model* m, float t_host) {
+    if (!g_step_row_direct || !g_step_cache || m->cfg.multi_speaker || t_host != t_host) return nullptr;
+    for (const cmtts_model::StepRow& e : m->step_rows)
+        if (e.t == t_host && hipEventQuery(e.ready) == hipSuccess) return e.row;
+    return nullptr;
+}
 int step_embedding(cmtts_model* m, const DenWs& w, const float* timesteps, const float* spk, int B, hipStream_t s,
                    float t_host = NAN) {
     const cmtts_config& c = m->cfg;
@@ -1384,7 +1413,8 @@
 int denoiser_core(cmtts_model* m, const DenWs& w, const float* x_src, float in_scale, const float* timesteps,
                   const float* cond_ct, const float* spk, int B, int T, const MelPost& post, hipStream_t s, bool embed = true,
                   SideStream* pending = nullptr, float t_host = NAN,
-                  const CondFactors* cfk = nullptr, bool* cp_ready = nullptr) {
+                  const CondFactors* cfk = nullptr, bool* cp_ready = nullptr,
+                  const float* drow = nullptr) {
     CHK(check_device_flag(true));
     const cmtts_config& c = m->cfg;
     const int C = c.res_channels, NL = c.res_layers, M = c.n_mels;
@@ -1402,6 +1432,7 @@
         memset(&pa, 0, sizeof(pa));
         pa.x0 = w.h; pa.cp = w.cp; pa.cp_bstride = (long)NL * C * T;
         pa.dp = dp; pa.d = w.dproj; pa.vec_stride = (long)NL * C;
+        if (drow) { pa.dp = pa.d = drow; pa.vec_stride = 0; }
         pa.skip = w.skip; pa.halo = w.halo; pa.tmo = g_tmo_host;
         pa.B = B; pa.T = T; pa.NL = NL;
         pa.halo_zeroed = halo_zeroed;
@@ -1440,6 +1471,7 @@
             if (pa.tail) return 0;
         }
     }
+    if (!layers_done && drow) k_broadcast_row(drow, w.dproj, B, NL * C, s);
     if (!layers_done && cfk && !(cp_ready && *cp_ready)) {
         CHK(cond_factored(m, w, *cfk, B, T, s));
         if (cp_ready) *cp_ready = true;
@@ -1808,9 +1840,11 @@
     if (ct.p) HIPCHK(hipMemcpyAsync(w.pctl, ct.p, (size_t)B * L * 4, hipMemcpyDeviceToDevice, s));
     if (enc_out_ct && !c.multi_speaker)
         k_copy_rows(enc_out_ct, L, w.x, Lp, L, (long)B * H, s);
-    k_pos_embed_add(w.x, w.h, m->energy.alpha, m->omega_h, m->pe_h, PE_ROWS, B, H, L, Lp, se);
+    LrInput epe{w.x, Lp, nullptr, nullptr, w.h, m->energy.alpha, m->omega_h, m->pe_h, H, 2};
+    if (!g_xres_pe) k_pos_embed_add(w.x, w.h, m->energy.alpha, m->omega_h, m->pe_h, PE_ROWS, B, H, L, Lp, se);
     EnergyHead eh{w.x, m->vc.e_target, m->vc.e_control, m->energy_bins, c.energy_bins - 1, m->energy_emb, w.out1, e_idx, w.escaled, false, ct.e};
-    CHK(predictor(m->energy, w.h, Lp, B, L, Lp, pad_lens, pad_lens, ec1, ec2, e_pred, 1, se, t16mode, false, H == 256 ? &eh : nullptr));
+    CHK(predictor(m->energy, g_xres_pe ? w.x : w.h, Lp, B, L, Lp, pad_lens, pad_lens, ec1, ec2, e_pred, 1, se, t16mode, false, H == 256 ? &eh : nullptr,
+                  g_xres_pe ? &epe : nullptr));
     if (ss) CHK(branch_join(ss));
     if (!eh.done)
         k_energy_embed(w.x, e_pred, w.escaled, m->vc.e_target, m->vc.e_control, m->energy_bins, c.energy_bins - 1, m->energy_emb,
@@ -1876,8 +1910,9 @@
     if (ss) CHK(branch_fork(ss));
     if (cond_p1t && !cond_p1) return fail(CMTTS_E_INVALID, "cmtts_frame_forward_sub_t: cond_p1t needs cond_p1");
     if (cond_p1 && m->cond_p2) {
-        CHK(cond_phoneme_factor(m, tw.out1, B, Lp, cond_p1, sst));
-        if (cond_p1t) k_transpose(cond_p1, cond_p1t, B * c.res_layers, c.res_channels, Lp, sst);
+        const bool gemm_t = cond_p1t && g_cond_gemm_t && C_IS_256(c) && ((uintptr_t)cond_p1t & 15) == 0;
+        CHK(cond_phoneme_factor(m, tw.out1, B, Lp, cond_p1, gemm_t ? cond_p1t : nullptr, sst));
+        if (cond_p1t && !gemm_t) k_transpose(cond_p1, cond_p1t, B * c.res_layers, c.res_channels, Lp, sst);
     }
     if (!(g_stats_mlp && k_stats_mlp(tw.out1, (long)H * Lp, Lp, m->st0_wt, m->st0_b, m->st2_wt, m->st2_b, m->st4_wt, m->st4_b, f0_stats, B, H, CH, CH, 2, sst))) {
         k_dense_small(tw.out1, (long)H * Lp, Lp, m->st0_wt, m->st0_b, nullptr, w.s1, B, H, CH, DENSE_RELU, sst);
@@ -1887,15 +1922,18 @@
     k_mel2ph(tw.cum, mel2ph, B, L, T, s);
     if (!g_cwt_in_phoneme) k_length_regulate(tw.out1, mel2ph, w.xlr, B, H, Lp, T, s);
     bool hp_done = false;
+    LrInput lri{};
     if (g_cwt_in_phoneme) {
-        k_pos_embed_add_lr(tw.h128, Lp, mel2ph, m->cwt_in.bias, w.hp, m->cwt.alpha, m->omega_cwt, m->pe_cwt, PE_ROWS, B, CH, T, s);
+        lri = LrInput{tw.h128, Lp, mel2ph, m->cwt_in.bias, w.hp, m->cwt.alpha, m->omega_cwt, m->pe_cwt, CH};
+        if (!g_k5q_gather) k_pos_embed_add_lr(tw.h128, Lp, mel2ph, m->cwt_in.bias, w.hp, m->cwt.alpha, m->omega_cwt, m->pe_cwt, PE_ROWS, B, CH, T, s);
         hp_done = true;
     } else {
         ConvArgs a = conv_args(m->cwt_in, w.xlr, T, T, (long)H * T, w.h128, T, (long)CH * T, T);
         CHK(launch(a, EPI_PLAIN, B, s));
     }
     if (!hp_done) k_pos_embed_add(w.h128, w.hp, m->cwt.alpha, m->omega_cwt, m->pe_cwt, PE_ROWS, B, CH, T, T, s);
-    CHK(predictor(m->cwt, w.hp, T, B, T, T, nullptr, nullptr, w.c1, w.c2, cwt_out, O, s, (m->text16 && (m->precision == 1 || m->precision == 2)) ? m->precision : 0, true));
+    CHK(predictor(m->cwt, w.hp, T, B, T, T, nullptr, nullptr, w.c1, w.c2, cwt_out, O, s, (m->text16 && (m->precision == 1 || m->precision == 2)) ? m->precision : 0, true,
+                  nullptr, g_cwt_in_phoneme && g_k5q_gather ? &lri : nullptr));
     if (ss) CHK(branch_join(ss));
     if (m->ct.p) k_pitch_table_scale(cwt_out, mel2ph, tw.cum, tw.pctl, B, O, L, T, s);
     else if (m->vc.p_control != 1.0f) k_scale(cwt_out, cwt_out, (long)B * T * O, m->vc.p_control, s);
@@ -2047,15 +2085,17 @@
     const cmtts_config& c = m->cfg;
     const long nel = (long)B * T * c.n_mels;
     SideStream* ss = g_fused_resblock ? side_for(s) : nullptr;
-    if (ss) CHK(branch_fork(ss));
     const CondFactors* cfk = nullptr;
     CondFactors cf_local;
     bool cp_ready = false;
+    const bool cf_ok = g_fused_resblock && cf && cf->usable(m);
+    const bool inkernel = cf_ok && g_cond_inkernel && g_persist && g_persist_tail && m->skip_f && m->outp_f && c.res_layers <= PERSIST_MAX_LAYERS &&
+                          cmtts_persist_plan(B, T, c.res_layers, persist_blocks(), g_persist == 2) > 0 && cf->ldp <= T && m->cond_p2t && C_IS_256(c);
+    if (ss && inkernel && cf->p1t && step_row_lookup(m, 250.0f * logf(sigmas[0] + 1e-44f))) ss = nullptr;
+    if (ss) CHK(branch_fork(ss));
     if (g_fused_resblock) {
-        if (cf && cf->usable(m)) {
-            const bool inkernel = g_cond_inkernel && g_persist && g_persist_tail && m->skip_f && m->outp_f && c.res_layers <= PERSIST_MAX_LAYERS &&
-                                  cmtts_persist_plan(B, T, c.res_layers, persist_blocks(), g_persist == 2) > 0;
-            if (inkernel && cf->ldp <= T && m->cond_p2t && C_IS_256(c)) {
+        if (cf_ok) {
+            if (inkernel) {
                 cf_local = *cf;
                 if (!cf_local.p1t) {
                     k_transpose(cf->p1, w.cp, B * c.res_layers, c.res_channels, cf->ldp, ss ? ss->side : s);
@@ -2067,6 +2107,7 @@
     }
     k_scale(noise, w.xcur, nel, c.sigma_max, s);
     const float smin = c.sigma_min, sd2 = c.sigma_data * c.sigma_data;
+    bool dproj_valid = false;
     for (int i = 0; i < n_steps; ++i) {
         const float sg = sigmas[i];
         const float dm = sg - smin;
@@ -2076,14 +2117,19 @@
         const float c_in = 1.0f / rt;
         const float t_resc = 250.0f * logf(sg + 1e-44f);
         const bool new_sigma = i == 0 || sigmas[i] != sigmas[i - 1];
-        const bool embed_side = i == 0 && ss != nullptr;
-        if (new_sigma) k_fill_float(w.tbuf, t_resc, B, embed_side ? ss->side : s);
+        const float* drow = step_row_lookup(m, t_resc);
+        const bool need_embed = !drow && (new_sigma || !dproj_valid);
+        const bool embed_side = need_embed && i == 0 && ss != nullptr;
+        if (need_embed) k_fill_float(w.tbuf, t_resc, B, embed_side ? ss->side : s);
         if (embed_side) CHK(step_embedding(m, w, w.tbuf, speaker_emb, B, ss->side, t_resc));
+        if (need_embed) dproj_valid = true;
+        else if (new_sigma) dproj_valid = false;
         const bool last = i + 1 == n_steps;
         const bool renoise = renoise_std[i] >= 0.0f;
         const MelPost post = {w.xcur, renoise ? noise + (long)(1 + i) * noise_stride : nullptr, c_out, c_skip,
                               renoise ? renoise_std[i] : 0.0f, last ? mel : w.xcur};
-        CHK(denoiser_core(m, w, w.xcur, c_in, w.tbuf, cond_ct, speaker_emb, B, T, post, s, new_sigma && !embed_side, i == 0 ? ss : nullptr, t_resc, cfk, &cp_ready));
+        CHK(denoiser_core(m, w, w.xcur, c_in, w.tbuf, cond_ct, speaker_emb, B, T, post, s, need_embed && !embed_side, i == 0 ? ss : nullptr, t_resc, cfk, &cp_ready,
+                          drow));
     }
     HIPCHK(hipGetLastError());
     return 0;
@@ -2862,6 +2908,10 @@
         {"energy_head", &g_energy_head, 0, 1},
         {"stats_mlp", &g_stats_mlp, 0, 1},
         {"text_xt16", &g_conv_xt16, 0, 1},
+        {"cond_gemm_t", &g_cond_gemm_t, 0, 1},
+        {"xres_pe", &g_xres_pe, 0, 1},
+        {"k5q_gather", &g_k5q_gather, 0, 1},
+        {"step_row_direct", &g_step_row_direct, 0, 1},
     };
     if (!strcmp(name, "voc_xl_split")) return cmtts_xl_set_split(value);
     if (!strcmp(name, "attn_qb")) return cmtts_attention_set_qb(value);
@@ -2890,6 +2940,31 @@
     CondFactors cf;
     cf.p1 = p1; cf.ldp = p1_ld; cf.L = L; cf.mel2ph = mel2ph; cf.p_idx = p_idx;
     return cond_factored(m, w, cf, B, T, (hipStream_t)stream);
+}
+
+int cmtts_internal_pitch_conv0(cmtts_model* m, const float* h128, int ldl, const int64_t* mel2ph, int B, int T, int gather, float* hp, float* out,
+                               void* stream) {
+    if (!m || !m->finalized || !h128 || !mel2ph || !hp || !out || B <= 0 || T <= 0 || ldl <= 0)
+        return fail(CMTTS_E_INVALID, "cmtts_internal_pitch_conv0: bad argument");
+    const Predictor& P = m->cwt;
+    const int CH = m->cfg.cwt_hidden;
+    if (P.convs.empty() || P.convs_q.empty() || !P.convs_q[0] || P.convs[0].taps != 5 || P.convs[0].cout != 256 || P.convs[0].cin != 128 || CH != 128)
+        return fail(CMTTS_E_UNSUPPORTED, "cmtts_internal_pitch_conv0: no F(4,3) form of the first block");
+    hipStream_t s = (hipStream_t)stream;
+    ConvXlArgs xa;
+    memset(&xa, 0, sizeof(xa));
+    xa.x = hp; xa.y = out; xa.wf = P.convs_q[0]; xa.bias = P.convs[0].bias; xa.bstride = (long)256 * T;
+    xa.B = B; xa.C = 256; xa.T = T; xa.ld = T; xa.k = 5; xa.dil = 1; xa.slope = 1.0f; xa.relu = 1;
+    xa.cin = CH; xa.xbstride = (long)CH * T;
+    int rc;
+    if (gather) {
+        const K5qGather kg{mel2ph, h128, m->cwt_in.bias, ldl, m->cwt.alpha, m->omega_cwt, m->pe_cwt, PE_ROWS};
+        rc = cmtts_launch_conv_k5q_lr(&xa, &kg, (void*)s);
+    } else {
+        k_pos_embed_add_lr(h128, ldl, mel2ph, m->cwt_in.bias, hp, m->cwt.alpha, m->omega_cwt, m->pe_cwt, PE_ROWS, B, CH, T, s);
+        rc = cmtts_launch_conv_k5q(&xa, (void*)s);
+    }
+    return rc == 0 ? 0 : fail(rc == -2 ? CMTTS_E_UNSUPPORTED : CMTTS_E_HIP, "cmtts_internal_pitch_conv0: launch failed");
 }
 
 int cmtts_poll_error(void) { return check_device_flag(); }
diff --git a/cm-tts_amd/csrc/cond_gemm.h b/cm-tts_amd/csrc/cond_gemm.h
--- a/cm-tts_amd/csrc/cond_gemm.h
+++ b/cm-tts_amd/csrc/cond_gemm.h
@@ -9,6 +9,7 @@
     int force;
     int flat;
     int row_split;
+    float* Yt = nullptr;
 };
 
 #ifdef __cplusplus
diff --git a/cm-tts_amd/csrc/cond_gemm.hip b/cm-tts_amd/csrc/cond_gemm.hip
--- a/cm-tts_amd/csrc/cond_gemm.hip
+++ b/cm-tts_amd/csrc/cond_gemm.hip
@@ -1,4 +1,5 @@
 #include <hip/hip_runtime.h>
+#include <stdint.h>
 #include "cond_gemm.h"
 
 typedef float f32x16 __attribute__((ext_vector_type(16)));
@@ -108,9 +109,22 @@
             for (int j = 0; j < NT; ++j) {
                 const long t = t0 + j * 32 + l31;
                 const long yo = col_y(t < ncol ? t : ncol - 1);
-#pragma unroll
-                for (int r = 0; r < 16; ++r)
-                    if (t < ncol) yb[yo + (long)(m0 + acc_row(r, lane)) * T] = acc[i][j][r] + bi[r];
+                if (yb) {
+#pragma unroll
+                    for (int r = 0; r < 16; ++r)
+                        if (t < ncol) yb[yo + (long)(m0 + acc_row(r, lane)) * T] = acc[i][j][r] + bi[r];
+                }
+                if (a.Yt) {
+                    const long tc = t < ncol ? t : ncol - 1;
+                    const long bb = a.flat ? tc / T : (long)blockIdx.y, tt = a.flat ? tc % T : tc;
+                    float* yt = a.Yt + ((bb * (a.M >> 8) + (m0 >> 8)) * T + tt) * 256 + (m0 & 255) + 4 * khalf;
+#pragma unroll
+                    for (int q = 0; q < 4; ++q) {
+                        const f32x4 v = {acc[i][j][4 * q] + bi[4 * q], acc[i][j][4 * q + 1] + bi[4 * q + 1], acc[i][j][4 * q + 2] + bi[4 * q + 2],
+                                         acc[i][j][4 * q + 3] + bi[4 * q + 3]};
+                        if (t < ncol) *reinterpret_cast<f32x4*>(yt + 8 * q) = v;
+                    }
+                }
             }
         }
     }
@@ -122,6 +136,8 @@
     const CondGemmArgs& a = *ap;
     if (a.K != K || a.M % (32 * MT * NW) != 0 || (long)a.M * a.T >= (1L << 30) || a.B <= 0 || a.T <= 0) return -2;
     if (a.flat && (long)a.B * a.T >= (1L << 30)) return -2;
+    if (!a.Y && !a.Yt) return -2;
+    if (a.Yt && (a.M % 256 != 0 || ((uintptr_t)a.Yt & 15) != 0)) return -2;
     if (!a.force && (long)((a.T + FN - 1) / FN) * a.B < 128) return -2;
     static bool attr_set = false;
     const size_t lds = (size_t)K * X_LD * sizeof(float);
diff --git a/cm-tts_amd/csrc/conv_k5q.h b/cm-tts_amd/csrc/conv_k5q.h
--- /dev/null
+++ b/cm-tts_amd/csrc/conv_k5q.h
@@ -0,0 +1,22 @@
+#pragma once
+#include <stdint.h>
+#include "resblock_pair.h"
+
+struct K5qGather {
+    const int64_t* mel2ph;
+    const float* src;
+    const float* pad;
+    int ldl;
+    const float* pe_alpha;
+    const float* pe_omega;
+    const float* pe_tab;
+    int pe_rows;
+};
+
+#ifdef __cplusplus
+extern "C" {
+#endif
+int cmtts_launch_conv_k5q_lr(const ConvXlArgs* a, const K5qGather* g, void* stream);
+#ifdef __cplusplus
+}
+#endif
diff --git a/cm-tts_amd/csrc/conv_k5q.hip b/cm-tts_amd/csrc/conv_k5q.hip
--- a/cm-tts_amd/csrc/conv_k5q.hip
+++ b/cm-tts_amd/csrc/conv_k5q.hip
@@ -2,6 +2,8 @@
 #include <stdint.h>
 #include "resblock_pair.h"
 #include "xcd_map.h"
+#include "pos_embed.h"
+#include "conv_k5q.h"
 #ifndef XCD_MAP
 #define XCD_MAP 1
 #endif
@@ -21,8 +23,8 @@
 constexpr int R = 4;
 constexpr int U = 2;
 
-template <int CIN, bool LN>
-__global__ __launch_bounds__(256, 2) void conv_k5q_kernel(const ConvXlArgs a) {
+template <int CIN, bool LN, bool GATHER>
+__global__ __launch_bounds__(256, 2) void conv_k5q_kernel(const ConvXlArgs a, const K5qGather g) {
     constexpr int NKS = CIN / 4;
     static_assert(NKS % U == 0, "k-steps per round");
     extern __shared__ __attribute__((aligned(16))) float Xs[];
@@ -39,6 +41,51 @@
     if (LN) {
         for (int i = tid; i < 256; i += nthr) { gs[i] = a.ln_g[i]; gs[256 + i] = a.ln_b[i]; }
     }
+    if constexpr (GATHER) {
+        __shared__ int g_ph[XW], g_flag[XW], g_pos[XW], g_cnt[4];
+        const int tbase = t0 - PAD;
+        const int64_t* mp = g.mel2ph + (long)b * T;
+        const float* s0 = g.src + (long)b * CIN * g.ldl;
+        const float pad0 = g.pad[0];
+        auto flag = [&](int t) { const int64_t ph = mp[t]; return (ph > 0 ? s0[ph - 1] : pad0) != 0.f; };
+        int cnt = 0;
+        for (int t = tid; t < tbase; t += nthr) cnt += flag(t) ? 1 : 0;
+#pragma unroll
+        for (int off = 32; off > 0; off >>= 1) cnt += __shfl_xor(cnt, off);
+        if (lane == 0) g_cnt[wl] = cnt;
+        for (int j = tid; j < XW; j += nthr) {
+            const int t = tbase + j;
+            const bool in = j < XIN && t >= 0 && t < T;
+            g_ph[j] = in ? (int)mp[t] : -1;
+            g_flag[j] = in && flag(t) ? 1 : 0;
+        }
+        __syncthreads();
+        int before = 0;
+        for (int i = 0; i < nwv; ++i) before += g_cnt[i];
+        for (int j = tid; j < XW; j += nthr) {
+            int run = before;
+            for (int i = 0; i <= j; ++i) run += g_flag[i];
+            g_pos[j] = g_flag[j] ? run : 0;
+        }
+        __syncthreads();
+        const float al = g.pe_alpha[0];
+        constexpr int total = CIN * NV;
+#pragma unroll 3
+        for (int idx = tid; idx < total; idx += nthr) {
+            const int r = idx / NV, q = idx - r * NV;
+            const float* sc = s0 + (long)r * g.ldl;
+            const float pc = g.pad[r];
+            f32x4 o;
+#pragma unroll
+            for (int c = 0; c < 4; ++c) {
+                const int ph = g_ph[4 * q + c];
+                const float sv = sc[ph > 0 ? ph - 1 : 0];
+                const float xv = ph > 0 ? sv : pc;
+                o[c] = ph >= 0 ? pos_embed_add_value(xv, al, g_pos[4 * q + c], r, CIN, g.pe_omega, g.pe_tab, g.pe_rows) : 0.f;
+            }
+            *reinterpret_cast<f32x4*>(Xs + r * XW + 4 * q) = o;
+        }
+    } else
     {
         const int tbase = t0 - PAD;
         constexpr int total = CIN * NV;
@@ -225,18 +272,18 @@
     }
 }
 
-template <int CIN, bool LN>
-int launch_k5q(const ConvXlArgs& a, hipStream_t stream) {
+template <int CIN, bool LN, bool GATHER = false>
+int launch_k5q(const ConvXlArgs& a, hipStream_t stream, const K5qGather& g = K5qGather{}) {
     const size_t lds = ((size_t)CIN * XW + (LN ? 512 : 0)) * sizeof(float);
     static bool attr_set = false;
     if (!attr_set) {
-        if (hipFuncSetAttribute(reinterpret_cast<const void*>(conv_k5q_kernel<CIN, LN>), hipFuncAttributeMaxDynamicSharedMemorySize, (int)lds) != hipSuccess) return -3;
+        if (hipFuncSetAttribute(reinterpret_cast<const void*>(conv_k5q_kernel<CIN, LN, GATHER>), hipFuncAttributeMaxDynamicSharedMemorySize, (int)lds) != hipSuccess) return -3;
         attr_set = true;
     }
     const long tiles = (long)((a.T + BN - 1) / BN) * a.B;
     const int split = a.row_split == 1 || a.row_split == 2 || a.row_split == 4 ? a.row_split : (tiles >= 128 ? 1 : tiles >= 64 ? 2 : 4);
     dim3 grid((a.T + BN - 1) / BN, a.B, split);
-    hipLaunchKernelGGL((conv_k5q_kernel<CIN, LN>), grid, dim3(256 / split), lds, stream, a);
+    hipLaunchKernelGGL((conv_k5q_kernel<CIN, LN, GATHER>), grid, dim3(256 / split), lds, stream, a, g);
     return hipGetLastError() == hipSuccess ? 0 : -3;
 }
 
@@ -251,3 +298,9 @@
     if (cin == 128 && !a->ln_g) return launch_k5q<128, false>(*a, s);
     return -2;
 }
+
+extern "C" int cmtts_launch_conv_k5q_lr(const ConvXlArgs* a, const K5qGather* g, void* stream_) {
+    if (a->C != CO || a->k != KT || a->dil != 1 || a->T < 1 || a->B < 1 || a->res || a->accum || a->slope != 1.0f || !a->wf || !a->bias) return -2;
+    if (a->cin != 128 || a->ln_g || !g || !g->mel2ph || !g->src || !g->pad || !g->pe_alpha || !g->pe_omega || g->ldl < 1) return -2;
+    return launch_k5q<128, false, true>(*a, (hipStream_t)stream_, *g);
+}
diff --git a/cm-tts_amd/csrc/conv_xres.hip b/cm-tts_amd/csrc/conv_xres.hip
--- a/cm-tts_amd/csrc/conv_xres.hip
+++ b/cm-tts_amd/csrc/conv_xres.hip
@@ -2,6 +2,8 @@
 #include <stdlib.h>
 #include "conv_args.h"
 #include "conv_epilogue.h"
+#include "conv_xres_pe.h"
+#include "pos_embed.h"
 
 typedef float f32x4 __attribute__((ext_vector_type(4)));
 typedef float f32x2 __attribute__((ext_vector_type(2)));
@@ -15,8 +17,8 @@
 constexpr int HALO = 8;
 constexpr int RING = 4;
 
-template <bool LN, int NT, int WQ = 0>
-__global__ __launch_bounds__(256, NT == 1 ? XRES_OCC1 : 1) void conv_xres_kernel(const ConvArgs a, const float* __restrict__ wfrag, long long* dbg) {
+template <bool LN, int NT, int WQ = 0, bool PE = false>
+__global__ __launch_bounds__(256, NT == 1 ? XRES_OCC1 : 1) void conv_xres_kernel(const ConvArgs a, const float* __restrict__ wfrag, long long* dbg, const XresPe pe) {
     constexpr int BN = 32 * NT;
     constexpr int X_LD = BN + HALO;
     extern __shared__ __attribute__((aligned(16))) float xs[];
@@ -57,6 +59,51 @@
     const int xw = BN + (a.taps - 1) * a.dil;
     float* gs = xs + a.K * X_LD;
     if (LN) { gs[tid] = a.ln_g[tid]; gs[256 + tid] = a.ln_b[tid]; }
+    if constexpr (PE) {
+        __shared__ int pe_flag[X_LD], pe_pos[X_LD], pe_cnt[4];
+        const int t00 = n0 - a.pad;
+        int cnt = 0;
+        for (int t = tid; t < min(t00, a.Tin); t += 256) cnt += Xb[t] != 0.f ? 1 : 0;
+#pragma unroll
+        for (int off = 32; off > 0; off >>= 1) cnt += __shfl_xor(cnt, off);
+        if (lane == 0) pe_cnt[w] = cnt;
+        if (tid < X_LD) {
+            const int t = t00 + tid;
+            pe_flag[tid] = (t >= 0 && t < a.Tin && Xb[t] != 0.f) ? 1 : 0;
+        }
+        __syncthreads();
+        if (tid < X_LD) {
+            int run = (pe_cnt[0] + pe_cnt[1]) + (pe_cnt[2] + pe_cnt[3]);
+            for (int i = 0; i <= tid; ++i) run += pe_flag[i];
+            pe_pos[tid] = pe_flag[tid] ? run : 0;
+        }
+        __syncthreads();
+        const float al = pe.alpha[0];
+        const int nel = a.K * X_LD;
+#pragma unroll 1
+        for (int base = tid; base < nel; base += 256 * 8) {
+            float xv[8], tv[8];
+#pragma unroll
+            for (int u = 0; u < 8; ++u) {
+                const int idx = min(base + 256 * u, nel - 1);
+                const int row = idx / X_LD, c = idx - row * X_LD;
+                const int t = t00 + c;
+                xv[u] = Xb[(long)row * a.ldx + min(max(t, 0), a.Tin - 1)];
+                tv[u] = pe.tab[(long)min(pe_pos[c], pe.rows - 1) * a.K + row];
+            }
+#pragma unroll
+            for (int u = 0; u < 8; ++u) {
+                const int idx = base + 256 * u;
+                if (idx < nel) {
+                    const int row = idx / X_LD, c = idx - row * X_LD;
+                    const int t = t00 + c, p = pe_pos[c];
+                    const bool ok = c < xw && t >= 0 && t < a.Tin;
+                    const float pv = p == 0 ? 0.f : (p < pe.rows ? tv[u] : pos_embed(p, row, a.K, pe.omega, pe.tab, pe.rows));
+                    xs[idx] = ok ? pos_embed_sum(xv[u], al, pv) : 0.f;
+                }
+            }
+        }
+    } else
     if (((n0 - a.pad) & 3) == 0 && (a.ldx & 3) == 0 && ((uintptr_t)Xb & 15) == 0) {
         constexpr int V = X_LD / 4, U = NT == 3 ? 26 : 10;
         const int nvec = a.K * V;
@@ -530,17 +577,38 @@
     if (dbg) {
         static const char* twice = getenv("CMTTS_XRES_DBG_TWICE");
         if (twice && atoi(twice) == 1 && a.out[0].res != a.out[0].Y && !a.w2frag) {
-            if (nt == 3) { if (a.ln_g) hipLaunchKernelGGL((conv_xres_kernel<true, 3>), grid, dim3(256), lds, st, a, wfrag, nullptr); else hipLaunchKernelGGL((conv_xres_kernel<false, 3>), grid, dim3(256), lds, st, a, wfrag, nullptr); }
-            else { if (a.ln_g) hipLaunchKernelGGL((conv_xres_kernel<true, 1>), grid, dim3(256), lds, st, a, wfrag, nullptr); else hipLaunchKernelGGL((conv_xres_kernel<false, 1>), grid, dim3(256), lds, st, a, wfrag, nullptr); }
+            if (nt == 3) { if (a.ln_g) hipLaunchKernelGGL((conv_xres_kernel<true, 3>), grid, dim3(256), lds, st, a, wfrag, nullptr, XresPe{}); else hipLaunchKernelGGL((conv_xres_kernel<false, 3>), grid, dim3(256), lds, st, a, wfrag, nullptr, XresPe{}); }
+            else { if (a.ln_g) hipLaunchKernelGGL((conv_xres_kernel<true, 1>), grid, dim3(256), lds, st, a, wfrag, nullptr, XresPe{}); else hipLaunchKernelGGL((conv_xres_kernel<false, 1>), grid, dim3(256), lds, st, a, wfrag, nullptr, XresPe{}); }
         }
     }
     if (nt == 3) {
-        if (a.ln_g) hipLaunchKernelGGL((conv_xres_kernel<true, 3>), grid, dim3(256), lds, st, a, wfrag, dbg);
-        else hipLaunchKernelGGL((conv_xres_kernel<false, 3>), grid, dim3(256), lds, st, a, wfrag, dbg);
+        if (a.ln_g) hipLaunchKernelGGL((conv_xres_kernel<true, 3>), grid, dim3(256), lds, st, a, wfrag, dbg, XresPe{});
+        else hipLaunchKernelGGL((conv_xres_kernel<false, 3>), grid, dim3(256), lds, st, a, wfrag, dbg, XresPe{});
     } else {
-        if (a.ln_g) hipLaunchKernelGGL((conv_xres_kernel<true, 1>), grid, dim3(256), lds, st, a, wfrag, dbg);
-        else hipLaunchKernelGGL((conv_xres_kernel<false, 1>), grid, dim3(256), lds, st, a, wfrag, dbg);
-    }
+        if (a.ln_g) hipLaunchKernelGGL((conv_xres_kernel<true, 1>), grid, dim3(256), lds, st, a, wfrag, dbg, XresPe{});
+        else hipLaunchKernelGGL((conv_xres_kernel<false, 1>), grid, dim3(256), lds, st, a, wfrag, dbg, XresPe{});
+    }
+    return hipGetLastError() == hipSuccess ? 0 : -3;
+}
+
+extern "C" int cmtts_launch_conv_xres_pe(const ConvArgs* ap, const float* wfrag, int nbatch, void* stream_, const XresPe* pe) {
+    const ConvArgs& a = *ap;
+    if (a.M <= 0 || a.N <= 0 || nbatch <= 0) return 0;
+    if (!wfrag || a.zdiv != 1 || a.split != INT_MAX || a.dil <= 0 || a.K % 32 != 0 || a.K > KMAX || (a.taps - 1) * a.dil > HALO ||
+        a.pre_div != 1.0f || a.pre_slope != 1.0f || a.ln_g || a.w2frag || !pe || !pe->alpha || !pe->omega || !pe->tab || pe->rows < 1 || a.Tin < 1)
+        return -2;
+    const int x_ld = 32 + HALO;
+    const size_t lds = (size_t)a.K * x_ld * sizeof(float);
+    static bool attr_set = false;
+    if (!attr_set) {
+        if (hipFuncSetAttribute(reinterpret_cast<const void*>(conv_xres_kernel<false, 1, 0, true>), hipFuncAttributeMaxDynamicSharedMemorySize,
+                                (int)((size_t)KMAX * x_ld * sizeof(float))) != hipSuccess)
+            return -3;
+        attr_set = true;
+    }
+    const int mblocks = ((a.M + 31) / 32 + 3) / 4;
+    dim3 grid((a.N + 31) / 32, mblocks, nbatch);
+    hipLaunchKernelGGL((conv_xres_kernel<false, 1, 0, true>), grid, dim3(256), lds, (hipStream_t)stream_, a, wfrag, nullptr, *pe);
     return hipGetLastError() == hipSuccess ? 0 : -3;
 }
 
@@ -584,18 +652,18 @@
     hipStream_t st = (hipStream_t)stream_;
     if (form == 2) {
         if (nt == 3) {
-            if (a.ln_g) hipLaunchKernelGGL((conv_xres_kernel<true, 3, 2>), grid, dim3(256), lds, st, a, wfrag, dbg);
-            else hipLaunchKernelGGL((conv_xres_kernel<false, 3, 2>), grid, dim3(256), lds, st, a, wfrag, dbg);
+            if (a.ln_g) hipLaunchKernelGGL((conv_xres_kernel<true, 3, 2>), grid, dim3(256), lds, st, a, wfrag, dbg, XresPe{});
+            else hipLaunchKernelGGL((conv_xres_kernel<false, 3, 2>), grid, dim3(256), lds, st, a, wfrag, dbg, XresPe{});
         } else {
-            if (a.ln_g) hipLaunchKernelGGL((conv_xres_kernel<true, 1, 2>), grid, dim3(256), lds, st, a, wfrag, dbg);
-            else hipLaunchKernelGGL((conv_xres_kernel<false, 1, 2>), grid, dim3(256), lds, st, a, wfrag, dbg);
+            if (a.ln_g) hipLaunchKernelGGL((conv_xres_kernel<true, 1, 2>), grid, dim3(256), lds, st, a, wfrag, dbg, XresPe{});
+            else hipLaunchKernelGGL((conv_xres_kernel<false, 1, 2>), grid, dim3(256), lds, st, a, wfrag, dbg, XresPe{});
         }
     } else if (nt == 3) {
-        if (a.ln_g) hipLaunchKernelGGL((conv_xres_kernel<true, 3, 1>), grid, dim3(256), lds, st, a, wfrag, dbg);
-        else hipLaunchKernelGGL((conv_xres_kernel<false, 3, 1>), grid, dim3(256), lds, st, a, wfrag, dbg);
+        if (a.ln_g) hipLaunchKernelGGL((conv_xres_kernel<true, 3, 1>), grid, dim3(256), lds, st, a, wfrag, dbg, XresPe{});
+        else hipLaunchKernelGGL((conv_xres_kernel<false, 3, 1>), grid, dim3(256), lds, st, a, wfrag, dbg, XresPe{});
     } else {
-        if (a.ln_g) hipLaunchKernelGGL((conv_xres_kernel<true, 1, 1>), grid, dim3(256), lds, st, a, wfrag, dbg);
-        else hipLaunchKernelGGL((conv_xres_kernel<false, 1, 1>), grid, dim3(256), lds, st, a, wfrag, dbg);
+        if (a.ln_g) hipLaunchKernelGGL((conv_xres_kernel<true, 1, 1>), grid, dim3(256), lds, st, a, wfrag, dbg, XresPe{});
+        else hipLaunchKernelGGL((conv_xres_kernel<false, 1, 1>), grid, dim3(256), lds, st, a, wfrag, dbg, XresPe{});
     }
     return hipGetLastError() == hipSuccess ? 0 : -3;
 }
diff --git a/cm-tts_amd/csrc/conv_xres_pe.h b/cm-tts_amd/csrc/conv_xres_pe.h
--- /dev/null
+++ b/cm-tts_amd/csrc/conv_xres_pe.h
@@ -0,0 +1,17 @@
+#pragma once
+#include "conv_args.h"
+
+struct XresPe {
+    const float* alpha;
+    const float* omega;
+    const float* tab;
+    int rows;
+};
+
+#ifdef __cplusplus
+extern "C" {
+#endif
+int cmtts_launch_conv_xres_pe(const ConvArgs* a, const float* wfrag, int nbatch, void* stream, const XresPe* pe);
+#ifdef __cplusplus
+}
+#endif
diff --git a/cm-tts_amd/csrc/internal_hooks.h b/cm-tts_amd/csrc/internal_hooks.h
--- a/cm-tts_amd/csrc/internal_hooks.h
+++ b/cm-tts_amd/csrc/internal_hooks.h
@@ -8,6 +8,8 @@
 int cmtts_internal_cond_factored(struct cmtts_model* m, const float* p1, int p1_ld, int L, const int64_t* mel2ph, const int64_t* p_idx, int B, int T,
                                  float* cp, void* stream);
 int cmtts_internal_mel_window_gather(const float* mel_ct, int B, int T, const int32_t* windows, int N, int Tw, float* out, void* stream);
+int cmtts_internal_pitch_conv0(struct cmtts_model* m, const float* h128, int ldl, const int64_t* mel2ph, int B, int T, int gather, float* hp, float* out,
+                               void* stream);
 #ifdef __cplusplus
 }
 #endif
diff --git a/cm-tts_amd/csrc/kernels.hip b/cm-tts_amd/csrc/kernels.hip
--- a/cm-tts_amd/csrc/kernels.hip
+++ b/cm-tts_amd/csrc/kernels.hip
@@ -2,20 +2,10 @@
 #include <math.h>
 #include <stdint.h>
 #include "kernels.h"
+#include "pos_embed.h"
 
 namespace {
 
-__device__ __forceinline__ float sin_exact(float a) { return (float)sin((double)a); }
-__device__ __forceinline__ float cos_exact(float a) { return (float)cos((double)a); }
-
-__device__ __forceinline__ float pos_embed(int p, int c, int C, const float* omega, const float* tab, int tab_rows) {
-    if (p == 0) return 0.f;
-    if (p < tab_rows) return tab[(long)p * C + c];
-    const int half = C >> 1;
-    const int j = c < half ? c : c - half;
-    const float arg = (float)p * omega[j];
-    return c < half ? sin_exact(arg) : cos_exact(arg);
-}
 
 template <typename FlagFn>
 __device__ void block_positions(FlagFn flag, int T, int* pos, int* counts) {
@@ -148,7 +138,7 @@
         const int c = c0 + cl;
         for (int t = threadIdx.x; t < T; t += 256) {
             const long off = ((long)b * C + c) * ld + t;
-            const float v = x[off] + al * pos_embed(pos[t], c, C, omega, tab, tab_rows);
+            const float v = pos_embed_add_value(x[off], al, pos[t], c, C, omega, tab, tab_rows);
             out[off] = t < valid ? v : 0.f;
         }
     }
@@ -174,7 +164,7 @@
         for (int t = threadIdx.x; t < T; t += 256) {
             const int64_t ph = mp[t];
             const float xv = ph > 0 ? sc[ph - 1] : pc;
-            out[((long)b * C + c) * T + t] = xv + al * pos_embed(pos[t], c, C, omega, tab, tab_rows);
+            out[((long)b * C + c) * T + t] = pos_embed_add_value(xv, al, pos[t], c, C, omega, tab, tab_rows);
         }
     }
 }
diff --git a/cm-tts_amd/csrc/pos_embed.h b/cm-tts_amd/csrc/pos_embed.h
--- /dev/null
+++ b/cm-tts_amd/csrc/pos_embed.h
@@ -0,0 +1,24 @@
+#pragma once
+#include <hip/hip_runtime.h>
+#include <math.h>
+
+namespace {
+
+__device__ __forceinline__ float sin_exact(float a) { return (float)sin((double)a); }
+__device__ __forceinline__ float cos_exact(float a) { return (float)cos((double)a); }
+
+__device__ __forceinline__ float pos_embed(int p, int c, int C, const float* omega, const float* tab, int tab_rows) {
+    if (p == 0) return 0.f;
+    if (p < tab_rows) return tab[(long)p * C + c];
+    const int half = C >> 1;
+    const int j = c < half ? c : c - half;
+    const float arg = (float)p * omega[j];
+    return c < half ? sin_exact(arg) : cos_exact(arg);
+}
+
+__device__ __forceinline__ float pos_embed_sum(float xv, float al, float pe) { return xv + al * pe; }
+__device__ __forceinline__ float pos_embed_add_value(float xv, float al, int p, int c, int C, const float* omega, const float* tab, int tab_rows) {
+    return pos_embed_sum(xv, al, pos_embed(p, c, C, omega, tab, tab_rows));
+}
+
+}
```
